# rpl-cmu/bevrender

Hardware: AMD Instinct MI355X
Metric: samples/sec fwd+bwd, 6-cam 256x704 BEV-lift+corr (higher is better)
Workload: dtype bf16; 1 GPU; cfg3: 6-cam 256x704 features (64x64x176), 200x200 BEV, C=64 h=2 D=5, L=2 encoder layers (TSA+SCA), T=2 (1 no-grad history frame(s) + 1 fwd+bwd), correlation head with contrastive + lifted-structure losses, AdamW; batch 8 per GPU; backbone/render CNN excluded; global_batch=8, per_gpu_batch=8, parallelism=dp1

## Files before the change

### bevrender_amd/_lib.py

```python
from __future__ import annotations

import ctypes as C
import os
import subprocess
import threading

import torch

_HERE = os.path.dirname(os.path.abspath(__file__))
LIB_PATH = os.environ.get("BEVRENDER_LIB") or os.path.join(_HERE, "lib", "libbevrender_hip.so")
CSRC = os.path.join(_HERE, "csrc")

PREC_F32, PREC_BF16, PREC_F16, PREC_BF16X3 = 0, 1, 2, 3
ABI_VERSION = 6

SYMBOLS = [
    "bevr_abi_version", "bevr_strerror", "bevr_attn_table_dims", "bevr_attn_key_ws_bytes", "bevr_attn_key_prep",
    "bevr_attn_fwd", "bevr_attn_bwd_q",
    "bevr_attn_bwd_k", "bevr_attn_fwd_dropout", "bevr_attn_bwd_q_dropout", "bevr_attn_bwd_k_dropout", "bevr_attn_cell_fwd", "bevr_attn_cell_bwd_q", "bevr_attn_cell_bwd_k", "bevr_attn_tap_ws_bytes", "bevr_attn_tap_prep", "bevr_attn_tap_fwd", "bevr_attn_tap_bwd_q", "bevr_attn_tap_bwd_k", "bevr_attn_tap_fwd_dropout", "bevr_attn_tap_bwd_q_dropout", "bevr_attn_tap_bwd_k_dropout", "bevr_attn_gather_fwd", "bevr_attn_gather_fwd_rows", "bevr_attn_gather_fwd_x3", "bevr_attn_slab_ws_bytes", "bevr_attn_slab_prep", "bevr_attn_slab_bwd_q", "bevr_attn_slab_rows_ws_bytes", "bevr_attn_slab_rows_prep", "bevr_attn_slab_bwd_q_rows", "bevr_sample_fwd", "bevr_sample_bwd", "bevr_sample_fwd_bf16", "bevr_sample_bwd_bf16", "bevr_project_bev_grid", "bevr_project_bev_grid_masked", "bevr_corr_fwd",
    "bevr_corr_bwd", "bevr_recall_rank", "bevr_dwconv_fwd", "bevr_dwconv_bwd_w", "bevr_dwconv_res_gelu", "bevr_affine_warp_fwd", "bevr_affine_warp_bwd",
    "bevr_offset_head_fwd", "bevr_offset_head_bwd", "bevr_key_positions_fwd", "bevr_key_positions_bwd", "bevr_kv_project", "bevr_layernorm_fwd", "bevr_layernorm_bwd", "bevr_merge_views_fwd", "bevr_merge_views_bwd", "bevr_merge_tap_fwd", "bevr_merge_tap_bwd", "bevr_attn_bwd_prep", "bevr_pack_kv", "bevr_unpack_dkv",
]


class AttnDesc(C.Structure):
    _fields_ = [(n, C.c_int32) for n in (
        "n_prob", "q_div", "heads", "groups", "S", "Sp", "N", "Np", "Ht", "Wt", "Hp", "Wp",
        "y_off", "x_off", "precision", "reserved")]


class BevrError(RuntimeError):
    pass


_lib = None
_lock = threading.Lock()


def build(verbose: bool = False) -> str:
    cmd = ["make", "-C", CSRC, "-j", "4"]
    res = subprocess.run(cmd, capture_output=True, text=True)
    if verbose or res.returncode != 0:
        print(res.stdout)
        print(res.stderr)
    if res.returncode != 0:
        raise BevrError("building libbevrender_hip.so failed (see output above)")
    return LIB_PATH


def lib() -> C.CDLL:
    global _lib
    if _lib is not None:
        return _lib
    with _lock:
        if _lib is not None:
            return _lib
        if not os.path.exists(LIB_PATH):
            raise BevrError(
                f"{LIB_PATH} not found: the HIP extension is required (no CPU fallback). "
                "Run `python -c 'import __graft_entry__ as g; g.build()'` or `make -C bevrender_amd/csrc`.")
        L = C.CDLL(LIB_PATH)
        vp, fp, ip = C.c_void_p, C.c_void_p, C.c_int
        dp = C.POINTER(AttnDesc)
        L.bevr_abi_version.restype = C.c_int
        L.bevr_strerror.restype = C.c_char_p
        L.bevr_strerror.argtypes = [C.c_int]
        L.bevr_attn_table_dims.argtypes = [dp]
        L.bevr_attn_key_ws_bytes.argtypes = [dp]
        L.bevr_attn_key_prep.argtypes = [dp, fp, fp, vp, vp]
        L.bevr_attn_fwd.argtypes = [dp, vp, vp, vp, vp, fp, fp, fp, vp]
        L.bevr_attn_bwd_q.argtypes = [dp] + [vp] * 4 + [vp, fp] + [vp, fp, fp, fp, fp, fp, vp]
        L.bevr_attn_bwd_k.argtypes = [dp] + [vp] * 4 + [fp] * 3 + [vp, vp, fp, fp, fp] + [fp] * 4 + [vp]
        u32 = C.c_uint32
        L.bevr_attn_fwd_dropout.argtypes = [dp, vp, vp, vp, vp, fp, fp, fp, u32, u32, vp]
        L.bevr_attn_bwd_q_dropout.argtypes = [dp] + [vp] * 4 + [vp, fp] + [vp, fp, fp, fp, fp, fp, u32, u32, vp]
        L.bevr_attn_bwd_k_dropout.argtypes = [dp] + [vp] * 4 + [fp] * 3 + [vp, vp, fp, fp, fp] + [fp] * 4 + [u32, u32, vp]
        L.bevr_attn_cell_fwd.argtypes = [dp, vp, vp, vp, vp, fp, fp, fp, fp, fp, vp]
        L.bevr_attn_cell_bwd_q.argtypes = [dp] + [vp] * 4 + [vp, fp] + [vp, fp, fp, fp, fp, fp, vp]
        L.bevr_attn_cell_bwd_k.argtypes = [dp] + [vp] * 4 + [vp, fp] + [vp, vp, fp, fp, fp] + [fp] * 4 + [vp]
        L.bevr_attn_tap_ws_bytes.argtypes = [dp]
        L.bevr_attn_tap_prep.argtypes = [dp, fp, fp, fp, fp, vp, vp]
        L.bevr_attn_tap_fwd.argtypes = [dp, vp, vp, fp, fp, fp, vp, vp]
        L.bevr_attn_tap_bwd_q.argtypes = [dp, vp, vp, vp, fp, fp, fp, vp]
        L.bevr_attn_tap_bwd_k.argtypes = [dp, vp, vp, vp, fp, fp, fp, fp, fp, vp]
        L.bevr_attn_tap_fwd_dropout.argtypes = [dp, vp, vp, fp, fp, fp, fp, vp, u32, u32, u32, vp]
        L.bevr_attn_tap_bwd_q_dropout.argtypes = [dp, vp, vp, vp, fp, fp, fp, u32, u32, u32, vp]
        L.bevr_attn_tap_bwd_k_dropout.argtypes = [dp, vp, vp, vp, fp, fp, fp, fp, fp, u32, u32, u32, vp]
        L.bevr_attn_gather_fwd.argtypes = [dp, vp, vp, vp, vp, vp, fp, fp, fp, vp, vp]
        L.bevr_attn_gather_fwd_rows.argtypes = [dp, vp, vp, vp, vp, vp, fp, fp, fp, vp, ip, ip, vp]
        L.bevr_attn_gather_fwd_x3.argtypes = [dp, vp, vp, vp, vp, vp, fp, fp, fp, vp, ip, ip, vp]
        L.bevr_attn_slab_ws_bytes.argtypes = [dp]
        L.bevr_attn_slab_prep.argtypes = [dp, fp, fp, vp, vp, vp]
        L.bevr_attn_slab_bwd_q.argtypes = [dp, vp, vp, vp, vp, fp, vp, fp, fp, fp, fp, fp, vp]
        L.bevr_attn_slab_rows_ws_bytes.argtypes = [dp]
        L.bevr_attn_slab_rows_prep.argtypes = [dp, fp, fp, vp, vp, vp]
        L.bevr_attn_slab_bwd_q_rows.argtypes = [dp, vp, vp, vp, vp, fp, vp, fp, fp, fp, fp, fp, ip, ip, vp]
        L.bevr_sample_fwd.argtypes = [fp, fp, fp] + [ip] * 5 + [vp]
        L.bevr_sample_bwd.argtypes = [fp] * 5 + [ip] * 5 + [vp]
        L.bevr_sample_fwd_bf16.argtypes = [vp, fp, fp] + [ip] * 5 + [vp]
        L.bevr_sample_bwd_bf16.argtypes = [vp] + [fp] * 4 + [ip] * 5 + [vp]
        L.bevr_project_bev_grid.argtypes = [fp] * 4 + [ip] * 4 + [vp]
        L.bevr_project_bev_grid_masked.argtypes = [fp] * 4 + [ip] * 4 + [vp] + [ip] * 3 + [vp]
        L.bevr_corr_fwd.argtypes = [fp] * 5 + [ip] * 4 + [vp]
        L.bevr_corr_bwd.argtypes = [fp] * 8 + [ip] * 4 + [vp]
        L.bevr_recall_rank.argtypes = [fp, vp, ip, vp]
        L.bevr_dwconv_fwd.argtypes = [fp, fp, fp, fp] + [ip] * 7 + [vp]
        L.bevr_dwconv_bwd_w.argtypes = [fp, fp, fp, fp] + [ip] * 6 + [vp]
        L.bevr_dwconv_res_gelu.argtypes = [fp] * 5 + [ip] * 6 + [vp]
        L.bevr_affine_warp_fwd.argtypes = [fp, fp, fp] + [ip] * 4 + [vp]
        L.bevr_affine_warp_bwd.argtypes = [fp, fp, fp] + [ip] * 4 + [vp]
        L.bevr_offset_head_fwd.argtypes = [fp] * 7 + [C.c_longlong] + [ip] * 4 + [C.c_float, vp]
        L.bevr_offset_head_bwd.argtypes = [fp] * 13 + [C.c_longlong] + [ip] * 4 + [C.c_float, vp]
        L.bevr_layernorm_fwd.argtypes = [fp] * 6 + [C.c_longlong, ip, C.c_float, vp]
        L.bevr_layernorm_bwd.argtypes = [fp] * 8 + [C.c_longlong, ip, vp]
        L.bevr_kv_project.argtypes = [vp, ip, fp, C.c_longlong, vp, fp] + [ip] * 9 + [vp] * 6 + [ip, vp]
        L.bevr_key_positions_fwd.argtypes = [fp, fp, vp, fp] + [ip] * 8 + [C.c_float, C.c_float, vp]
        L.bevr_key_positions_bwd.argtypes = [fp, fp, vp, fp, fp] + [ip] * 8 + [C.c_float, C.c_float, vp]
        L.bevr_pack_kv.argtypes = [fp, fp, C.c_longlong, C.c_longlong] + [ip] * 6 + [vp] * 5
        L.bevr_merge_views_fwd.argtypes = [fp] * 5 + [ip] * 6 + [vp]
        L.bevr_merge_views_bwd.argtypes = [fp] * 9 + [ip] * 6 + [vp]
        L.bevr_merge_tap_fwd.argtypes = [fp] * 7 + [ip] * 6 + [vp]
        L.bevr_merge_tap_bwd.argtypes = [fp] * 13 + [ip] * 6 + [vp]
        L.bevr_attn_bwd_prep.argtypes = [fp] * 5 + [vp, vp, fp, fp] + [ip] * 3 + [vp]
        L.bevr_unpack_dkv.argtypes = [fp] * 4 + [C.c_longlong, C.c_longlong] + [ip] * 5 + [vp]
        for name in SYMBOLS:
            fn = getattr(L, name)
            if name in ("bevr_attn_key_ws_bytes", "bevr_attn_tap_ws_bytes", "bevr_attn_slab_ws_bytes",
                        "bevr_attn_slab_rows_ws_bytes"):
                fn.restype = C.c_size_t
            elif name not in ("bevr_strerror",):
                fn.restype = C.c_int
        if L.bevr_abi_version() != ABI_VERSION:
            raise BevrError(f"libbevrender_hip.so ABI version {L.bevr_abi_version()} != {ABI_VERSION}: rebuild "
                            "(make -C bevrender_amd/csrc)")
        _lib = L
    return _lib


def check(code: int, what: str) -> None:
    if code != 0:
        msg = lib().bevr_strerror(code).decode()
        raise BevrError(f"{what} failed: {msg} (code {code})")
```

### bevrender_amd/csrc/attn_bwd_k.hip

```cpp
#include "attn_kstage.h"

#include "bevr_prof.h"

BEVR_PROF_DEFINE(bwd_k, 16)

namespace {

constexpr int KEYS_WG = 384;

struct KBox { int amin, amax; float bmin, bmax; };

__device__ __forceinline__ KBox wg_key_box(int a_lo, int a_hi, float b_lo, float b_hi, KBox* red, int n_wave, int wave,
                                           int lane) {
  KBox w;
  w.amin = lanes_min<64>(a_lo);
  w.amax = lanes_max<64>(a_hi);
  w.bmin = lanes_min<64>(b_lo);
  w.bmax = lanes_max<64>(b_hi);
  if (lane == 0) red[wave] = w;
  __syncthreads();
  KBox r = red[0];
  for (int k = 1; k < n_wave; ++k) {
    const KBox o = red[k];
    r.amin = min(r.amin, o.amin);
    r.amax = max(r.amax, o.amax);
    r.bmin = fminf(r.bmin, o.bmin);
    r.bmax = fmaxf(r.bmax, o.bmax);
  }
  return r;
}

struct Slab {
  int rows;
  int pitch;
  int ncw;
  bool fits;
};
__device__ __forceinline__ Slab make_slab(const KBox& kb, const bevr_attn_desc& d, int wcap, float rx_ceil) {
  Slab sl;
  if (kb.amax < kb.amin) {
    sl.rows = 1; sl.pitch = 1; sl.ncw = 1; sl.fits = true;
    return sl;
  }
  sl.rows = kb.amax - kb.amin + d.Sp + 1;
  sl.pitch = sl.rows + ((7 - sl.rows) & 31);
  sl.ncw = wcap / sl.pitch - 1;
  const int need = (int)floorf(kb.bmax - kb.bmin) + 4 + (int)rx_ceil + 1;
  sl.fits = sl.ncw >= need;
  return sl;
}

__device__ __forceinline__ void key_split(float a, float b, const bevr_attn_desc& d, int& A, float& fy, float& bc) {
  const KeyClamp c = key_clamp(a, b, d);
  bc = c.b;
  A = (int)c.af;
  fy = c.a - c.af;
}

constexpr int TW = 768;
constexpr int KWW = 1;

template <int PREC>
__global__ __launch_bounds__(TW, 3) void attn_bwd_k_win_kernel(
    bevr_attn_desc d, const char* __restrict__ Q, const char* __restrict__ Qt, const char* __restrict__ K,
    const char* __restrict__ V, const float* __restrict__ key_a, const float* __restrict__ key_b,
    const char* __restrict__ table_pair, const char* __restrict__ dO, const char* __restrict__ dOt,
    const float* __restrict__ LSE, const float* __restrict__ delta, const float* __restrict__ grad_scale,
    float* __restrict__ dK, float* __restrict__ dV, float* __restrict__ dkey_a, float* __restrict__ dkey_b BEVR_DROP_PARAMS) {
  constexpr int NT = is16(PREC) ? 2 : 1;
  const float kp16 = PREC == BEVR_PREC_F16 ? grad_scale[2] : 0.f, c2_16 = PREC == BEVR_PREC_F16 ? grad_scale[3] : 1.f;
  const float ds_inv = PREC == BEVR_PREC_F16 ? grad_scale[4] : 1.f, p_inv = PREC == BEVR_PREC_F16 ? grad_scale[5] : 1.f;
  typedef LdsK<PREC, NT> L;
  constexpr int EB = L::EB;
  static_assert(2 * L::BUF + L::WCAP * 4 + 256 <= 160 * 1024, "LDS budget");
  __shared__ __attribute__((aligned(16))) char smem[2 * L::BUF];
  __shared__ __attribute__((aligned(16))) float win[L::WCAP];
  __shared__ __attribute__((aligned(16))) KBox red[TW / 64];

  const int n_kb = (d.Np + KEYS_WG - 1) / KEYS_WG;
  const int n_ph = d.n_prob * d.heads;
  const int xcd = blockIdx.x & 7, slot = blockIdx.x >> 3;
  const int ph = (slot / n_kb) * 8 + xcd;
  if (ph >= n_ph) return;
  const int kblk = slot % n_kb;
  const int prob = ph / d.heads, hd = ph % d.heads;
  const int grp = hd / (d.heads / d.groups);
  const int qb = prob / d.q_div;

  const int tid = threadIdx.x, wave = tid >> 6, lane = tid & 63, lq = lane & 31, hi = lane >> 5;
  const int Mp = d.S * d.Sp;
  const int n_rb = d.Sp / 32;

  const char* Kh = K + ((size_t)ph * d.Np) * 32 * EB;
  const char* Vh = V + ((size_t)ph * d.Np) * 32 * EB;
  const float* ka = key_a + (size_t)(prob * d.groups + grp) * d.Np;
  const float* kb = key_b + (size_t)(prob * d.groups + grp) * d.Np;
  const char* tbl = table_pair + (size_t)hd * d.Wp * d.Hp * 8;
  const float rx = (float)(d.Wt - 1) / (2.0f * (float)(d.S - 1));

  bool wave_live[KWW], dead[KWW];
  int key[KWW], A[KWW];
  float fy[KWW], bcl[KWW];
  int a_lo = 0x7fffffff, a_hi = (int)0x80000000;
  float b_lo = 3.0e38f, b_hi = -3.0e38f;
#pragma unroll
  for (int w = 0; w < KWW; ++w) {
    const int k0 = kblk * KEYS_WG + (wave * KWW + w) * 32;
    wave_live[w] = k0 < d.Np;
    key[w] = wave_live[w] ? k0 + lq : lq;
    dead[w] = !wave_live[w] || key[w] >= d.N;
    key_split(ka[key[w]], kb[key[w]], d, A[w], fy[w], bcl[w]);
    if (!dead[w]) {
      a_lo = min(a_lo, A[w]); a_hi = max(a_hi, A[w]);
      b_lo = fminf(b_lo, bcl[w]); b_hi = fmaxf(b_hi, bcl[w]);
    }
  }
  const KBox box = wg_key_box(a_lo, a_hi, b_lo, b_hi, red, TW / 64, wave, lane);
  const Slab sl = make_slab(box, d, L::WCAP, ceilf(rx));
  if (!sl.fits) {
#pragma unroll
    for (int w = 0; w < KWW; ++w) {
      if (!wave_live[w]) continue;
      float* kr = dK + ((size_t)ph * d.Np + key[w]) * 32;
      float* vr = dV + ((size_t)ph * d.Np + key[w]) * 32;
      const f32x4 z = {0.f, 0.f, 0.f, 0.f};
#pragma unroll
      for (int g4 = 0; g4 < 4; ++g4) {
        *reinterpret_cast<f32x4*>(kr + 8 * g4 + 4 * hi) = z;
        *reinterpret_cast<f32x4*>(vr + 8 * g4 + 4 * hi) = z;
      }
    }
    return;
  }
  if (box.amax < box.amin) {
#pragma unroll
    for (int w = 0; w < KWW; ++w) {
      if (!wave_live[w]) continue;
      float* kr = dK + ((size_t)ph * d.Np + key[w]) * 32;
      float* vr = dV + ((size_t)ph * d.Np + key[w]) * 32;
      const f32x4 z = {0.f, 0.f, 0.f, 0.f};
#pragma unroll
      for (int g4 = 0; g4 < 4; ++g4) {
        *reinterpret_cast<f32x4*>(kr + 8 * g4 + 4 * hi) = z;
        *reinterpret_cast<f32x4*>(vr + 8 * g4 + 4 * hi) = z;
      }
    }
    return;
  }
  int arel4[KWW];
  Frag<PREC> kf[KWW], vf[KWW];
  f32x16 dk[KWW], dv[KWW];
  float da[KWW], db[KWW], fx[KWW];
  int base0[KWW], base1[KWW];
#pragma unroll
  for (int w = 0; w < KWW; ++w) {
    if (dead[w]) { A[w] = box.amin; bcl[w] = box.bmin; fy[w] = 0.f; }
    arel4[w] = (A[w] - box.amin) * 4;
    kf[w].load(Kh + (size_t)key[w] * 32 * EB, hi);
    vf[w].load(Vh + (size_t)key[w] * 32 * EB, hi);
#pragma unroll
    for (int r = 0; r < 16; ++r) { dk[w][r] = 0.f; dv[w][r] = 0.f; }
    da[w] = 0.f; db[w] = 0.f; fx[w] = 0.f; base0[w] = 0; base1[w] = 0;
  }

  QStage<PREC, TW, NT> qs;
  qs.init(tid, Q + ((size_t)(qb * d.heads + hd) * Mp) * 32 * EB, dO + ((size_t)ph * Mp) * 32 * EB,
          Qt + ((size_t)(qb * d.heads + hd) * 32) * Mp * EB, dOt + ((size_t)ph * 32) * Mp * EB,
          LSE + (size_t)ph * Mp, delta + (size_t)ph * Mp, Mp, kp16);
  const int n_tile = d.S * n_rb;
  const int n_it = (n_tile + NT - 1) / NT;
  auto first_tile = [&](int it) { return NT == 1 ? it : max(0, min(NT * it, n_tile - NT)); };
  qs.load(tid, (size_t)first_tile(0) * 32);
  qs.store(tid, smem);

  const int xbase = (int)floorf(box.bmin) - 8;
  const float inv_ncw = 1.0f / (float)sl.ncw;
  auto slot_of = [&](int X) {
    const int xs = X - xbase;
    int q = (int)((float)xs * inv_ncw);
    int r = xs - q * sl.ncw;
    r = r < 0 ? r + sl.ncw : r;
    r = r >= sl.ncw ? r - sl.ncw : r;
    return r;
  };
  int whi = -(1 << 30);
  constexpr int PF = 4;
  const int kill_off = sl.ncw * sl.pitch * 4;
  for (int r = tid; r < sl.pitch; r += TW) win[sl.ncw * sl.pitch + r] = BEVR_NEG_BIG;
  const int n_chunk = (sl.rows + 63) / 64;
  const size_t trow0 = (size_t)(box.amin + d.y_off);
  __syncthreads();

  PROF_ACC(8);
  for (int it = 0; it < n_it; ++it) {
    PROF_T_LGKM(t0, 0.f);
    const int buf = it & 1;
    const char* base = smem + buf * L::BUF;
    const int t_first = first_tile(it);
    if (it + 1 < n_it) qs.load(tid, (size_t)first_tile(it + 1) * 32);
    int pf_first = 0, pf_units = 0;
    float pf_v[PF];
#pragma unroll
    for (int sub = 0; sub < NT; ++sub) {
    const int t = t_first + sub;
    if (t < NT * it) continue;
    const int j = t / n_rb, rb = t - j * n_rb;
    if (rb == 0) {
      const float jr = (float)j * rx;
      const int xhi = (int)floorf(jr + box.bmax) + 1;
      if (whi < xhi) {
        const int xlo = (int)floorf(jr + box.bmin);
        const int xfirst = max(whi + 1, xlo);
        const int n_new = xhi - xfirst + 1;
        for (int u = wave; u < n_new * n_chunk; u += TW / 64) {
          const int c = u / n_chunk, ch = u - c * n_chunk;
          const int X = xfirst + c;
          const int row = ch * 64 + lane;
          if (row < sl.rows) {
            const float v = *reinterpret_cast<const float*>(tbl + ((size_t)(X + d.x_off) * d.Hp + trow0 + row) * 8);
            win[slot_of(X) * sl.pitch + row] = v;
          }
        }
        whi = xhi;
        __syncthreads();
      }
#pragma unroll
      for (int w = 0; w < KWW; ++w) {
        const float tx = jr + bcl[w];
        const float xf = floorf(tx);
        fx[w] = dead[w] ? 0.f : tx - xf;
        const int X = (int)xf;
        base0[w] = dead[w] ? kill_off : slot_of(X) * sl.pitch * 4 + arel4[w];
        base1[w] = dead[w] ? kill_off : slot_of(X + 1) * sl.pitch * 4 + arel4[w];
      }
    }
    if (sub == NT - 1 && rb == n_rb - 1 && j + 1 < d.S) {
      const float jr = (float)(j + 1) * rx;
      const int xhi = (int)floorf(jr + box.bmax) + 1;
      const int xfirst = max(whi + 1, (int)floorf(jr + box.bmin));
      const int units = (xhi - xfirst + 1) * n_chunk;
      if (units <= PF * (TW / 64)) {
        pf_first = xfirst;
        pf_units = units;
        whi = xhi;
#pragma unroll
        for (int k = 0; k < PF; ++k) {
          const int u = wave + k * (TW / 64);
          const int c = u / n_chunk, ch = u - c * n_chunk;
          const int row = ch * 64 + lane;
          pf_v[k] = 0.f;
          if (u < units && row < sl.rows)
            pf_v[k] = *reinterpret_cast<const float*>(tbl + ((size_t)(xfirst + c + d.x_off) * d.Hp + trow0 + row) * 8);
        }
      }
    }
    PROF_T_LGKM(t1, 0.f);
    PROF_ADD(0, t1 - t0);

#pragma unroll
    for (int w = 0; w < KWW; ++w) {
      if (!wave_live[w]) continue;
      const f32x4* rc = reinterpret_cast<const f32x4*>(base + 2 * L::TILE_Q + 2 * L::TILE_T) + sub * 8;
      f32x16 s, dp;
      {
        Frag<PREC> qf;
        qf.load(base + (sub * 32 + lq) * L::STRIDE, hi);
#pragma unroll
        for (int g4 = 0; g4 < 4; ++g4) {
          const f32x4 l4 = rc[2 * g4 + hi];
#pragma unroll
          for (int k = 0; k < 4; ++k) s[4 * g4 + k] = l4[k];
        }
        s = mma_frag(qf, kf[w], s);
      }
      {
        Frag<PREC> dof;
        dof.load(base + L::TILE_Q + (sub * 32 + lq) * L::STRIDE, hi);
#pragma unroll
        for (int g4 = 0; g4 < 4; ++g4) {
          const f32x4 d4 = rc[NT * 8 + 2 * g4 + hi];
#pragma unroll
          for (int k = 0; k < 4; ++k) dp[4 * g4 + k] = d4[k];
        }
        dp = mma_frag(dof, vf[w], dp);
      }
#if BEVR_DROP
      unsigned kmask = 0u;
      const float ksc = 65536.0f / (65536.0f - (float)drop_thr);
#pragma unroll
      for (int r = 0; r < 16; ++r) {
        const uint32_t hrow = bevr_drop_row(drop_seed, (uint32_t)ph, (uint32_t)(j * d.Sp + rb * 32 + crow(r, hi)));
        const bool keep = bevr_drop_keep(hrow, (uint32_t)key[w], drop_thr);
        const float nd = rc[NT * 8 + 2 * (r >> 2) + hi][r & 3];
        dp[r] = keep ? fmaf(ksc, dp[r] - nd, nd) : nd;
        kmask |= (keep ? 1u : 0u) << r;
      }
#endif
      PROF_T_LGKM(t2, s[0] + dp[15]);
      PROF_ADD(1, t2 - t1);

      const int ioff = (rb * 32 + 4 * hi) * 4;
      const char* p0 = reinterpret_cast<const char*>(win) + base0[w] + ioff;
      const char* p1 = reinterpret_cast<const char*>(win) + base1[w] + ioff;
      const f32x2 fy2 = {fy[w], fy[w]}, fx2 = {fx[w], fx[w]};
      f32x2 sa2 = {0.f, 0.f}, sb2 = {0.f, 0.f};
      const int n_live = d.S - rb * 32;
#pragma unroll
      for (int g4 = 0; g4 < 4; ++g4) {
        if (8 * g4 >= n_live) {
#pragma unroll
          for (int k = 0; k < 4; ++k) { s[4 * g4 + k] = 0.f; dp[4 * g4 + k] = 0.f; }
          continue;
        }
#pragma unroll
        for (int h = 0; h < 2; ++h) {
          const int r = 4 * g4 + 2 * h, o = (8 * g4 + 2 * h) * 4;
          const float* a0 = reinterpret_cast<const float*>(p0 + o);
          const float* a1 = reinterpret_cast<const float*>(p1 + o);
          const f32x2 ta = {a0[0], a0[1]}, tb = {a0[1], a0[2]};
          const f32x2 qa = {a1[0], a1[1]}, qb = {a1[1], a1[2]};
          const f32x2 d0 = tb - ta, d1 = qb - qa;
          const f32x2 u0 = ta + fy2 * d0;
          const f32x2 u1 = qa + fy2 * d1;
          const f32x2 du = u1 - u0;
          const f32x2 s2 = {s[r], s[r + 1]}, dp2 = {dp[r], dp[r + 1]};
          const f32x2 sv = (s2 + u0) + fx2 * du;
          const f32x2 pp = {fast_exp2(sv[0]), fast_exp2(sv[1])};
          f32x2 ds = pp * dp2;
          if constexpr (PREC == BEVR_PREC_F16) ds *= f32x2{c2_16, c2_16};
          s[r] = pp[0]; s[r + 1] = pp[1];
          dp[r] = ds[0]; dp[r + 1] = ds[1];
          sa2 += ds * (d0 + fx2 * (d1 - d0));
          sb2 += ds * du;
        }
      }
      const float sa = sa2[0] + sa2[1], sb = sb2[0] + sb2[1];
      da[w] += sa;
      db[w] += sb;
#if BEVR_DROP
#pragma unroll
      for (int r = 0; r < 16; ++r) s[r] = ((kmask >> r) & 1u) ? s[r] * ksc : 0.f;
#endif
      PROF_T_LGKM(t3, sa + sb + s[15]);
      PROF_ADD(2, t3 - t2);
      {
        Frag<PREC> dotf;
        load_perm(dotf, base + 2 * L::TILE_Q + L::TILE_T + lq * L::TSTRIDE + sub * 32 * EB, hi);
        dv[w] = mma_acc_b(dotf, s, dv[w]);
      }
      {
        Frag<PREC> qtf;
        load_perm(qtf, base + 2 * L::TILE_Q + lq * L::TSTRIDE + sub * 32 * EB, hi);
        dk[w] = mma_acc_b(qtf, dp, dk[w]);
      }
      PROF_T_LGKM(t4, dk[w][0] + dv[w][0]);
      PROF_ADD(3, t4 - t3);
    }

    }

    PROF_T_LGKM(t5, 0.f);
    if (pf_units > 0) {
#pragma unroll
      for (int k = 0; k < PF; ++k) {
        const int u = wave + k * (TW / 64);
        const int c = u / n_chunk, ch = u - c * n_chunk;
        const int row = ch * 64 + lane;
        if (u < pf_units && row < sl.rows) win[slot_of(pf_first + c) * sl.pitch + row] = pf_v[k];
      }
    }
    if (it + 1 < n_it) qs.store(tid, smem + (buf ^ 1) * L::BUF);
    PROF_T_LGKM(t6, 0.f);
    __syncthreads();
    PROF_T_LGKM(t7, 0.f);
    PROF_ADD(4, t6 - t5);
    PROF_ADD(5, t7 - t6);
    PROF_ADD(6, t7 - t0);
    PROF_ADD(7, 1);
  }
  PROF_FLUSH(bwd_k, wave ? 8 : 0, lane == 0 && (wave == 0 || wave == 11));

#pragma unroll
  for (int w = 0; w < KWW; ++w) {
    if (!wave_live[w]) continue;
    float* kr = dK + ((size_t)ph * d.Np + key[w]) * 32;
    float* vr = dV + ((size_t)ph * d.Np + key[w]) * 32;
#pragma unroll
    for (int g4 = 0; g4 < 4; ++g4) {
      f32x4 a, b;
#pragma unroll
      for (int k = 0; k < 4; ++k) { a[k] = BEVR_LN2 * ds_inv * dk[w][4 * g4 + k]; b[k] = p_inv * dv[w][4 * g4 + k]; }
      *reinterpret_cast<f32x4*>(kr + 8 * g4 + 4 * hi) = a;
      *reinterpret_cast<f32x4*>(vr + 8 * g4 + 4 * hi) = b;
    }
    const float sa = BEVR_LN2 * ds_inv * (da[w] + __shfl_xor(da[w], 32));
    const float sb = BEVR_LN2 * ds_inv * (db[w] + __shfl_xor(db[w], 32));
    if (hi == 0) {
      atomicAdd(dkey_a + (size_t)(prob * d.groups + grp) * d.Np + key[w], sa);
      atomicAdd(dkey_b + (size_t)(prob * d.groups + grp) * d.Np + key[w], sb);
    }
  }
}

constexpr int TG = 256;
constexpr int KW = 3;
constexpr int GSPLIT = 4;

template <int PREC>
__global__ __launch_bounds__(TG) void attn_bwd_k_gather_kernel(
    bevr_attn_desc d, const char* __restrict__ Q, const char* __restrict__ Qt, const char* __restrict__ K,
    const char* __restrict__ V, const float* __restrict__ key_a, const float* __restrict__ key_b,
    const char* __restrict__ table_pair, const char* __restrict__ dO, const char* __restrict__ dOt,
    const float* __restrict__ LSE, const float* __restrict__ delta, const float* __restrict__ grad_scale,
    float* __restrict__ dK, float* __restrict__ dV, float* __restrict__ dkey_a, float* __restrict__ dkey_b BEVR_DROP_PARAMS) {
  typedef LdsK<PREC> L;
  const float kp16 = PREC == BEVR_PREC_F16 ? grad_scale[2] : 0.f, c2_16 = PREC == BEVR_PREC_F16 ? grad_scale[3] : 1.f;
  const float ds_inv = PREC == BEVR_PREC_F16 ? grad_scale[4] : 1.f, p_inv = PREC == BEVR_PREC_F16 ? grad_scale[5] : 1.f;
  constexpr int EB = L::EB;
  __shared__ __attribute__((aligned(16))) char smem[2 * L::BUF];
  __shared__ __attribute__((aligned(16))) KBox red[4];

  const int n_kb = (d.Np + KEYS_WG - 1) / KEYS_WG;
  const int n_ph = d.n_prob * d.heads;
  const int xcd = blockIdx.x & 7, slot = blockIdx.x >> 3;
  const int ph = (slot / (n_kb * GSPLIT)) * 8 + xcd;
  if (ph >= n_ph) return;
  const int kblk = (slot % (n_kb * GSPLIT)) / GSPLIT;
  const int split = slot % GSPLIT;
  const int prob = ph / d.heads, hd = ph % d.heads;
  const int grp = hd / (d.heads / d.groups);
  const int qb = prob / d.q_div;

  const int tid = threadIdx.x, wave = tid >> 6, lane = tid & 63, lq = lane & 31, hi = lane >> 5;
  const int Mp = d.S * d.Sp;
  const int n_rb = d.Sp / 32;

  const char* Kh = K + ((size_t)ph * d.Np) * 32 * EB;
  const char* Vh = V + ((size_t)ph * d.Np) * 32 * EB;
  const float* ka = key_a + (size_t)(prob * d.groups + grp) * d.Np;
  const float* kb = key_b + (size_t)(prob * d.groups + grp) * d.Np;
  const char* tbl = table_pair + (size_t)hd * d.Wp * d.Hp * 8;
  const int Hp8 = d.Hp * 8;
  const float rx = (float)(d.Wt - 1) / (2.0f * (float)(d.S - 1));

  KeyC kc[KW];
  bool wave_live[KW];
  int key_idx[KW];
#pragma unroll
  for (int w = 0; w < KW; ++w) {
    const int k0 = kblk * KEYS_WG + (wave * KW + w) * 32;
    wave_live[w] = k0 < d.Np;
    const int key = wave_live[w] ? k0 + lq : lq;
    key_idx[w] = key;
    kc[w] = make_keyc(ka[key], kb[key], d);
  }
  KBox box;
  {
    int a_lo = 0x7fffffff, a_hi = (int)0x80000000;
    float b_lo = 3.0e38f, b_hi = -3.0e38f;
#pragma unroll
    for (int w = 0; w < KW; ++w) {
      if (wave_live[w] && key_idx[w] < d.N) {
        int A;
        float fy, bc;
        key_split(ka[key_idx[w]], kb[key_idx[w]], d, A, fy, bc);
        a_lo = min(a_lo, A); a_hi = max(a_hi, A);
        b_lo = fminf(b_lo, bc); b_hi = fmaxf(b_hi, bc);
      }
    }
    box = wg_key_box(a_lo, a_hi, b_lo, b_hi, red, TG / 64, wave, lane);
  }
  if (make_slab(box, d, L::WCAP, ceilf(rx)).fits) return;

  Frag<PREC> kf[KW], vf[KW];
#pragma unroll
  for (int w = 0; w < KW; ++w) {
    kf[w].load(Kh + (size_t)key_idx[w] * 32 * EB, hi);
    vf[w].load(Vh + (size_t)key_idx[w] * 32 * EB, hi);
  }
  f32x16 dk[KW], dv[KW];
  float da[KW], db[KW];
#pragma unroll
  for (int w = 0; w < KW; ++w) {
#pragma unroll
    for (int r = 0; r < 16; ++r) { dk[w][r] = 0.f; dv[w][r] = 0.f; }
    da[w] = 0.f;
    db[w] = 0.f;
  }

  QStage<PREC, TG> qs;
  qs.init(tid, Q + ((size_t)(qb * d.heads + hd) * Mp) * 32 * EB, dO + ((size_t)ph * Mp) * 32 * EB,
          Qt + ((size_t)(qb * d.heads + hd) * 32) * Mp * EB, dOt + ((size_t)ph * 32) * Mp * EB,
          LSE + (size_t)ph * Mp, delta + (size_t)ph * Mp, Mp, kp16);
  const int n_all = d.S * n_rb;
  const int chunk = (n_all + GSPLIT - 1) / GSPLIT;
  const int it_first = split * chunk, n_it = min(n_all, it_first + chunk);
  if (it_first >= n_it) return;
  qs.load(tid, (size_t)(it_first / n_rb) * d.Sp + (it_first % n_rb) * 32);
  qs.store(tid, smem);
  __syncthreads();

  for (int it = it_first; it < n_it; ++it) {
    const int buf = (it - it_first) & 1;
    const char* base = smem + buf * L::BUF;
    const int j = it / n_rb, i0 = (it % n_rb) * 32;
    if (it + 1 < n_it) {
      const int jn = (it + 1) / n_rb, rbn = (it + 1) % n_rb;
      qs.load(tid, (size_t)jn * d.Sp + rbn * 32);
    }
    const float jr = (float)j * rx;

    Frag<PREC> qf, dof, qtf, dotf;
    qf.load(base + lq * L::STRIDE, hi);
    dof.load(base + L::TILE + lq * L::STRIDE, hi);
    load_perm(qtf, base + 2 * L::TILE + lq * L::STRIDE, hi);
    load_perm(dotf, base + 3 * L::TILE + lq * L::STRIDE, hi);
    const f32x4* rc = reinterpret_cast<const f32x4*>(base + 4 * L::TILE);

#pragma unroll
    for (int w = 0; w < KW; ++w) {
      if (!wave_live[w]) continue;
      f32x16 s, dp;
#pragma unroll
      for (int g4 = 0; g4 < 4; ++g4) {
        f32x4 l4 = rc[2 * g4 + hi], d4 = rc[8 + 2 * g4 + hi];
#pragma unroll
        for (int k = 0; k < 4; ++k) { s[4 * g4 + k] = l4[k]; dp[4 * g4 + k] = d4[k]; }
      }
      s = mma_frag(qf, kf[w], s);
      dp = mma_frag(dof, vf[w], dp);
#if BEVR_DROP
      unsigned kmask = 0u;
      const float ksc = 65536.0f / (65536.0f - (float)drop_thr);
#pragma unroll
      for (int r = 0; r < 16; ++r) {
        const uint32_t hrow = bevr_drop_row(drop_seed, (uint32_t)ph, (uint32_t)(j * d.Sp + i0 + crow(r, hi)));
        const bool keep = bevr_drop_keep(hrow, (uint32_t)key_idx[w], drop_thr);
        const float nd = rc[8 + 2 * (r >> 2) + hi][r & 3];
        dp[r] = keep ? fmaf(ksc, dp[r] - nd, nd) : nd;
        kmask |= (keep ? 1u : 0u) << r;
      }
#endif

      const KeyC c = kc[w];
      float tx = jr + c.b;
      float xf = floorf(tx);
      float fx = tx - xf;
      const char* tp = tbl + (unsigned)((int)xf * Hp8 + c.aoff + (i0 + 4 * hi) * 8);
      const bool dead = key_idx[w] >= d.N;
      float sa = 0.f, sb = 0.f;
#pragma unroll
      for (int r = 0; r < 16; ++r) {
        f32x2 t0 = *reinterpret_cast<const f32x2*>(tp + crow(r, 0) * 8);
        f32x2 t1 = *reinterpret_cast<const f32x2*>(tp + Hp8 + crow(r, 0) * 8);
        float u0 = t0[0] * c.wy0 + t0[1] * c.fy;
        float u1 = t1[0] * c.wy0 + t1[1] * c.fy;
        float sv = s[r] + u0 + fx * (u1 - u0);
        float p = dead ? 0.f : fast_exp2(sv);
        float ds = BEVR_LN2 * c2_16 * p * dp[r];
        s[r] = p;
        dp[r] = ds;
        float ga = (t0[1] - t0[0]) + fx * ((t1[1] - t1[0]) - (t0[1] - t0[0]));
        sa += ds * ga;
        sb += ds * (u1 - u0);
      }
      da[w] += sa;
      db[w] += sb;
#if BEVR_DROP
#pragma unroll
      for (int r = 0; r < 16; ++r) s[r] = ((kmask >> r) & 1u) ? s[r] * ksc : 0.f;
#endif
      dv[w] = mma_acc_b(dotf, s, dv[w]);
      dk[w] = mma_acc_b(qtf, dp, dk[w]);
    }

    if (it + 1 < n_it) qs.store(tid, smem + (buf ^ 1) * L::BUF);
    __syncthreads();
  }

#pragma unroll
  for (int w = 0; w < KW; ++w) {
    if (!wave_live[w]) continue;
    const int key = key_idx[w];
    float* kr = dK + ((size_t)ph * d.Np + key) * 32;
    float* vr = dV + ((size_t)ph * d.Np + key) * 32;
#pragma unroll
    for (int g4 = 0; g4 < 4; ++g4) {
#pragma unroll
      for (int k = 0; k < 4; ++k) {
        atomicAdd(kr + 8 * g4 + 4 * hi + k, ds_inv * dk[w][4 * g4 + k]);
        atomicAdd(vr + 8 * g4 + 4 * hi + k, p_inv * dv[w][4 * g4 + k]);
      }
    }
    float sa = ds_inv * (da[w] + __shfl_xor(da[w], 32));
    float sb = ds_inv * (db[w] + __shfl_xor(db[w], 32));
    if (hi == 0) {
      atomicAdd(dkey_a + (size_t)(prob * d.groups + grp) * d.Np + key, sa);
      atomicAdd(dkey_b + (size_t)(prob * d.groups + grp) * d.Np + key, sb);
    }
  }
}

template <int PREC>
int launch(const bevr_attn_desc& d, const void* Q, const void* Qt, const void* K, const void* V, const float* key_a,
           const float* key_b, const float* table_pair, const void* dO, const void* dOt, const float* LSE,
           const float* delta, const float* gs, float* dK, float* dV, float* dka, float* dkb, hipStream_t st BEVR_DROP_PARAMS) {
  const int n_kb = (d.Np + KEYS_WG - 1) / KEYS_WG;
  const int n_ph = d.n_prob * d.heads;
  const int grid = ((n_ph + 7) / 8) * 8 * n_kb;
  hipLaunchKernelGGL((attn_bwd_k_win_kernel<PREC>), dim3(grid), dim3(TW), 0, st, d, (const char*)Q, (const char*)Qt,
                     (const char*)K, (const char*)V, key_a, key_b, (const char*)table_pair, (const char*)dO,
                     (const char*)dOt, LSE, delta, gs, dK, dV, dka, dkb BEVR_DROP_ARGS);
  int rc = (int)hipGetLastError();
  if (rc) return rc;
  hipLaunchKernelGGL((attn_bwd_k_gather_kernel<PREC>), dim3(grid * GSPLIT), dim3(TG), 0, st, d, (const char*)Q,
                     (const char*)Qt, (const char*)K, (const char*)V, key_a, key_b, (const char*)table_pair,
                     (const char*)dO, (const char*)dOt, LSE, delta, gs, dK, dV, dka, dkb BEVR_DROP_ARGS);
  return (int)hipGetLastError();
}

}

#if BEVR_DROP
extern "C" int bevr_attn_bwd_k_dropout(const bevr_attn_desc* d, const void* Q, const void* Qt, const void* K, const void* V,
                                       const float* key_a, const float* key_b, const float* table_pair, const void* dO,
                                       const void* dOt, const float* LSE, const float* delta, const float* grad_scale,
                                       float* dK, float* dV, float* dkey_a, float* dkey_b, unsigned drop_thr,
                                       unsigned drop_seed, void* stream) {
  if (drop_thr >= 65536u) return BEVR_E_SHAPE;
#else
extern "C" int bevr_attn_bwd_k(const bevr_attn_desc* d, const void* Q, const void* Qt, const void* K, const void* V,
                               const float* key_a, const float* key_b, const float* table_pair, const void* dO,
                               const void* dOt, const float* LSE, const float* delta, const float* grad_scale,
                               float* dK, float* dV, float* dkey_a, float* dkey_b, void* stream) {
#endif
  int rc = bevr_check_desc(d);
  if (rc) return rc;
  if (!Q || !Qt || !K || !V || !key_a || !key_b || !table_pair || !dO || !dOt || !LSE || !delta || !dK || !dV ||
      !dkey_a || !dkey_b || (d->precision == BEVR_PREC_F16 && !grad_scale))
    return BEVR_E_NULL;
  if (!bevr_aligned16(Q) || !bevr_aligned16(Qt) || !bevr_aligned16(K) || !bevr_aligned16(V) || !bevr_aligned16(dO) ||
      !bevr_aligned16(dOt) || !bevr_aligned16(dK) || !bevr_aligned16(dV) || !bevr_aligned16(table_pair))
    return BEVR_E_ALIGN;
  hipStream_t st = (hipStream_t)stream;
  if (d->precision == BEVR_PREC_BF16)
    return launch<BEVR_PREC_BF16>(*d, Q, Qt, K, V, key_a, key_b, table_pair, dO, dOt, LSE, delta, grad_scale, dK, dV,
                                  dkey_a, dkey_b, st BEVR_DROP_ARGS);
  if (d->precision == BEVR_PREC_F16)
    return launch<BEVR_PREC_F16>(*d, Q, Qt, K, V, key_a, key_b, table_pair, dO, dOt, LSE, delta, grad_scale, dK, dV,
                                 dkey_a, dkey_b, st BEVR_DROP_ARGS);
  if (d->precision == BEVR_PREC_BF16X3)
    return launch<BEVR_PREC_BF16X3>(*d, Q, Qt, K, V, key_a, key_b, table_pair, dO, dOt, LSE, delta, grad_scale, dK, dV,
                               dkey_a, dkey_b, st BEVR_DROP_ARGS);
  return launch<BEVR_PREC_F32>(*d, Q, Qt, K, V, key_a, key_b, table_pair, dO, dOt, LSE, delta, grad_scale, dK, dV,
                               dkey_a, dkey_b, st BEVR_DROP_ARGS);
}
```

### bevrender_amd/csrc/attn_tap_bwd_k.hip

```cpp
#include <type_traits>
#include "attn_tap.h"

namespace {

constexpr int NKW = 7;
constexpr int NCW = 8;
constexpr int NRX = 8;
constexpr int SPB = 2;
template <int NP> struct LdsKn {
  static constexpr int OFF_G = 0;
  static constexpr int OFF_H = 1024;
  static constexpr int OFF_LO = 2048;
  static constexpr int SLAB = 2048 * NP;
  static constexpr int BUF = SPB * SLAB;
};
typedef LdsKn<1> LdsK;
template <int PREC> using LdsKp = LdsKn<tap_np<PREC>>;
constexpr int tap_bwd_k_waves(int prec) { return tap_split(prec) ? 2 : 4; }
__host__ __device__ __forceinline__ int win_dwords(int Sp) { return (Sp + NRX + 8) / 2; }

__device__ __forceinline__ bool tile_fits(const StepBox& sb, float jrx, int a0w, float bminw) {
  const int da = sb.amin - a0w;
  const int dx = (int)floorf(jrx + sb.bmin) - (int)floorf(jrx + bminw);
  return sb.amax >= sb.amin && da >= 0 && da <= NRX && box_fits(sb, jrx) && dx >= 0 && dx <= NCW - CELL_C;
}

template <int PREC, bool SLOW>
__global__ __launch_bounds__(64 * (NKW + 1), tap_bwd_k_waves(PREC)) void attn_tap_bwd_k_kernel(
    bevr_attn_desc d, const char* __restrict__ G, const char* __restrict__ H, const char* __restrict__ tap_ws,
    const float* __restrict__ table_t, float* __restrict__ dkey_a, float* __restrict__ dkey_b,
    float* __restrict__ dkey_y, float* __restrict__ dkey_x, int n_wg_ph TAP_DROP_PARAMS) {
  typedef LdsKp<PREC> L;
  constexpr bool X3 = tap_split(PREC);
  constexpr int NP = tap_np<PREC>;
  extern __shared__ __attribute__((aligned(16))) char smem[];

  const int n_ph = d.n_prob * d.heads;
  const int xcd = blockIdx.x & 7, slot = blockIdx.x >> 3;
  const int ph = (slot / n_wg_ph) * 8 + xcd;
  if (ph >= n_ph) return;
  const int wg = slot % n_wg_ph;
  const int prob = ph / d.heads, hd = ph % d.heads;
  const int tid = threadIdx.x;
  const int wave = __builtin_amdgcn_readfirstlane(tid >> 6), lane = tid & 63;
  const int li = lane & 15, g = lane >> 4;
  const int Mp = d.S * d.Sp;
  const int nslab = d.Sp / 32, nstep = (nslab + SPB - 1) / SPB;
  const int n_tiles = d.Np / 32;
  const float rx = (float)(d.Wt - 1) / (2.0f * (float)(d.S - 1));
  const int HpT = d.Hp + 1;
  const float* tbl = table_t + (size_t)hd * d.Wp * HpT;
  const StepBox* box = reinterpret_cast<const StepBox*>(tap_ws + tap_ws_box_offset(d)) + (size_t)prob * (d.Np / 32);
  const int NRWD = win_dwords(d.Sp);
  const int win_bytes = 4 * NCW * NRWD * 4;
  char* win_base = smem + 2 * L::BUF;
  TapRec* stash = reinterpret_cast<TapRec*>(win_base + 3 * win_bytes) + wave * 32;

  int a0w = 0x7fffffff;
  float bminw = 3.0e38f;
  for (int t = 0; t < NKW; ++t) {
    const int tile = wg * NKW + t;
    if (tile < n_tiles) {
      const StepBox b = box[tile];
      if (b.amax >= b.amin) {
        a0w = min(a0w, b.amin);
        bminw = fminf(bminw, b.bmin);
      }
    }
  }
  if (a0w == 0x7fffffff) { a0w = 0; bminw = 0.f; }
  if constexpr (SLOW) {
    bool unfit = false;
    for (int t = 0; t < NKW; ++t) {
      const int tile = wg * NKW + t;
      if (tile >= n_tiles) break;
      const StepBox b = box[tile];
      if (b.amax < b.amin) continue;
      for (int j = lane; j < d.S; j += 64) unfit = unfit || !tile_fits(b, (float)j * rx, a0w, bminw);
    }
    if (!__any(unfit)) return;
  }

  if (wave == NKW) {
    __builtin_amdgcn_s_setprio(3);
    const int n_quad = (NRWD + 1) / 2, n_item = NCW * n_quad;
    auto item_load = [&](int jn, int it, float (&t)[5]) {
      if (it >= n_item || jn >= d.S) return;
      const int c = it / n_quad, m = it - c * n_quad;
      const int x0w = (int)floorf((float)jn * rx + bminw);
      const int xc = max(0, min(x0w + c + d.x_off, d.Wp - 1));
      const int y = max(0, min(a0w + d.y_off + 4 * m, HpT - 5));
      const float* src = tbl + (size_t)xc * HpT + y;
#pragma unroll
      for (int k = 0; k < 5; ++k) t[k] = src[k];
    };
    auto item_store = [&](int jn, int it, const float (&t)[5]) {
      if (it >= n_item || jn >= d.S) return;
      const int c = it / n_quad, m = it - c * n_quad;
      const uint32_t h01 = TapHalf<PREC>::pack2(t[0], t[1]), h23 = TapHalf<PREC>::pack2(t[2], t[3]);
      const uint32_t h12 = TapHalf<PREC>::pack2(t[1], t[2]), h34 = TapHalf<PREC>::pack2(t[3], t[4]);
      const uint32_t l01 = TapHalf<PREC>::pack2(t[0] - TapHalf<PREC>::lo(h01), t[1] - TapHalf<PREC>::hi(h01));
      const uint32_t l23 = TapHalf<PREC>::pack2(t[2] - TapHalf<PREC>::lo(h23), t[3] - TapHalf<PREC>::hi(h23));
      const uint32_t l12 = TapHalf<PREC>::pack2(t[1] - TapHalf<PREC>::lo(h12), t[2] - TapHalf<PREC>::hi(h12));
      const uint32_t l34 = TapHalf<PREC>::pack2(t[3] - TapHalf<PREC>::lo(h34), t[4] - TapHalf<PREC>::hi(h34));
      uint32_t* w = reinterpret_cast<uint32_t*>(win_base + (jn % 3) * win_bytes) + c * NRWD + 2 * m;
      const bool second = 2 * m + 1 < NRWD;
      w[0] = h01;
      w[NCW * NRWD] = h12;
      w[2 * NCW * NRWD] = l01;
      w[3 * NCW * NRWD] = l12;
      if (second) {
        w[1] = h23;
        w[NCW * NRWD + 1] = h34;
        w[2 * NCW * NRWD + 1] = l23;
        w[3 * NCW * NRWD + 1] = l34;
      }
    };
    const int per_step = (n_item + nstep - 1) / nstep;
    auto slice_item = [&](int s2, int r) {
      const int k = r * 64 + lane;
      return k < per_step ? s2 * per_step + k : n_item;
    };
    float f0[5] = {0.f, 0.f, 0.f, 0.f, 0.f}, f1[5] = {0.f, 0.f, 0.f, 0.f, 0.f};
    if constexpr (!SLOW) {
      for (int it = lane; it < n_item; it += 64) {
        float t[5] = {0.f, 0.f, 0.f, 0.f, 0.f};
        item_load(0, it, t);
        item_store(0, it, t);
      }
      item_load(1, slice_item(0, 0), f0);
      item_load(1, slice_item(0, 1), f1);
    }
    const char* Gp = G + ((size_t)ph * Mp) * 32 + lane * 16;
    const char* Hq = H + ((size_t)ph * Mp) * 32 + lane * 16;
    auto slab_index = [&](int j2, int st2, int u) { return min(j2 * nslab + min(SPB * st2 + u, nslab - 1), d.S * nslab - 1); };
    int e = 0;
    u32x4 gv[NP][SPB], hv[NP][SPB];
    const size_t g_lo = (size_t)n_ph * Mp * 32;
    auto rows_load = [&](int j2, int st2) {
#pragma unroll
      for (int pl = 0; pl < NP; ++pl)
#pragma unroll
        for (int u = 0; u < SPB; ++u) {
          gv[pl][u] = gload16(Gp + pl * g_lo + (size_t)slab_index(j2, st2, u) * 1024);
          hv[pl][u] = gload16(Hq + pl * g_lo + (size_t)slab_index(j2, st2, u) * 1024);
        }
    };
    rows_load(0, 0);
    for (int j = 0; j < d.S; ++j) {
      for (int st = 0; st < nstep; ++st, ++e) {
        char* bb = smem + (e & 1) * L::BUF;
#pragma unroll
        for (int pl = 0; pl < NP; ++pl)
#pragma unroll
          for (int u = 0; u < SPB; ++u) {
            *reinterpret_cast<u32x4*>(bb + u * L::SLAB + pl * L::OFF_LO + L::OFF_G + lane * 16) = gv[pl][u];
            *reinterpret_cast<u32x4*>(bb + u * L::SLAB + pl * L::OFF_LO + L::OFF_H + lane * 16) = hv[pl][u];
          }
        if constexpr (!SLOW) {
          item_store(j + 1, slice_item(st, 0), f0);
          item_store(j + 1, slice_item(st, 1), f1);
          for (int k = 128 + lane; k < per_step; k += 64) {
            float t[5] = {0.f, 0.f, 0.f, 0.f, 0.f};
            item_load(j + 1, st * per_step + k, t);
            item_store(j + 1, st * per_step + k, t);
          }
        }
        const int jn = st + 1 < nstep ? j : min(j + 1, d.S - 1), stn = st + 1 < nstep ? st + 1 : 0;
        rows_load(jn, stn);
        if constexpr (!SLOW) {
          const int jf = st + 1 < nstep ? j + 1 : j + 2;
          item_load(jf, slice_item(stn, 0), f0);
          item_load(jf, slice_item(stn, 1), f1);
        }
        __syncthreads();
      }
    }
    __syncthreads();
    return;
  }

  const int tile = wg * NKW + wave;
  const bool have_tile = tile < n_tiles;
  const TapRec* recs = reinterpret_cast<const TapRec*>(tap_ws) + (size_t)prob * d.Np;
  const int tl = have_tile ? tile : 0;
  const StepBox sb = box[tl];
  const int da = sb.amin - a0w;

  TapOp<NP> bk[2];
  f32x4 zt[2], zv[2], zc[2];
  float acc_a[2] = {0.f, 0.f}, acc_b[2] = {0.f, 0.f};
#pragma unroll
  for (int kb = 0; kb < 2; ++kb) {
    const TapRec r0 = recs[(size_t)tl * 32 + 16 * kb + li];
    if (g == 0) stash[16 * kb + li] = r0;
    TapOp<NP> t[2];
    tap_weights<PREC>(r0.ys, r0.xs, t);
#pragma unroll
    for (int pl = 0; pl < NP; ++pl) bk[kb].p[pl] = g == 0 ? t[0].p[pl] : t[1].p[pl];
    zt[kb] = f32x4{0.f, 0.f, 0.f, 0.f};
    zv[kb] = f32x4{0.f, 0.f, 0.f, 0.f};
    zc[kb] = f32x4{0.f, 0.f, 0.f, 0.f};
  }
  const int a_row = L::OFF_G + li * 32 + (g & 1) * 16;
  const int t_off = (4 * g + (li >> 2)) * 32 + (lane & 3) * 8;
  const int cell_c = li >> 2, cell_r = li & 3;
#if BEVR_DROP
  uint32_t khk[2];
#pragma unroll
  for (int kb = 0; kb < 2; ++kb)
    khk[kb] = ((key0 + (uint32_t)(tl * 32 + 16 * kb + li)) * 0xC2B2AE3Du) ^ drop_seed ^ ((uint32_t)ph * 0x9E3779B1u);
  uint32_t hcol = 0u;
#endif

  int e = 0;
  float jrx = 0.f;
  const char* win_b = nullptr;
  int wq0 = 0, wq1 = 0, wth = 0, wtl = 0;
  const int win_lo = 2 * NCW * NRWD * 4;
  auto slab = [&](auto fit_tag, const char* base, int i0) {
    constexpr bool FIT = decltype(fit_tag)::value;
    TapOp<NP> qa[2], ha[2];
#pragma unroll
    for (int rb = 0; rb < 2; ++rb) {
      qa[rb] = ha[rb] = TapOp<NP>{};
      if (g < 2) {
        qa[rb] = tap_ld<NP>(base + a_row + rb * 512, L::OFF_LO);
        ha[rb] = tap_ld<NP>(base + L::OFF_H - L::OFF_G + a_row + rb * 512, L::OFF_LO);
      } else if (FIT) {
#pragma unroll
        for (int pl = 0; pl < NP; ++pl) {
          const uint32_t* w0 = reinterpret_cast<const uint32_t*>(win_b + pl * win_lo + wq0 + 2 * i0) + 8 * rb;
          const uint32_t* w1 = reinterpret_cast<const uint32_t*>(win_b + pl * win_lo + wq1 + 2 * i0) + 8 * rb;
          qa[rb].p[pl] = __builtin_bit_cast(bf16x8, u32x4{w0[0], w0[1], w1[0], w1[1]});
        }
      }
    }
    const TapOp<NP> gt = tap_ld_tr<NP>(base + L::OFF_G + t_off, 512, L::OFF_LO);
    const TapOp<NP> ht = tap_ld_tr<NP>(base + L::OFF_H + t_off, 512, L::OFF_LO);
    bf16x8 thi = gt.p[0], tlo = gt.p[0];
    if constexpr (FIT) {
      const uint32_t* w0 = reinterpret_cast<const uint32_t*>(win_b + wth + 2 * i0);
      const uint32_t* w1 = reinterpret_cast<const uint32_t*>(win_b + wtl + 2 * i0);
      thi = __builtin_bit_cast(bf16x8, u32x4{w0[0], w0[1], w0[8], w0[9]});
      tlo = __builtin_bit_cast(bf16x8, u32x4{w1[0], w1[1], w1[8], w1[9]});
    }
#if BEVR_DROP
    const uint32_t hq0 = hcol + (uint32_t)i0 * 0x85EBCA77u;
    auto hq = [&](int r) { return hq0 + (uint32_t)(16 * (r >> 2) + (r & 3)) * 0x85EBCA77u; };
    float ndel[8];
#pragma unroll
    for (int r = 0; r < 8; ++r) {
      const uint32_t c2 = *reinterpret_cast<const uint32_t*>(base + L::OFF_H + (16 * (r >> 2) + 4 * g + (r & 3)) * 32 + TAP_CHI * 2);
      ndel[r] = TapHalf<PREC>::lo(c2) + TapHalf<PREC>::hi(c2);
    }
#endif
#pragma unroll
    for (int kb = 0; kb < 2; ++kb) {
      const f32x4 z4 = {0.f, 0.f, 0.f, 0.f};
      const f32x4 s0 = tap_mm<PREC, true>(qa[0], bk[kb], z4);
      const f32x4 s1 = tap_mm<PREC, true>(qa[1], bk[kb], z4);
      const f32x4 q0 = tap_mm<PREC>(ha[0], bk[kb], z4);
      const f32x4 q1 = tap_mm<PREC>(ha[1], bk[kb], z4);
      float p[8], ds[8];
      if constexpr (!FIT) {
        const TapRec rk = stash[16 * kb + li];
        const float a = rk.a, tx = jrx + rk.b;
        const float af = floorf(a), xf = floorf(tx);
        const float fy = a - af, fx = tx - xf;
        const bool dead = rk.ys < -50.0f;
        const int xc = max(0, min((int)xf + d.x_off, d.Wp - 2));
        const int yb = (int)af + d.y_off + i0 + 4 * g;
        float pa = 0.f, pb = 0.f;
#pragma unroll
        for (int r = 0; r < 8; ++r) {
          const int y = max(0, min(yb + (r & 3) + 16 * (r >> 2), HpT - 2));
          const float* c0p = tbl + (size_t)xc * HpT + y;
          const float t00 = c0p[0], t01 = c0p[1], t10 = c0p[HpT], t11 = c0p[HpT + 1];
          const float u0 = t00 + fy * (t01 - t00), u1 = t10 + fy * (t11 - t10);
          const float sv = (r < 4 ? s0[r & 3] : s1[r & 3]) + (dead ? 0.f : u0 + fx * (u1 - u0));
          p[r] = fast_exp2(sv);
#if BEVR_DROP
          {
            const bool keep = tap_drop_keep(hq(r), khk[kb], drop_thr);
            ds[r] = p[r] * (keep ? (r < 4 ? q0[r & 3] : q1[r & 3]) : ndel[r]);
            p[r] = keep ? p[r] : 0.f;
          }
#else
          ds[r] = p[r] * (r < 4 ? q0[r & 3] : q1[r & 3]);
#endif
          pa += ds[r] * ((1.0f - fx) * (t01 - t00) + fx * (t11 - t10));
          pb += ds[r] * (u1 - u0);
        }
        acc_a[kb] += dead ? 0.f : pa;
        acc_b[kb] += dead ? 0.f : pb;
      } else {
#pragma unroll
        for (int r = 0; r < 4; ++r) {
#if BEVR_DROP
          p[r] = fast_exp2(s0[r]);
          p[4 + r] = fast_exp2(s1[r]);
          const bool keep0 = tap_drop_keep(hq(r), khk[kb], drop_thr), keep1 = tap_drop_keep(hq(4 + r), khk[kb], drop_thr);
          ds[r] = p[r] * (keep0 ? q0[r] : ndel[r]);
          ds[4 + r] = p[4 + r] * (keep1 ? q1[r] : ndel[4 + r]);
          p[r] = keep0 ? p[r] : 0.f;
          p[4 + r] = keep1 ? p[4 + r] : 0.f;
#else
          p[r] = fast_exp2(s0[r]);
          ds[r] = p[r] * q0[r];
          p[4 + r] = fast_exp2(s1[r]);
          ds[4 + r] = p[4 + r] * q1[r];
#endif
        }
      }
      u32x4 dsw[NP], pw[NP];
#pragma unroll
      for (int k = 0; k < 4; ++k) {
        tap_pack2<PREC>(ds[2 * k], ds[2 * k + 1], k, dsw);
        tap_pack2<PREC>(p[2 * k], p[2 * k + 1], k, pw);
      }
      const TapOp<NP> ds8 = tap_op(dsw), p8 = tap_op(pw);
      zt[kb] = tap_mm<PREC>(gt, ds8, zt[kb]);
      zv[kb] = tap_mm<PREC>(ht, p8, zv[kb]);
      if constexpr (FIT) {
        zc[kb] = mfma16<PREC>(tlo, ds8.p[0], zc[kb]);
        if constexpr (X3) zc[kb] = mfma16<PREC>(thi, ds8.p[1], zc[kb]);
        zc[kb] = mfma16<PREC>(thi, ds8.p[0], zc[kb]);
      }
    }
  };

  for (int j = 0; j < d.S; ++j) {
    jrx = (float)j * rx;
#if BEVR_DROP
    hcol = (uint32_t)(j * d.Sp + 4 * g) * 0x85EBCA77u;
#endif
    const int x0 = (int)floorf(jrx + sb.bmin), a0 = sb.amin;
    const int dx = x0 - (int)floorf(jrx + bminw);
    const bool fit = tile_fits(sb, jrx, a0w, bminw);
    const bool mine = have_tile && sb.amax >= sb.amin && fit != SLOW;
    auto chunk_coords = [&](int kb, float& tcol, float& trow) {
      const TapRec rk = stash[16 * kb + li];
      const float tx = jrx + rk.b;
      const float xf = floorf(tx);
      tcol = rk.ys < -50.0f ? -8.0f : (xf - (float)x0) + (tx - xf);
      trow = rk.a - (float)a0;
    };
#pragma unroll
    for (int kb = 0; kb < 2; ++kb) {
      if (g >= 2) {
        bk[kb] = TapOp<NP>{};
        if (!SLOW && mine) {
          float tcol, trow;
          chunk_coords(kb, tcol, trow);
          bk[kb] = tap_cell_half<PREC>(tcol, trow, g - 2);
        }
      }
      zc[kb] = f32x4{0.f, 0.f, 0.f, 0.f};
    }
    win_b = win_base + (j % 3) * win_bytes;
    {
      const int iq = li + da, pq = iq & 1;
      wq0 = ((pq * NCW + dx + 2 * max(g - 2, 0)) * NRWD + ((iq - pq) >> 1)) * 4;
      wq1 = wq0 + NRWD * 4;
      const int it = 4 * g + cell_r + da, pt = it & 1;
      wth = ((pt * NCW + dx + cell_c) * NRWD + ((it - pt) >> 1)) * 4;
      wtl = wth + win_lo;
    }
    for (int st = 0; st < nstep; ++st, ++e) {
      __syncthreads();
      if (!mine) continue;
#pragma unroll
      for (int u = 0; u < SPB; ++u)
        if (SPB * st + u < nslab) slab(std::integral_constant<bool, !SLOW>{}, smem + (e & 1) * L::BUF + u * L::SLAB, 32 * (SPB * st + u));
    }
    if (!SLOW && mine) {
#pragma unroll
      for (int kb = 0; kb < 2; ++kb) {
        float tc, tr;
        chunk_coords(kb, tc, tr);
        const float c0 = floorf(tc), r0 = floorf(tr);
        const float wxg = hat((float)g - tc);
        const float z0 = zc[kb][0], z1 = zc[kb][1], z2 = zc[kb][2], z3 = zc[kb][3];
        const float zl = r0 < 0.5f ? z0 : (r0 < 1.5f ? z1 : z2);
        const float zh = r0 < 0.5f ? z1 : (r0 < 1.5f ? z2 : z3);
        const float zrow = hat(0.f - tr) * z0 + hat(1.f - tr) * z1 + hat(2.f - tr) * z2 + hat(3.f - tr) * z3;
        const float sg = ((float)g == c0 + 1.0f ? 1.0f : 0.f) - ((float)g == c0 ? 1.0f : 0.f);
        acc_a[kb] += wxg * (zh - zl);
        acc_b[kb] += sg * zrow;
      }
    }
  }
  __syncthreads();

  if (!have_tile) return;
#pragma unroll
  for (int kb = 0; kb < 2; ++kb) {
    const TapRec rk = stash[16 * kb + li];
    const float ys = rk.ys, xs = rk.xs;
    const float y0 = floorf(ys), x0f = floorf(xs);
    float gy = 0.f, gx = 0.f;
#pragma unroll
    for (int e2 = 0; e2 < 4; ++e2) {
      const int t = 4 * g + e2;
      const float r = (float)(t / 3), c = (float)(t % 3);
      const float dwy = (r == y0 + 1.0f ? 1.0f : 0.f) - (r == y0 ? 1.0f : 0.f);
      const float dwx = (c == x0f + 1.0f ? 1.0f : 0.f) - (c == x0f ? 1.0f : 0.f);
      const float z = g < 3 ? zt[kb][e2] + BEVR_LOG2E * zv[kb][e2] : 0.f;
      gy += z * dwy * hat(c - xs);
      gx += z * hat(r - ys) * dwx;
    }
    float va = acc_a[kb], vb = acc_b[kb];
    gy += __shfl_xor(gy, 16); gx += __shfl_xor(gx, 16); va += __shfl_xor(va, 16); vb += __shfl_xor(vb, 16);
    gy += __shfl_xor(gy, 32); gx += __shfl_xor(gx, 32); va += __shfl_xor(va, 32); vb += __shfl_xor(vb, 32);
    const int n = tile * 32 + 16 * kb + li;
    if (g == 0 && n < d.N) {
      const size_t idx = (size_t)prob * d.Np + n;
      atomicAdd(dkey_a + idx, va);
      atomicAdd(dkey_b + idx, vb);
      atomicAdd(dkey_y + idx, gy);
      atomicAdd(dkey_x + idx, gx);
    }
  }
}

template <int PREC>
int launch(const bevr_attn_desc& d, const void* G, const void* H, const void* tap_ws, const float* table_t, float* dkey_a,
           float* dkey_b, float* dkey_y, float* dkey_x, hipStream_t st TAP_DROP_PARAMS) {
  typedef LdsKp<PREC> L;
  const int n_ph = d.n_prob * d.heads;
  const int n_tiles = d.Np / 32;
  const int n_wg_ph = (n_tiles + NKW - 1) / NKW;
  const size_t lds = 2 * L::BUF + (size_t)3 * 4 * NCW * win_dwords(d.Sp) * 4 + NKW * 32 * sizeof(TapRec);
  if (lds > 160 * 1024) return BEVR_E_SHAPE;
  const long long grid = (long long)((n_ph + 7) / 8) * 8 * n_wg_ph;
  if (grid > 0x7fffffffLL) return BEVR_E_SHAPE;
  hipLaunchKernelGGL((attn_tap_bwd_k_kernel<PREC, false>), dim3((unsigned)grid), dim3(64 * (NKW + 1)), lds, st, d, (const char*)G,
                     (const char*)H, (const char*)tap_ws, table_t, dkey_a, dkey_b, dkey_y, dkey_x, n_wg_ph TAP_DROP_ARGS);
  const int rc = (int)hipGetLastError();
  if (rc) return rc;
  hipLaunchKernelGGL((attn_tap_bwd_k_kernel<PREC, true>), dim3((unsigned)grid), dim3(64 * (NKW + 1)), lds, st, d, (const char*)G,
                     (const char*)H, (const char*)tap_ws, table_t, dkey_a, dkey_b, dkey_y, dkey_x, n_wg_ph TAP_DROP_ARGS);
  return (int)hipGetLastError();
}

}

#if BEVR_TAP_X3
int bevr_tap_bwd_k_x3(const bevr_attn_desc& d, const void* G, const void* H, const void* tap_ws, const float* table_t,
                      float* dkey_a, float* dkey_b, float* dkey_y, float* dkey_x, hipStream_t st) {
  return launch<BEVR_PREC_BF16X3>(d, G, H, tap_ws, table_t, dkey_a, dkey_b, dkey_y, dkey_x, st);
}
#else
#if BEVR_DROP
extern "C" int bevr_attn_tap_bwd_k_dropout(const bevr_attn_desc* d, const void* G, const void* H, const void* tap_ws,
                                           const float* table_t, float* dkey_a, float* dkey_b, float* dkey_y,
                                           float* dkey_x, unsigned key0, unsigned drop_thr, unsigned drop_seed,
                                           void* stream) {
  if (drop_thr >= 65536u) return BEVR_E_SHAPE;
#else
extern "C" int bevr_attn_tap_bwd_k(const bevr_attn_desc* d, const void* G, const void* H, const void* tap_ws,
                                   const float* table_t, float* dkey_a, float* dkey_b, float* dkey_y, float* dkey_x,
                                   void* stream) {
#endif
  int rc = bevr_check_desc(d);
  if (rc) return rc;
  if (!G || !H || !tap_ws || !table_t || !dkey_a || !dkey_b || !dkey_y || !dkey_x) return BEVR_E_NULL;
  if (d->groups != 1) return BEVR_E_SHAPE;
  if (!bevr_aligned16(G) || !bevr_aligned16(H) || !bevr_aligned16(tap_ws)) return BEVR_E_ALIGN;
  hipStream_t st = (hipStream_t)stream;
  if (d->precision == BEVR_PREC_BF16) return launch<BEVR_PREC_BF16>(*d, G, H, tap_ws, table_t, dkey_a, dkey_b, dkey_y, dkey_x, st TAP_DROP_ARGS);
  if (d->precision == BEVR_PREC_F16) return launch<BEVR_PREC_F16>(*d, G, H, tap_ws, table_t, dkey_a, dkey_b, dkey_y, dkey_x, st TAP_DROP_ARGS);
#if !BEVR_DROP
  if (d->precision == BEVR_PREC_BF16X3) return bevr_tap_bwd_k_x3(*d, G, H, tap_ws, table_t, dkey_a, dkey_b, dkey_y, dkey_x, st);
#endif
  return BEVR_E_PRECISION;
}
#endif
```

### bevrender_amd/ops.py

```python
from __future__ import annotations

import ctypes as C
import math
import os
from dataclasses import dataclass, replace as dc_replace
from types import SimpleNamespace
from typing import Optional, Tuple

import torch
import torch.nn.functional as F

from . import _lib

LOG2E = 1.4426950408889634
HEAD_DIM = 32


def perm32(r: int) -> int:
    return (r & ~12) | ((r & 4) << 1) | ((r & 8) >> 1)


_PERM_CACHE = {}


def perm_index(n: int, device) -> torch.Tensor:
    key = (n, str(device))
    if key not in _PERM_CACHE:
        base = torch.arange(n, device=device)
        r = base % 32
        pr = (r & ~12) | ((r & 4) << 1) | ((r & 8) >> 1)
        _PERM_CACHE[key] = (base - r + pr)
    return _PERM_CACHE[key]


@dataclass(frozen=True)
class AttnGeom:
    n_prob: int
    q_div: int
    heads: int
    groups: int
    S: int
    N: int
    Wt: int
    precision: int

    @property
    def Sp(self): return 32 * ((self.S + 31) // 32)
    @property
    def Mp(self): return self.S * self.Sp
    @property
    def Np(self): return 64 * ((self.N + 63) // 64)
    @property
    def Ht(self): return 2 * self.S - 1
    @property
    def y_off(self): return self.Sp + 2
    @property
    def Hp(self): return self.Ht + 2 * self.Sp + 4
    @property
    def x_off(self): return self.Wt // 2 + 4
    @property
    def Wp(self): return self.Wt + 2 * (self.Wt // 2) + 9
    @property
    def rx(self): return (self.Wt - 1) / (2.0 * (self.S - 1))

    def desc(self) -> _lib.AttnDesc:
        return _lib.AttnDesc(self.n_prob, self.q_div, self.heads, self.groups, self.S, self.Sp, self.N, self.Np,
                             self.Ht, self.Wt, self.Hp, self.Wp, self.y_off, self.x_off, self.precision, 0)


def pack_query(query: torch.Tensor, heads: int) -> torch.Tensor:
    B, Cc, S, _ = query.shape
    c = Cc // heads
    if c > HEAD_DIM:
        raise ValueError(f"head_dim {c} > {HEAD_DIM} is not supported by the gfx950 kernels")
    Sp = 32 * ((S + 31) // 32)
    q = query.reshape(B, heads, c, S, S) * (c ** -0.5 * LOG2E)
    q = q.permute(0, 1, 4, 3, 2)
    q = F.pad(q, (0, HEAD_DIM - c, 0, Sp - S))
    return q.reshape(B, heads, S * Sp, HEAD_DIM)


def pack_keys(x: torch.Tensor, heads: int) -> torch.Tensor:
    Bp, N, Cc = x.shape
    c = Cc // heads
    Np = 64 * ((N + 63) // 64)
    k = x.reshape(Bp, N, heads, c).permute(0, 2, 1, 3)
    return F.pad(k, (0, HEAD_DIM - c, 0, Np - N))


def unpack_out(O: torch.Tensor, S: int, c: int) -> torch.Tensor:
    Bp, h, Mp, _ = O.shape
    Sp = Mp // S
    o = O.reshape(Bp, h, S, Sp, HEAD_DIM)[:, :, :, :S, :c]
    return o.permute(0, 3, 2, 1, 4).reshape(Bp, S * S, h * c)


def unpack_out_views(O: torch.Tensor, S: int, c: int, views: int) -> torch.Tensor:
    BV, h, Mp, _ = O.shape
    Sp = Mp // S
    o = O.reshape(BV // views, views, h, S, Sp, HEAD_DIM)[:, :, :, :, :S, :c]
    return o.permute(0, 4, 3, 1, 2, 5).reshape(BV // views, S * S, views * h * c)


class _LinearRows(torch.autograd.Function):

    @staticmethod
    def forward(ctx, x, weight, bias):
        ctx.save_for_backward(x, weight)
        ctx.has_bias = bias is not None
        return F.linear(x, weight, bias)

    @staticmethod
    def backward(ctx, dy):
        x, weight = ctx.saved_tensors
        K, N = x.shape[-1], dy.shape[-1]
        d2, x2 = dy.reshape(-1, N), x.reshape(-1, K)
        R = d2.shape[0]
        dx = dw = db = None
        if ctx.needs_input_grad[0]:
            dx = (d2 @ weight).reshape(x.shape)
        if ctx.needs_input_grad[1]:
            nfull = R // LINEAR_ROWS_CHUNK
            n0 = nfull * LINEAR_ROWS_CHUNK
            dw = torch.bmm(d2[:n0].reshape(nfull, LINEAR_ROWS_CHUNK, N).transpose(1, 2),
                           x2[:n0].reshape(nfull, LINEAR_ROWS_CHUNK, K)).sum(0)
            if n0 < R:
                dw = dw + d2[n0:].t() @ x2[n0:]
        if ctx.has_bias and ctx.needs_input_grad[2]:
            db = d2.sum(0)
        return dx, dw, db


LINEAR_ROWS_CHUNK = 4096
LINEAR_ROWS_MIN = 65536


def linear_rows(x: torch.Tensor, weight: torch.Tensor, bias: Optional[torch.Tensor] = None) -> torch.Tensor:
    if not x.is_cuda or x.dtype != torch.float32 or x.numel() // x.shape[-1] < LINEAR_ROWS_MIN or not x.is_contiguous():
        return F.linear(x, weight, bias)
    return _LinearRows.apply(x, weight, bias)


class _MergeViews(torch.autograd.Function):

    @staticmethod
    def forward(ctx, O_r, L_r, O_c, L_c, S, c, views):
        _require_gpu(O_r, L_r, O_c, L_c)
        BV, h, Mp, hd = O_r.shape
        assert hd == HEAD_DIM and Mp % S == 0 and BV % views == 0
        two = O_c is not None
        O_r = O_r.float().contiguous()
        if two:
            O_c, L_r, L_c = O_c.float().contiguous(), L_r.float().contiguous(), L_c.float().contiguous()
            assert O_c.shape == O_r.shape and L_r.shape == L_c.shape == O_r.shape[:3]
        out = torch.empty(BV // views, S * S, views * h * c, device=O_r.device, dtype=torch.float32)
        nbytes = float((O_r.numel() * (2 if two else 1)) * S / (Mp // S) * c / HEAD_DIM * 4 + out.numel() * 4)
        _launch("bevr_merge_views_fwd", _ptr(O_r), _ptr(L_r) if two else None, _ptr(O_c) if two else None,
                _ptr(L_c) if two else None, _ptr(out), BV, views, h, S, Mp // S, c, _stream(), flops=0.0, nbytes=nbytes)
        ctx.save_for_backward(*((O_r, L_r, O_c, L_c) if two else ()))
        ctx.dims = (BV, views, h, S, Mp // S, c, two)
        return out

    @staticmethod
    def backward(ctx, dout):
        BV, views, h, S, Sp, c, two = ctx.dims
        dout = dout.float().contiguous()
        dO_r = torch.empty(BV, h, S * Sp, HEAD_DIM, device=dout.device, dtype=torch.float32)
        if two:
            O_r, L_r, O_c, L_c = ctx.saved_tensors
            dO_c, dL_r, dL_c = torch.empty_like(dO_r), torch.empty_like(L_r), torch.empty_like(L_c)
        else:
            O_r = L_r = O_c = L_c = dO_c = dL_r = dL_c = None
        nbytes = float(dout.numel() * 4 * (5 if two else 2))
        _launch("bevr_merge_views_bwd", _ptr(dout), _ptr(O_r) if two else None, _ptr(L_r) if two else None,
                _ptr(O_c) if two else None, _ptr(L_c) if two else None, _ptr(dO_r), _ptr(dL_r) if two else None,
                _ptr(dO_c) if two else None, _ptr(dL_c) if two else None, BV, views, h, S, Sp, c, _stream(), flops=0.0,
                nbytes=nbytes)
        return dO_r, dL_r, dO_c, dL_c, None, None, None


class _MergeTap(torch.autograd.Function):

    @staticmethod
    def forward(ctx, O_r, L_r, Rn, L_c, Vp, bv, S, c, views):
        _require_gpu(O_r, L_r, Rn, L_c, Vp, bv)
        BV, h, Mp, hd = O_r.shape
        assert hd == HEAD_DIM and Mp % S == 0 and BV % views == 0 and Rn.shape == (BV, h, Mp, TAP_N)
        assert Vp.shape == (BV, h, TAP_N, HEAD_DIM) and bv.shape == (h, HEAD_DIM)
        O_r, L_r, Rn, L_c, Vp, bv = (t.float().contiguous() for t in (O_r, L_r, Rn, L_c, Vp, bv))
        out = torch.empty(BV // views, S * S, views * h * c, device=O_r.device, dtype=torch.float32)
        live = S / (Mp // S)
        nbytes = float(O_r.numel() * live * (c / HEAD_DIM + TAP_N / HEAD_DIM) * 4 + out.numel() * 4)
        _launch("bevr_merge_tap_fwd", _ptr(O_r), _ptr(L_r), _ptr(Rn), _ptr(L_c), _ptr(Vp), _ptr(bv), _ptr(out), BV, views, h, S,
                Mp // S, c, _stream(), flops=0.0, nbytes=nbytes, timer="bevr_merge_views_fwd")
        ctx.save_for_backward(O_r, L_r, Rn, L_c, Vp, bv)
        ctx.dims = (BV, views, h, S, Mp // S, c)
        return out

    @staticmethod
    def backward(ctx, dout):
        BV, views, h, S, Sp, c = ctx.dims
        O_r, L_r, Rn, L_c, Vp, bv = ctx.saved_tensors
        dout = dout.float().contiguous()
        dO_r, dL_r, dRn, dL_c = torch.empty_like(O_r), torch.empty_like(L_r), torch.empty_like(Rn), torch.empty_like(L_c)
        dVp, dbv = torch.zeros_like(Vp), torch.zeros_like(bv)
        nbytes = float(dout.numel() * 4 * (3 + 2 * TAP_N / HEAD_DIM))
        _launch("bevr_merge_tap_bwd", _ptr(dout), _ptr(O_r), _ptr(L_r), _ptr(Rn), _ptr(L_c), _ptr(Vp), _ptr(bv), _ptr(dO_r),
                _ptr(dL_r), _ptr(dRn), _ptr(dL_c), _ptr(dVp), _ptr(dbv), BV, views, h, S, Sp, c, _stream(), flops=0.0,
                nbytes=nbytes, timer="bevr_merge_views_bwd")
        return dO_r, dL_r, dRn, dL_c, dVp, dbv, None, None, None


def merge_tap(O_r, L_r, Rn, L_c, Vp, bv, S: int, c: int, views: int) -> torch.Tensor:
    return _MergeTap.apply(O_r, L_r, Rn, L_c, Vp, bv, S, c, views)


def merge_views(O_r: torch.Tensor, S: int, c: int, views: int, L_r=None, O_c=None, L_c=None) -> torch.Tensor:
    if c % 4 != 0:
        if O_c is not None:
            L_t = torch.logaddexp2(L_r, L_c)
            O_r = torch.exp2(L_r - L_t)[..., None] * O_r + torch.exp2(L_c - L_t)[..., None] * O_c
        return unpack_out_views(O_r, S, c, views)
    return _MergeViews.apply(O_r, L_r, O_c, L_c, S, c, views)


def key_coords(pos: torch.Tensor, S: int, Wt: int, Np: int) -> Tuple[torch.Tensor, torch.Tensor]:
    a = (1.0 - pos[..., 0]) * ((S - 1) / 2.0)
    b = (1.0 - pos[..., 1]) * ((Wt - 1) / 4.0)
    N = pos.shape[1]
    return F.pad(a, (0, Np - N)).contiguous(), F.pad(b, (0, Np - N)).contiguous()


def pack_table(rpe_table: torch.Tensor, g: AttnGeom) -> torch.Tensor:
    t = rpe_table * LOG2E
    t = F.pad(t, (g.x_off, g.Wp - g.Wt - g.x_off, g.y_off, g.Hp + 1 - g.Ht - g.y_off))
    return t.transpose(1, 2).contiguous()


def kd_key_order(pos_ref, S: int, Wt: int, leaf: int = 32):
    import numpy as np
    leaf = int(os.environ.get("BEVR_KD_LEAF", leaf))
    pr = np.asarray(pos_ref, dtype=np.float64)
    a = (1.0 - pr[:, 0]) * ((S - 1) / 2.0)
    b = (1.0 - pr[:, 1]) * ((Wt - 1) / 4.0)
    out = []

    def rec(ids):
        n = len(ids)
        if n <= leaf:
            out.append(ids)
            return
        ka, kb = a[ids], b[ids]
        key = ka if (ka.max() - ka.min()) >= (kb.max() - kb.min()) else kb
        order = np.argsort(key, kind="stable")
        n_leaf = -(-n // leaf)
        left = (n_leaf // 2) * leaf
        rec(ids[order[:left]])
        rec(ids[order[left:]])

    rec(np.arange(len(pr)))
    return np.concatenate(out)


def split_key_order(ref_yx, S: int, Wt: int, min_cell_keys: int = 1024):
    import numpy as np
    yx = np.asarray(ref_yx, dtype=np.float64)
    V, N, _ = yx.shape
    pinned = (yx == -1.0).all(-1)
    n_b = (int(pinned.sum(1).min()) // 64) * 64
    if n_b < min_cell_keys or os.environ.get("BEVR_CELL", "1") == "0":
        n_b = 0
    orders = []
    for v in range(V):
        ip = np.nonzero(pinned[v])[0]
        seg_b = ip[len(ip) - n_b:] if n_b else ip[:0]
        keep = np.ones(N, dtype=bool)
        keep[seg_b] = False
        seg_a = np.nonzero(keep)[0]
        seg_a = seg_a[kd_key_order(yx[v][seg_a], S, Wt)]
        orders.append(torch.from_numpy(np.concatenate((seg_a, seg_b))))
    return torch.stack(orders, 0), N - n_b


def _require_gpu(*tensors):
    for t in tensors:
        if t is not None and not t.is_cuda:
            raise _lib.BevrError("bevrender_amd ops need ROCm device tensors; there is no CPU fallback")


def _ptr(t: Optional[torch.Tensor]):
    return None if t is None else C.c_void_p(t.data_ptr())


def _stream():
    return C.c_void_p(torch.cuda.current_stream().cuda_stream)


class _KernelTimer:

    def __init__(self):
        self.on = False
        self.records = []
        self.by_tag = {}

    def start(self):
        self.on, self.records = True, []

    def stop(self):
        self.on = False
        torch.cuda.synchronize()
        out = {}
        self.by_tag = {}
        for name, flops, nbytes, e0, e1, tag in self.records:
            ms = e0.elapsed_time(e1)
            for key, dst in ((name, out), (f"{name}[{tag}]", self.by_tag)):
                r = dst.setdefault(key, {"ms": 0.0, "n": 0, "flops": 0.0, "bytes": 0.0, "max_ms": 0.0})
                r["ms"] += ms
                r["max_ms"] = max(r["max_ms"], ms)
                r["n"] += 1
                r["flops"] += flops
                r["bytes"] += nbytes
        self.records = []
        return out

    def run(self, name, flops, fn, *args, nbytes=0.0, tag=""):
        if not self.on:
            return fn(*args)
        e0, e1 = torch.cuda.Event(enable_timing=True), torch.cuda.Event(enable_timing=True)
        e0.record()
        rc = fn(*args)
        e1.record()
        self.records.append((name, flops, nbytes, e0, e1, tag))
        return rc


KERNEL_TIMER = _KernelTimer()


def _edtype(precision: int):
    return {_lib.PREC_BF16: torch.bfloat16, _lib.PREC_F16: torch.float16}.get(precision, torch.float32)


def _perm_t(x: torch.Tensor) -> torch.Tensor:
    L = x.shape[-2]
    return x.index_select(-2, perm_index(L, x.device)).transpose(-1, -2).contiguous()


def _split_rows(x: torch.Tensor) -> torch.Tensor:
    sh = x.shape[:-1]
    hi = x.to(torch.bfloat16)
    lo = (x - hi.float()).to(torch.bfloat16)
    out = torch.stack((hi.reshape(*sh, 2, 16), lo.reshape(*sh, 2, 16)), dim=-2)
    return out.reshape(*sh, 64).contiguous().view(torch.float32)


def _unsplit_rows(xs: torch.Tensor) -> torch.Tensor:
    sh = xs.shape[:-1]
    b = xs.contiguous().view(torch.bfloat16).reshape(*sh, 2, 2, 16).float()
    return (b[..., 0, :] + b[..., 1, :]).reshape(*sh, 32)


def _split_perm_t(x: torch.Tensor) -> torch.Tensor:
    y = _perm_t(x)
    sh, L = y.shape[:-1], y.shape[-1]
    hi = y.to(torch.bfloat16)
    lo = (y - hi.float()).to(torch.bfloat16)
    out = torch.stack((hi.reshape(*sh, L // 32, 2, 2, 8), lo.reshape(*sh, L // 32, 2, 2, 8)), dim=-4)
    return out.transpose(-3, -2).reshape(*sh, 2 * L).contiguous().view(torch.float32)


def _attn_flops(geom, n_matmul, n_keys=None):
    n = geom.N if n_keys is None else n_keys
    return 2.0 * HEAD_DIM * geom.n_prob * geom.heads * (geom.S * geom.S) * n * n_matmul


def _call_tag(geom) -> str:
    return ("tsa" if geom.Wt == 2 * geom.S - 1 else "sca") + f",N={geom.N}"


def cell_order(a: torch.Tensor, b: torch.Tensor, n_tail: int = 0) -> torch.Tensor:
    A = torch.floor(a).to(torch.int64)
    Bc = torch.floor(b).to(torch.int64)
    A = A - A.amin(1, keepdim=True)
    Bc = Bc - Bc.amin(1, keepdim=True)
    nB = Bc.amax(1, keepdim=True) + 1
    snake = torch.where(A % 2 == 0, Bc, nB - 1 - Bc)
    cid = (A * nB + snake).to(torch.int32)
    order = cid.argsort(1)
    if n_tail <= 0:
        return order
    P, N = cid.shape
    s = cid.gather(1, order)
    idx = torch.arange(N, device=cid.device, dtype=torch.int32).expand(P, N)
    pop = torch.searchsorted(s, s, right=True, out_int32=True) - torch.searchsorted(s, s, right=False, out_int32=True)
    if N <= 65536:
        tail = (pop.clamp(max=32767) * 65536 + idx).topk(n_tail, dim=1, largest=False, sorted=False).indices
    else:
        tail = pop.argsort(dim=1, stable=True)[:, :n_tail]
    flag = torch.ones(P, N, dtype=torch.uint8, device=cid.device).scatter_(1, tail, 0)
    return order.gather(1, flag.argsort(dim=1, stable=True))


def _u32(x):
    return x & 0xFFFFFFFF


def dropout_keep_mask(seed: int, thr16: int, n_ph: int, S: int, N: int, device="cpu", rows=None) -> torch.Tensor:
    Sp = 32 * ((S + 31) // 32)
    i = torch.arange(S, dtype=torch.int64, device=device)
    mq = (i[None, :] * Sp + i[:, None]).reshape(-1)
    if rows is not None:
        mq = mq[torch.as_tensor(rows, dtype=torch.int64, device=device)]
    ph = torch.arange(n_ph, dtype=torch.int64, device=device)
    n = torch.arange(N, dtype=torch.int64, device=device)
    row = _u32(seed ^ _u32(ph * 0x9E3779B1)[:, None] ^ _u32(mq * 0x85EBCA77)[None, :])
    x = _u32(row[:, :, None] ^ _u32(n * 0xC2B2AE3D)[None, None, :])
    x = x ^ (x >> 16)
    x = _u32(x * 0x7FEB352D)
    x = x ^ (x >> 15)
    x = _u32(x * 0x846CA68B)
    x = x ^ (x >> 16)
    return (x >> 16) >= thr16


def _launch(entry, *args, flops=None, nbytes=0.0, tag="", timer=None, label=None):
    fn = getattr(_lib.lib(), entry)
    rc = fn(*args) if flops is None else KERNEL_TIMER.run(timer or entry, flops, fn, *args, nbytes=nbytes, tag=tag)
    _lib.check(rc, label or entry)


class K:
    FWD, FWD_DROP = "bevr_attn_fwd", "bevr_attn_fwd_dropout"
    GATHER, GATHER_ROWS = "bevr_attn_gather_fwd", "bevr_attn_gather_fwd_rows"
    GATHER_X3 = "bevr_attn_gather_fwd_x3"
    BWD_Q, BWD_Q_DROP, SLAB_BWD_Q = "bevr_attn_bwd_q", "bevr_attn_bwd_q_dropout", "bevr_attn_slab_bwd_q"
    SLAB_BWD_Q_ROWS = "bevr_attn_slab_bwd_q_rows"
    BWD_K, BWD_K_DROP = "bevr_attn_bwd_k", "bevr_attn_bwd_k_dropout"
    CELL_FWD, CELL_BWD_Q, CELL_BWD_K = "bevr_attn_cell_fwd", "bevr_attn_cell_bwd_q", "bevr_attn_cell_bwd_k"
    TAP_FWD, TAP_FWD_DROP = "bevr_attn_tap_fwd", "bevr_attn_tap_fwd_dropout"
    TAP_BWD_Q, TAP_BWD_Q_DROP = "bevr_attn_tap_bwd_q", "bevr_attn_tap_bwd_q_dropout"
    TAP_BWD_K, TAP_BWD_K_DROP = "bevr_attn_tap_bwd_k", "bevr_attn_tap_bwd_k_dropout"


@dataclass(frozen=True)
class KeySegment:
    kind: str
    n0: int
    n1: int
    fwd: str
    bwd_q: str
    bwd_k: str


@dataclass(frozen=True)
class AttnRoute:
    segments: Tuple[KeySegment, ...]
    split: int
    gather: Optional[str]
    kn2: bool
    merge: str

    @property
    def tap(self) -> bool:
        return self.segments[-1].kind == "tap"

    @property
    def n_core(self) -> int:
        return self.segments[-1].n0 if self.tap else self.segments[-1].n1


def attention_route(precision: int, groups: int, S: int, Wt: int, N: int, cell_split: Optional[int] = None,
                    tap_source=False, dropout: bool = False, source: str = "kv", C: int = HEAD_DIM, heads: int = 1,
                    keys_in_tap_grid=None) -> AttnRoute:
    if dropout:
        if source == "tap_pix":
            raise ValueError("tap_pix has no attention dropout: pass every key's projected rows and no tap segment")
        if not (tap_source and cell_split is not None and source == "kv_source"
                and tap_supported(precision, groups, dropout=True) and 16 * ((S + 15) // 16) <= 448):
            cell_split, tap_source = None, None
    if source == "kv_source" and not kv_source_supported(C, heads, groups, precision):
        raise ValueError("kv_source needs a 16-bit operand mode, C % 16 == 0 and (C / groups) % 4 == 0")
    split = N if cell_split is None else int(cell_split)
    if not 0 <= split <= N:
        raise ValueError("cell_split must lie in [0, N]")
    if dropout and tap_source and tap_source != "pinned" and split < N:
        if not (split > 0 and keys_in_tap_grid(split)):
            tap_source, split = None, N
    tap = bool(tap_source) and split < N
    if tap and (source == "kv" or not tap_supported(precision, groups, dropout=dropout) or 16 * ((S + 15) // 16) > 448):
        raise ValueError("tap_source needs kv_source or tap_pix, groups == 1, a precision tap_supported accepts and S <= 448")
    if source == "tap_pix" and not tap:
        raise ValueError("tap_pix needs a tap segment: 0 <= cell_split < N")
    Sp = 32 * ((S + 31) // 32)
    f32_layout = precision in (_lib.PREC_F32, _lib.PREC_BF16X3)
    n_region = split
    if not tap and split < N and (Sp > 480 or (f32_layout and Sp > 224) or (N - split) > 8 * 100 * 1024):
        n_region = N
    segs, gather = [], None
    if n_region > 0:
        if dropout:
            segs.append(KeySegment("region", 0, n_region, K.FWD_DROP, K.BWD_Q_DROP, K.BWD_K_DROP))
        else:
            if gather_supported(precision, S):
                gather = "whole" if len(gather_bands(S)) == 1 else "bands"
            if precision == _lib.PREC_BF16X3 and gather:
                fwd = K.GATHER_X3
            else:
                fwd = {None: K.FWD, "whole": K.GATHER, "bands": K.GATHER_ROWS}[gather]
            if slab_rows_supported(precision, S, Wt):
                bwd_q = K.SLAB_BWD_Q_ROWS
            else:
                bwd_q = K.SLAB_BWD_Q if slab_supported(precision, S, Wt) else K.BWD_Q
            segs.append(KeySegment("region", 0, n_region, fwd, bwd_q, K.BWD_K))
    if tap and dropout:
        segs.append(KeySegment("tap", split, N, K.TAP_FWD_DROP, K.TAP_BWD_Q_DROP, K.TAP_BWD_K_DROP))
    elif tap:
        segs.append(KeySegment("tap", split, N, K.TAP_FWD, K.TAP_BWD_Q, K.TAP_BWD_K))
    elif n_region < N:
        segs.append(KeySegment("cell", n_region, N, K.CELL_FWD, K.CELL_BWD_Q, K.CELL_BWD_K))
    kn2 = source == "kv_source" and gather is not None and os.environ.get("BEVR_KNORM", "1") != "0"
    fused_merge = (tap and split > 0 and not dropout and (C // heads) % 4 == 0
                   and os.environ.get("BEVR_MERGE_TAP", "1") != "0")
    return AttnRoute(tuple(segs), split, gather, kn2, "merge_tap" if fused_merge else "merge_views")


def gather_supported(precision, S) -> bool:
    if S > GATHER_MAX_S or os.environ.get("BEVR_GATHER", "1") == "0":
        return False
    if precision == _lib.PREC_BF16X3:
        return os.environ.get("BEVR_GATHER_X3", GATHER_X3_DEFAULT) != "0"
    return precision in (_lib.PREC_BF16, _lib.PREC_F16)


GATHER_MAX_S, GATHER_BAND_ROWS = 448, 224
GATHER_X3_DEFAULT = "0"


def gather_split_table(pair: torch.Tensor) -> torch.Tensor:
    hi = pair.to(torch.bfloat16)
    return torch.stack((hi, (pair.float() - hi.float()).to(torch.bfloat16))).contiguous()


def gather_bands(S):
    n = -(-S // GATHER_BAND_ROWS)
    step = 16 * (-(-S // (16 * n)))
    return [(r, min(step, S - r)) for r in range(0, S, step)]


def slab_supported(precision, S, Wt=None) -> bool:
    mode = os.environ.get("BEVR_SLAB", "1")
    if mode == "0" or precision not in (_lib.PREC_BF16, _lib.PREC_F16) or S > 211:
        return False
    return mode == "2" or Wt is None or Wt - 1 >= 4 * (S - 1)


SLAB_ROWS_MAX_S, SLAB_BAND_BLOCKS = 448, 7


def slab_rows_supported(precision, S, Wt=None) -> bool:
    mode = os.environ.get("BEVR_SLAB_ROWS", "0")
    if mode not in ("1", "2") or precision not in (_lib.PREC_BF16, _lib.PREC_F16) or S > SLAB_ROWS_MAX_S:
        return False
    if mode == "2":
        return True
    slab = os.environ.get("BEVR_SLAB", "1")
    return S > 211 and slab != "0" and (slab == "2" or Wt is None or Wt - 1 >= 4 * (S - 1))


def slab_bands(S, max_blocks=None):
    max_blocks = SLAB_BAND_BLOCKS if max_blocks is None else max_blocks
    nb = -(-S // 31)
    n = -(-nb // max_blocks)
    step = 31 * (-(-nb // n))
    return [(r, min(step, S - r)) for r in range(0, S, step)]


def backward_scales(bound: torch.Tensor, pmax_log2: torch.Tensor, f16: bool, drop_thr: int = 0) -> torch.Tensor:
    dev = bound.device
    if drop_thr:
        pmax_log2 = pmax_log2 + math.log2(65536.0 / (65536.0 - drop_thr))
    zero, one = torch.zeros((), device=dev), torch.ones((), device=dev)
    if f16:
        kp = torch.floor(14.0 - pmax_log2)
        e16 = torch.floor(14.0 - torch.log2(bound) - pmax_log2).clamp(-100.0, 100.0)
        return torch.stack((torch.exp2(e16 + 16.0), torch.exp2(-e16 - 16.0), kp, torch.exp2(e16 - kp),
                            torch.exp2(-e16), torch.exp2(-kp), zero, zero)).float().contiguous()
    e = torch.floor(30.0 - torch.log2(bound) - pmax_log2).clamp(-100.0, 100.0)
    return torch.stack((torch.exp2(e), torch.exp2(-e), zero, one, one, one, zero, zero)).float().contiguous()


def _fwd_tile(name, o):
    _launch(name, C.byref(o.desc), _ptr(o.Qe), _ptr(o.Ke), _ptr(o.Vt), _ptr(o.key_ws), _ptr(o.pair), _ptr(o.O), _ptr(o.LSE),
            *o.drop, _stream(), flops=_attn_flops(o.g, 2), tag=_call_tag(o.g))


def _fwd_cell(name, o):
    chain = (_ptr(o.O), _ptr(o.LSE)) if o.chained else (None, None)
    _launch(name, C.byref(o.desc), _ptr(o.Qe), _ptr(o.Ke), _ptr(o.Vt), _ptr(o.key_ws), _ptr(o.pair), *chain, _ptr(o.O),
            _ptr(o.LSE), _stream(), flops=_attn_flops(o.g, 2), tag=_call_tag(o.g))


def _fwd_gather(name, o):
    g, Ttc = o.g, o.Ttc
    x3 = name == K.GATHER_X3
    pair_pk = gather_split_table(o.pair) if x3 else o.pair.to(o.Qe.dtype)
    tmax = torch.maximum(Ttc.amax(-1).amax(-1), -Ttc.amin(-1).amin(-1))
    qn = torch.linalg.vector_norm(o.Qp if x3 else o.Qe, dim=-1, dtype=torch.float32)
    if o.kn2 is not None:
        kmx = o.kn2.sqrt()
    elif x3:
        kmx = torch.linalg.vector_norm(o.krows.reshape(g.n_prob, g.N, g.heads, -1), dim=-1, dtype=torch.float32).amax(1)
    else:
        kmx = torch.linalg.vector_norm(o.Ke[:, :, :g.N], dim=-1, dtype=torch.float32).amax(-1)
    ub = 1.01 * (qn.repeat_interleave(g.q_div, 0) * kmx[..., None] + tmax[None, :, None]) + 0.01
    mref = (ub - tap_headroom(g.precision)).contiguous()
    bands = gather_bands(g.S) if name in (K.GATHER_ROWS, K.GATHER_X3) else [()]
    gflags = torch.zeros(len(bands), g.n_prob * g.heads * g.S, device=o.O.device, dtype=torch.int32)
    for bi, rows in enumerate(bands):
        flops = _attn_flops(g, 2) * rows[1] / g.S if rows else _attn_flops(g, 2)
        _launch(name, C.byref(o.desc), _ptr(o.Qe), _ptr(o.Ke), _ptr(o.Ve), _ptr(o.key_ws), _ptr(pair_pk), _ptr(mref),
                _ptr(o.O), _ptr(o.LSE), _ptr(gflags[bi]), *rows, _stream(), flops=flops, tag=_call_tag(g), timer=K.GATHER)


def _bwd_q_tile(name, o):
    _launch(name, C.byref(o.desc), _ptr(o.Qe), _ptr(o.Ke), _ptr(o.Kt), _ptr(o.Ve), _ptr(o.key_ws), _ptr(o.pair), _ptr(o.dOe),
            _ptr(o.LSE), _ptr(o.delta), _ptr(o.gscale), _ptr(o.dQ), _ptr(o.dT), *o.drop, _stream(),
            flops=_attn_flops(o.g, 3), tag=_call_tag(o.g))


def _slab_operands(o, ws_bytes, prep):
    g, Ke, Ve = o.g, o.Ke, o.Ve
    order = o.kb[:, :g.N].argsort(1)
    hpg = g.heads // g.groups
    idx = order.view(g.n_prob, g.groups, 1, g.N).expand(-1, -1, hpg, -1).reshape(g.n_prob, g.heads, g.N, 1)
    idx = idx.expand(-1, -1, -1, HEAD_DIM)
    Ks, Vs = Ke[:, :, :g.N].gather(2, idx), Ve[:, :, :g.N].gather(2, idx)
    sws = torch.empty(getattr(_lib.lib(), ws_bytes)(C.byref(o.desc)), device=Ke.device, dtype=torch.uint8)
    _launch(prep, C.byref(o.desc), _ptr(o.ka), _ptr(o.kb), _ptr(order.to(torch.int32).contiguous()), _ptr(sws), _stream())
    return Ks, Vs, sws


def _bwd_q_slab(name, o):
    g = o.g
    Ks, Vs, sws = _slab_operands(o, "bevr_attn_slab_ws_bytes", "bevr_attn_slab_prep")
    _launch(name, C.byref(o.desc), _ptr(o.Qe), _ptr(Ks), _ptr(Vs), _ptr(sws), _ptr(o.pair), _ptr(o.dOe), _ptr(o.LSE),
            _ptr(o.delta), _ptr(o.gscale), _ptr(o.dQ), _ptr(o.dT), _stream(), flops=_attn_flops(g, 3), tag=_call_tag(g))


def _bwd_q_slab_rows(name, o):
    g = o.g
    Ks, Vs, sws = _slab_operands(o, "bevr_attn_slab_rows_ws_bytes", "bevr_attn_slab_rows_prep")
    for row0, n_rows in slab_bands(g.S):
        _launch(name, C.byref(o.desc), _ptr(o.Qe), _ptr(Ks), _ptr(Vs), _ptr(sws), _ptr(o.pair), _ptr(o.dOe), _ptr(o.LSE),
                _ptr(o.delta), _ptr(o.gscale), _ptr(o.dQ), _ptr(o.dT), row0, n_rows, _stream(),
                flops=_attn_flops(g, 3) * n_rows / g.S, tag=_call_tag(g), timer=K.SLAB_BWD_Q)


def _bwd_k(name, o, *keys):
    _launch(name, C.byref(o.desc), _ptr(o.Qe), _ptr(o.Qt), _ptr(o.Ke), _ptr(o.Ve), *keys, _ptr(o.pair), _ptr(o.dOe),
            _ptr(o.dOt), _ptr(o.LSE), _ptr(o.delta), _ptr(o.gscale), _ptr(o.dK), _ptr(o.dV), _ptr(o.da), _ptr(o.db), *o.drop,
            _stream(), flops=_attn_flops(o.g, 4), tag=_call_tag(o.g))


def _bwd_k_tile(name, o):
    _bwd_k(name, o, _ptr(o.ka), _ptr(o.kb))


def _bwd_k_cell(name, o):
    _bwd_k(name, o, _ptr(o.key_ws))


def _tap_fwd(name, o):
    _launch(name, C.byref(o.desc), _ptr(o.G16), _ptr(o.ws), _ptr(o.pair), _ptr(o.mref), _ptr(o.R), *o.lsum, _ptr(o.flags),
            *o.drop, _stream(), flops=_attn_flops(o.g, 2), tag=_call_tag(o.g))


def _tap_bwd_q(name, o):
    _launch(name, C.byref(o.desc), _ptr(o.Gq), _ptr(o.H16), _ptr(o.ws), _ptr(o.pair), _ptr(o.dG), _ptr(o.dT), *o.drop,
            _stream(), flops=_attn_flops(o.g, 3), tag=_call_tag(o.g))


def _tap_bwd_k(name, o):
    _launch(name, C.byref(o.desc), _ptr(o.Gq), _ptr(o.H16), _ptr(o.ws), _ptr(o.Ttc), *[_ptr(t) for t in o.dk], *o.drop,
            _stream(), flops=_attn_flops(o.g, 4), tag=_call_tag(o.g))


_RUN = {K.FWD: _fwd_tile, K.FWD_DROP: _fwd_tile, K.GATHER: _fwd_gather, K.GATHER_ROWS: _fwd_gather,
        K.GATHER_X3: _fwd_gather, K.CELL_FWD: _fwd_cell,
        K.BWD_Q: _bwd_q_tile, K.BWD_Q_DROP: _bwd_q_tile, K.CELL_BWD_Q: _bwd_q_tile, K.SLAB_BWD_Q: _bwd_q_slab,
        K.SLAB_BWD_Q_ROWS: _bwd_q_slab_rows,
        K.BWD_K: _bwd_k_tile, K.BWD_K_DROP: _bwd_k_tile, K.CELL_BWD_K: _bwd_k_cell,
        K.TAP_FWD: _tap_fwd, K.TAP_FWD_DROP: _tap_fwd, K.TAP_BWD_Q: _tap_bwd_q, K.TAP_BWD_Q_DROP: _tap_bwd_q,
        K.TAP_BWD_K: _tap_bwd_k, K.TAP_BWD_K_DROP: _tap_bwd_k}


def _run(name, o):
    _RUN[name](name, o)


def _kv_source_adjoint(dkv, feat, spos, Wkv, G, need_dfeat, need_dW, need_dbias):
    nb, Hi, Wi, Cc = feat.shape
    fg = feat.reshape(nb, Hi, Wi, G, Cc // G).permute(0, 3, 1, 2, 4).reshape(nb * G, Hi, Wi, Cc // G).contiguous()
    xs = _Sample.sample(fg, spos).reshape(nb, G, -1, Cc // G).permute(0, 2, 1, 3).reshape(nb, -1, Cc)
    d2 = dkv.reshape(-1, dkv.shape[-1])
    dW = torch.bmm(dkv.transpose(1, 2), xs).sum(0) if need_dW else None
    dbias = d2.sum(0) if need_dbias else None
    dxs = (d2 @ Wkv.float()).reshape(nb, -1, G, Cc // G).permute(0, 2, 1, 3).reshape(nb * G, -1, Cc // G).contiguous()
    del xs
    dfg, dspos = _Sample.scatter(fg, spos, dxs, need_dfeat)
    dfeat = None if dfg is None else dfg.reshape(nb, G, Hi, Wi, Cc // G).permute(0, 2, 3, 1, 4).reshape(feat.shape)
    return dfeat, dspos, dW, dbias


class _AttnCore(torch.autograd.Function):

    @staticmethod
    def forward(ctx, Qp, kv, key_a, key_b, Tt, geom: AttnGeom, route: AttnRoute, feat=None, spos=None, Wkv=None, bkv=None,
                drop=None):
        _require_gpu(Qp, kv, key_a, key_b, Tt, feat, spos, Wkv, bkv)
        L = _lib.lib()
        ed = _edtype(geom.precision)
        ctx.drop = drop if drop and drop[0] > 0 else None
        x3 = geom.precision == _lib.PREC_BF16X3
        Qe = _split_rows(Qp.float()) if x3 else Qp.to(ed).contiguous()
        fused = kv is None
        if fused:
            feat, spos = feat.contiguous(), spos.float().contiguous()
            N, C2 = spos.shape[1], 2 * feat.shape[-1]
            W_e = Wkv.detach().to(ed).contiguous()
            vn2 = torch.zeros(1, device=Qp.device, dtype=torch.float32)
            b_f = None if bkv is None else bkv.detach().float().contiguous()
        else:
            kv = kv.float().contiguous()
            N, C2 = kv.shape[1], kv.shape[-1]
        c = C2 // 2 // geom.heads
        dev = Qp.device
        segs = [sg for sg in route.segments if sg.kind != "tap"]
        Ttc = Tt.contiguous()
        pair = torch.stack((Ttc[..., :-1], Ttc[..., 1:]), dim=-1).contiguous()
        O = torch.zeros(geom.n_prob, geom.heads, geom.Mp, HEAD_DIM, device=dev, dtype=torch.float32)
        LSE = torch.full((2, geom.n_prob, geom.heads, geom.Mp), float("-inf"), device=dev, dtype=torch.float32)
        need_bwd = any(ctx.needs_input_grad)
        o = SimpleNamespace(Qe=Qe, Qp=Qp, pair=pair, Ttc=Ttc, O=O, LSE=LSE, drop=ctx.drop or ())
        saved = []
        for i, sg in enumerate(segs):
            g = dc_replace(geom, N=sg.n1 - sg.n0)
            Ke = torch.empty(g.n_prob, g.heads, g.Np, HEAD_DIM, device=dev, dtype=ed)
            Ve = torch.empty_like(Ke)
            Vt = torch.empty(g.n_prob, g.heads, HEAD_DIM, g.Np, device=dev, dtype=ed)
            Kt = torch.empty_like(Vt) if need_bwd else None
            kn2 = None
            if fused:
                nb, Hi, Wi, Cc = feat.shape
                if route.kn2 and sg.kind == "region":
                    kn2 = torch.zeros(g.n_prob, g.heads, device=dev, dtype=torch.float32)
                _launch("bevr_kv_project", _ptr(feat), int(feat.dtype == torch.bfloat16),
                        C.c_void_p(spos.data_ptr() + sg.n0 * 8), N, _ptr(W_e), _ptr(b_f), nb, Hi, Wi, Cc, g.N, g.Np, g.heads, c,
                        g.precision, _ptr(Ke), _ptr(Ve), _ptr(Kt), _ptr(Vt), _ptr(vn2) if need_bwd else None, _ptr(kn2),
                        g.groups, _stream(), flops=0.0,
                        nbytes=float(feat.numel() * feat.element_size() + 8 * nb * g.N + (4 if need_bwd else 3) * Ke.numel() * 2))
            else:
                kp = kv.data_ptr() + sg.n0 * C2 * 4
                _launch("bevr_pack_kv", C.c_void_p(kp), C.c_void_p(kp + 2 * C2), C2, N, g.n_prob, g.N, g.Np, g.heads, c,
                        g.precision, _ptr(Ke), _ptr(Ve), _ptr(Kt), _ptr(Vt), _stream())
            ka = F.pad(key_a[:, sg.n0:sg.n1], (0, g.Np - g.N)).contiguous()
            kb = F.pad(key_b[:, sg.n0:sg.n1], (0, g.Np - g.N)).contiguous()
            d = g.desc()
            key_ws = torch.empty(L.bevr_attn_key_ws_bytes(C.byref(d)), device=dev, dtype=torch.uint8)
            _launch("bevr_attn_key_prep", C.byref(d), _ptr(ka), _ptr(kb), _ptr(key_ws), _stream())
            krows = None if fused else kv[:, sg.n0:sg.n1, :C2 // 2]
            o.__dict__.update(g=g, desc=d, Ke=Ke, Ve=Ve, Vt=Vt, key_ws=key_ws, kn2=kn2, krows=krows, chained=i > 0)
            _run(sg.fwd, o)
            saved += [Ke, Ve, Kt, ka, kb, key_ws]
        ctx.geom = geom
        ctx.vmax = kv[..., C2 // 2:].reshape(kv.shape[0], N, geom.heads, c).norm(dim=-1).max() if x3 and need_bwd else None
        ctx.segs = segs
        ctx.kv_shape = (geom.n_prob, N, C2)
        ctx.fused = fused
        if fused:
            ctx.n_seg_saved = len(saved)
            saved += [feat, spos, Wkv, vn2] + ([bkv] if bkv is not None else [])
            ctx.has_bias = bkv is not None
        ctx.save_for_backward(Qe, pair, O, LSE, *saved)
        ctx.set_materialize_grads(False)
        return O, LSE[0].clone()

    @staticmethod
    def backward(ctx, dO, dLSE=None):
        geom: AttnGeom = ctx.geom
        Qe, pair, O, LSE, *saved = ctx.saved_tensors
        if ctx.fused:
            src = saved[ctx.n_seg_saved:]
            saved = saved[:ctx.n_seg_saved]
        ed = _edtype(geom.precision)
        if dO is None:
            dO = torch.zeros_like(O)
        dO = dO.contiguous()
        f16 = geom.precision == _lib.PREC_F16
        if f16:
            sdo = torch.exp2(torch.floor(10.0 - torch.log2(dO.abs().max().clamp_min(1e-30))))
        x3 = geom.precision == _lib.PREC_BF16X3
        dev = dO.device
        prep = geom.precision in (_lib.PREC_BF16, _lib.PREC_F16) and dO.dtype == torch.float32 and O.dtype == torch.float32
        if prep:
            dOe = torch.empty(O.shape, device=dev, dtype=ed)
            dOt_p = torch.empty(geom.n_prob, geom.heads, HEAD_DIM, geom.Mp, device=dev, dtype=ed)
            delta = torch.empty(geom.n_prob, geom.heads, geom.Mp, device=dev, dtype=torch.float32)
            pstats = torch.zeros(2, device=dev, dtype=torch.float32)
            dl_in = dLSE.float().contiguous() if dLSE is not None else None
            lse0 = LSE[0].contiguous() if dLSE is not None else None
            _launch("bevr_attn_bwd_prep", _ptr(dO), _ptr(O), _ptr(sdo) if f16 else None, _ptr(dl_in), _ptr(lse0), _ptr(dOe),
                    _ptr(dOt_p), _ptr(delta), _ptr(pstats), geom.n_prob * geom.heads, geom.Mp, geom.precision, _stream())
            dOr = None
        else:
            if f16:
                dO = dO * sdo
            dOe = _split_rows(dO.float()) if x3 else dO.to(ed).contiguous()
            dOr = dO.float() if x3 else dOe.float()
            delta = (dOr * O).sum(-1)
            if dLSE is not None:
                dl = torch.where(torch.isfinite(LSE[0]), dLSE.float(), torch.zeros_like(delta)) * LOG2E
                delta = delta - (dl * sdo if f16 else dl)
            delta = delta.contiguous()
        dQ = torch.zeros(geom.n_prob, geom.heads, geom.Mp, HEAD_DIM, device=dev, dtype=torch.float32)
        dT = torch.zeros(geom.heads, geom.Wp, geom.Hp + 1, device=dev, dtype=torch.float32)
        Qt = _split_perm_t(_unsplit_rows(Qe)) if x3 else _perm_t(Qe)
        dOt = dOt_p if prep else (_split_perm_t(dOr) if x3 else _perm_t(dOe))
        N, C2 = ctx.kv_shape[1], ctx.kv_shape[-1]
        dkv = torch.empty(ctx.kv_shape, device=dev, dtype=torch.float32)
        if ctx.fused:
            vmax = src[3][0].sqrt() * 1.01
        elif x3:
            vmax = ctx.vmax
        else:
            vmax = torch.stack([saved[6 * i + 1].float().norm(dim=-1).max() for i in range(len(ctx.segs))]).max()
        if prep:
            bound = (pstats[0].sqrt() * vmax + pstats[1]).clamp_min(1e-30)
        else:
            bound = (dOr.norm(dim=-1).max() * vmax + delta.abs().max()).clamp_min(1e-30)
        pmax_log2 = (LSE[1].max() + 0.05).clamp(-60.0, 0.0)
        gscale = backward_scales(bound, pmax_log2, f16, ctx.drop[0] if ctx.drop else 0)
        o = SimpleNamespace(Qe=Qe, Qt=Qt, pair=pair, dOe=dOe, dOt=dOt, LSE=LSE, delta=delta, gscale=gscale, dQ=dQ, dT=dT,
                            drop=ctx.drop or ())
        das, dbs = [], []
        for i, sg in enumerate(ctx.segs):
            g = dc_replace(geom, N=sg.n1 - sg.n0)
            o.Ke, o.Ve, o.Kt, o.ka, o.kb, o.key_ws = saved[6 * i:6 * i + 6]
            o.g, o.desc = g, g.desc()
            _run(sg.bwd_q, o)
            o.dK = torch.empty(g.n_prob, g.heads, g.Np, HEAD_DIM, device=dev, dtype=torch.float32)
            o.dV = torch.empty_like(o.dK)
            o.da, o.db = torch.zeros_like(o.ka), torch.zeros_like(o.kb)
            _run(sg.bwd_k, o)
            kp = dkv.data_ptr() + sg.n0 * C2 * 4
            _launch("bevr_unpack_dkv", _ptr(o.dK), _ptr(o.dV), C.c_void_p(kp), C.c_void_p(kp + 2 * C2), C2, N, g.n_prob,
                    g.N, g.Np, g.heads, C2 // 2 // g.heads, _stream())
            das.append(o.da[:, :g.N])
            dbs.append(o.db[:, :g.N])
        if geom.q_div > 1:
            dQ = dQ.reshape(geom.n_prob // geom.q_div, geom.q_div, geom.heads, geom.Mp, HEAD_DIM).sum(1)
        da = das[0] if len(das) == 1 else torch.cat(das, 1)
        db = dbs[0] if len(dbs) == 1 else torch.cat(dbs, 1)
        if f16:
            inv = 1.0 / sdo
            dQ, dkv, da, db, dT = dQ * inv, dkv * inv, da * inv, db * inv, dT * inv
        if not ctx.fused:
            return dQ, dkv, da, db, dT, None, None, None, None, None, None, None
        dfeat, dspos, dW, dbias = _kv_source_adjoint(dkv, src[0], src[1], src[2], geom.groups, ctx.needs_input_grad[7],
                                                     ctx.needs_input_grad[9], ctx.has_bias and ctx.needs_input_grad[10])
        return dQ, None, da, db, dT, None, None, dfeat, dspos, dW, dbias, None


def attention_core(query: torch.Tensor, kproj: Optional[torch.Tensor], vproj: Optional[torch.Tensor], pos: torch.Tensor,
                   rpe_table: torch.Tensor, *, heads: int, groups: int, views: int, precision: int,
                   kv: Optional[torch.Tensor] = None, cell_split: Optional[int] = None, kv_source=None,
                   tap_source=None, attn_drop=None, concat_views: bool = False, tap_pix=None) -> torch.Tensor:
    B, Cc, S, _ = query.shape
    drop = None
    if attn_drop is not None and attn_drop[0] > 0.0:
        thr = int(round(float(attn_drop[0]) * 65536.0))
        if not 0 < thr < 65536:
            raise ValueError("attention dropout probability must lie in (0, 1)")
        drop = (thr, int(attn_drop[1]) & 0xFFFFFFFF)
    if kv_source is not None:
        if kv is not None or kproj is not None or vproj is not None:
            raise ValueError("pass kv_source alone")
        source, (feat, Wkv, bkv) = "kv_source", kv_source
        Bp, N = feat.shape[0], pos.shape[1]
        if pos.shape[0] != Bp * groups or feat.shape[-1] != Cc or tuple(Wkv.shape) != (2 * Cc, Cc):
            raise ValueError("kv_source shapes: feat (B*views, Hi, Wi, C), pos (B*views*groups, N, 2), Wkv (2C, C)")
    else:
        if kv is None:
            kv = torch.cat((kproj, vproj), -1)
        elif kproj is not None or vproj is not None:
            raise ValueError("pass either kproj and vproj, or kv")
        Bp, N, C2 = kv.shape
        if C2 != 2 * Cc:
            raise ValueError(f"K | V rows must have 2 x {Cc} channels, got {C2}")
        source = "kv" if tap_pix is None else "tap_pix"
        if tap_pix is not None:
            if not tap_source or cell_split is None or N != int(cell_split) or pos.shape[0] != Bp:
                raise ValueError("tap_pix needs tap_source, cell_split and the projected rows of the keys [0, cell_split) alone")
            N = pos.shape[1]
            feat, Wkv, bkv = tap_pix
            if feat.shape[0] != Bp or feat.shape[-1] != Cc or tuple(Wkv.shape) != (2 * Cc, Cc):
                raise ValueError("tap_pix shapes: feat (B*views, Hi, Wi, C), Wkv (2C, C), bkv (2C,)")
    Wt = rpe_table.shape[-1]
    if rpe_table.shape[-2] != 2 * S - 1:
        raise ValueError("rpe_table height must be 2S-1")

    def keys_in_tap_grid(split):
        ky = (pos[:, split:, 0].float() + 1.0) * (0.5 * (feat.shape[1] - 1))
        kx = (pos[:, split:, 1].float() + 1.0) * (0.5 * (feat.shape[2] - 1))
        return bool(((ky < TAP_R - 1) & (kx < TAP_C - 1)).all())
    route = attention_route(precision, groups, S, Wt, N, cell_split, tap_source, drop is not None, source, Cc, heads,
                            keys_in_tap_grid)
    c = Cc // heads
    n = route.n_core
    geom = AttnGeom(n_prob=Bp, q_div=views, heads=heads, groups=groups, S=S, N=n, Wt=Wt, precision=precision)
    Qp = pack_query(query.float(), heads)
    a, b = key_coords(pos.float(), S, Wt, N)
    Tt = pack_table(rpe_table.float(), geom)
    O_r = LSE_r = None
    if n > 0:
        a_r, b_r = (a, b) if n == N else (a[:, :n], b[:, :n])
        if source == "kv_source":
            spos = pos.float() if n == N else pos[:, :n].float().contiguous()
            O_r, LSE_r = _AttnCore.apply(Qp, None, a_r, b_r, Tt, geom, route, feat, spos, Wkv, bkv, drop)
        else:
            O_r, LSE_r = _AttnCore.apply(Qp, kv.float(), a_r, b_r, Tt, geom, route, None, None, None, None, drop)
    if not route.tap:
        return _unpacked(O_r, S, c, views, concat_views)

    V = views
    Hi, Wi = feat.shape[1], feat.shape[2]
    fpix = feat[:, :TAP_R, :TAP_C, :].float()
    fpix = F.pad(fpix, (0, 0, 0, TAP_C - fpix.shape[2], 0, TAP_R - fpix.shape[1])).reshape(Bp, TAP_N, Cc)
    kvp = F.linear(fpix, Wkv.float())
    pad_c = HEAD_DIM - c
    Kp = F.pad(kvp[..., :Cc].reshape(B, V, TAP_N, heads, c), (0, pad_c)).permute(0, 3, 4, 1, 2).reshape(B, heads, HEAD_DIM, V * TAP_N)
    G = torch.matmul(Qp, Kp).reshape(B, heads, geom.Mp, V, TAP_N).permute(0, 3, 1, 2, 4).reshape(Bp, heads, geom.Mp, TAP_N)
    Gb = torch.matmul(Qp[..., :c], bkv[:Cc].float().reshape(heads, c, 1)).squeeze(-1)
    key_y = (pos[:, n:, 0].float() + 1.0) * (0.5 * (Hi - 1))
    key_x = (pos[:, n:, 1].float() + 1.0) * (0.5 * (Wi - 1))
    Rn, *mass, LSE_c = _TapAttn.apply(G, a[:, n:], b[:, n:], key_y, key_x, Tt, dc_replace(geom, N=N - n), route.segments[-1],
                                      drop and (drop[0], drop[1], n))
    LSE_c = (LSE_c.reshape(B, V, heads, geom.Mp) + Gb[:, None]).reshape(Bp, heads, geom.Mp)
    Vp = F.pad(kvp[..., Cc:].reshape(Bp, TAP_N, heads, c), (0, pad_c)).permute(0, 2, 1, 3)
    bv = F.pad(bkv[Cc:].float().reshape(1, heads, 1, c), (0, pad_c))
    if route.merge == "merge_tap":
        return merge_tap(O_r, LSE_r, Rn, LSE_c, Vp, bv.reshape(heads, HEAD_DIM), S, c, views if concat_views else 1)
    O_c = torch.matmul(Rn, Vp) + (mass[0][..., None] * bv if mass else bv)
    if O_r is None:
        return _unpacked(O_c, S, c, views, concat_views)
    return _unpacked(O_r, S, c, views, concat_views, LSE_r, O_c, LSE_c)


def _unpacked(O, S, c, views, concat_views, L_r=None, O_c=None, L_c=None):
    return merge_views(O, S, c, views if concat_views else 1, L_r, O_c, L_c)


TAP_R, TAP_C, TAP_N, TAP_SLOTS = 4, 3, 12, 16
TAP_HEADROOM = 64.0
TAP_HEADROOM_F16 = 8.0


TAP_X3_DEFAULT = "0"


def tap_headroom(precision: int) -> float:
    return TAP_HEADROOM_F16 if precision == _lib.PREC_F16 else TAP_HEADROOM
LN2 = 0.6931471805599453


def _neg_big(ed):
    return -1.0e30 if ed == torch.bfloat16 else -30000.0


def _set_offset(op: torch.Tensor, c: torch.Tensor, x3: bool = False) -> torch.Tensor:
    dst = [(op[0], 12), (op[1], 12), (op[0], 13), (op[1], 13)] if x3 else [(op, 12), (op, 13)]
    r, parts = c.float(), []
    for t, slot in dst:
        p = r.to(op.dtype)
        t[..., slot] = p
        parts.append(p.float())
        r = r - p.float()
    total = parts.pop()
    while parts:
        total = total + parts.pop()
    return total


def _tap_operand(rows: torch.Tensor, x3: bool, ed=torch.bfloat16, dead: float = 0.0, slot15=None):
    rows = rows.float()
    shape = tuple(rows.shape[:-1]) + (TAP_SLOTS,)
    if x3:
        op = torch.zeros((2,) + shape, device=rows.device, dtype=torch.bfloat16)
        hi = rows.to(torch.bfloat16)
        op[0][..., :TAP_N] = hi
        op[1][..., :TAP_N] = (rows - hi.float()).to(torch.bfloat16)
        main = op[0]
    else:
        main = op = torch.zeros(shape, device=rows.device, dtype=ed)
        op[..., :TAP_N] = rows
    main[..., 14] = dead
    if slot15 is not None:
        main[..., 15] = slot15
    return op, (op[0][..., :TAP_N].float() + op[1][..., :TAP_N].float() if x3 else op[..., :TAP_N].float())


def tap_split_rows(rows: torch.Tensor, c: Optional[torch.Tensor] = None, dead: float = 0.0):
    planes, _ = _tap_operand(rows, True, dead=dead)
    return planes, None if c is None else _set_offset(planes, c, True)


class _TapAttn(torch.autograd.Function):

    @staticmethod
    def forward(ctx, G, key_a, key_b, key_y, key_x, Tt, geom: AttnGeom, seg: KeySegment, drop=None):
        _require_gpu(G, key_a, key_b, key_y, key_x, Tt)
        L = _lib.lib()
        ed = _edtype(geom.precision)
        dev = G.device
        P, h, Mp = geom.n_prob, geom.heads, geom.Mp
        d = geom.desc()
        pad = geom.Np - geom.N
        ka, kb, ky, kx = (F.pad(t.float(), (0, pad)).contiguous() for t in (key_a, key_b, key_y, key_x))
        ws = torch.empty(L.bevr_attn_tap_ws_bytes(C.byref(d)), device=dev, dtype=torch.uint8)
        _launch("bevr_attn_tap_prep", C.byref(d), _ptr(ka), _ptr(kb), _ptr(ky), _ptr(kx), _ptr(ws), _stream())
        Ttc = Tt.contiguous()
        pair = torch.stack((Ttc[..., :-1], Ttc[..., 1:]), dim=-1).contiguous()
        x3 = geom.precision == _lib.PREC_BF16X3
        tmax = Ttc.amax(-1).amax(-1).clamp_min(0.0)
        G16, Gv = _tap_operand(G, x3, ed, _neg_big(torch.bfloat16 if x3 else ed))
        ub = 1.01 * ((G.float() if x3 else Gv).amax(-1).clamp_min(0.0) + tmax[None, :, None]) + 0.01
        mref = (-_set_offset(G16, tap_headroom(geom.precision) - ub, x3)).contiguous()
        R = torch.zeros(P, h, Mp, TAP_SLOTS, device=dev, dtype=torch.float32)
        flags = torch.zeros(P * h, geom.S, device=dev, dtype=torch.int32)
        ctx.drop = drop if drop and drop[0] > 0 else None
        valid = (torch.arange(Mp, device=dev) % geom.Sp) < geom.S
        lsum = torch.zeros(P, h, Mp, device=dev, dtype=torch.float32) if ctx.drop else None
        thr, seed, key0 = ctx.drop or (0, 0, 0)
        _run(seg.fwd, SimpleNamespace(g=geom, desc=d, G16=G16, ws=ws, pair=pair, mref=mref, R=R, flags=flags,
                                      lsum=(_ptr(lsum),) if ctx.drop else (), drop=(key0, thr, seed) if ctx.drop else ()))
        l = torch.where(valid, lsum if ctx.drop else R[..., 15], torch.ones_like(mref))
        LSE = torch.where(valid, mref + torch.log2(l), torch.zeros_like(mref))
        if ctx.drop:
            sc = torch.where(valid, (65536.0 / (65536.0 - thr)) / l, torch.zeros_like(l))
            outs = (R[..., :TAP_N] * sc[..., None], R[..., 15] * sc, LSE)
        else:
            outs = (torch.where(valid[:, None], R[..., :TAP_N] / l[..., None], torch.zeros_like(R[..., :TAP_N])), LSE)
        ctx.geom, ctx.seg = geom, seg
        ctx.save_for_backward(G16, outs[0], LSE, ws, pair, Ttc, *outs[1:-1])
        ctx.set_materialize_grads(False)
        return outs

    @staticmethod
    def backward(ctx, dRn, *rest):
        geom: AttnGeom = ctx.geom
        drop = ctx.drop
        dmass, dLSE = rest if drop else (None, rest[0])
        G16, Rn, LSE, ws, pair, Ttc, *mass = ctx.saved_tensors
        Dk = 65536.0 / (65536.0 - drop[0]) if drop else 1.0
        ed = G16.dtype
        dev = G16.device
        P, h, Mp = geom.n_prob, geom.heads, geom.Mp
        valid = (torch.arange(Mp, device=dev) % geom.Sp) < geom.S
        x3 = geom.precision == _lib.PREC_BF16X3
        sdo = None
        if ed == torch.float16:
            big = torch.zeros((), device=dev)
            for t in (dRn, dLSE, dmass):
                if t is not None:
                    big = torch.maximum(big, t.abs().max())
            sdo = torch.exp2(torch.floor(8.0 - torch.log2(big.clamp_min(1e-30))) - math.ceil(math.log2(Dk)))
            dRn, dLSE, dmass = (None if t is None else t * sdo for t in (dRn, dLSE, dmass))
        H16, Hv = _tap_operand(torch.zeros_like(Rn) if dRn is None else dRn * (LN2 * Dk), x3, ed,
                               slot15=None if dmass is None else dmass * (LN2 * Dk))
        delta = (Rn * Hv).sum(-1)
        if drop:
            delta = (delta + mass[0] * H16[..., 15].float()) / Dk
        if dLSE is not None:
            delta = delta - dLSE
        _set_offset(H16, -delta, x3)
        Gq = G16.clone()
        _set_offset(Gq, torch.where(valid, -LSE, torch.full_like(LSE, _neg_big(ed))), x3)
        dG = torch.zeros(P, h, Mp, TAP_SLOTS, device=dev, dtype=torch.float32)
        dT = torch.zeros_like(Ttc)
        dk = [torch.zeros(P, geom.Np, device=dev, dtype=torch.float32) for _ in range(4)]
        o = SimpleNamespace(g=geom, desc=geom.desc(), Gq=Gq, H16=H16, ws=ws, pair=pair, Ttc=Ttc, dG=dG, dT=dT, dk=dk,
                            drop=(drop[2], drop[0], drop[1]) if drop else ())
        _run(ctx.seg.bwd_q, o)
        _run(ctx.seg.bwd_k, o)
        da, db, dy, dx = (t[:, :geom.N] for t in dk)
        dGo = dG[..., :TAP_N] * valid[:, None]
        if sdo is not None:
            inv = 1.0 / sdo
            dGo, da, db, dy, dx, dT = dGo * inv, da * inv, db * inv, dy * inv, dx * inv, dT * inv
        return dGo, da, db, dy, dx, dT, None, None, None


def tap_supported(precision: int, groups: int, dropout: bool = False) -> bool:
    if groups != 1 or os.environ.get("BEVR_TAP", "1") == "0":
        return False
    if precision == _lib.PREC_BF16X3:
        return not dropout and os.environ.get("BEVR_TAP_X3", TAP_X3_DEFAULT) != "0"
    return precision in (_lib.PREC_BF16, _lib.PREC_F16)


def kv_source_supported(C: int, heads: int, groups: int, precision: int) -> bool:
    return (groups >= 1 and C % groups == 0 and (C // groups) % 4 == 0 and precision in (_lib.PREC_BF16, _lib.PREC_F16)
            and C % 16 == 0 and C <= 256 and C % heads == 0 and C // heads <= 32
            and os.environ.get("BEVR_FUSED_KV", "1") != "0")


class _Sample(torch.autograd.Function):

    @staticmethod
    def forward(ctx, feat, pos):
        _require_gpu(feat, pos)
        feat, pos = feat.contiguous(), pos.contiguous()
        out = _Sample.sample(feat, pos)
        ctx.save_for_backward(feat, pos)
        return out

    @staticmethod
    def backward(ctx, dout):
        feat, pos = ctx.saved_tensors
        return _Sample.scatter(feat, pos, dout, ctx.needs_input_grad[0])

    @staticmethod
    def sample(feat, pos):
        nb, Hi, Wi, Cc = feat.shape
        N = pos.shape[1]
        out = torch.empty(nb, N, Cc, device=feat.device, dtype=torch.float32)
        bf = feat.dtype == torch.bfloat16
        _launch("bevr_sample_fwd" + ("_bf16" if bf else ""), _ptr(feat), _ptr(pos), _ptr(out), nb, Hi, Wi, Cc, N, _stream(),
                flops=0.0, nbytes=4.0 * nb * (Hi * Wi * Cc * (0.5 if bf else 1.0) + N * Cc + 2 * N),
                timer="bevr_sample_fwd", label="bevr_sample_fwd")
        return out

    @staticmethod
    def scatter(feat, pos, dout, need_dfeat=True):
        nb, Hi, Wi, Cc = feat.shape
        N = pos.shape[1]
        dout = dout.contiguous()
        bf = feat.dtype == torch.bfloat16
        dfeat = torch.zeros(feat.shape, device=feat.device, dtype=torch.float32)
        dpos = torch.empty_like(pos)
        _launch("bevr_sample_bwd" + ("_bf16" if bf else ""), _ptr(feat), _ptr(pos), _ptr(dout), _ptr(dfeat), _ptr(dpos), nb, Hi,
                Wi, Cc, N, _stream(), flops=0.0, nbytes=4.0 * nb * (N * Cc + (1.5 if bf else 2.0) * Hi * Wi * Cc + 4 * N),
                timer="bevr_sample_bwd", label="bevr_sample_bwd")
        return (dfeat.to(feat.dtype) if bf and need_dfeat else dfeat if not bf else None), dpos


def sample_features(feat_nchw: torch.Tensor, pos: torch.Tensor, groups: int) -> torch.Tensor:
    B, Cc, Hi, Wi = feat_nchw.shape
    g = groups
    N = pos.shape[1]
    f = feat_nchw if feat_nchw.dtype == torch.bfloat16 else feat_nchw.float()
    f = f.reshape(B, g, Cc // g, Hi, Wi).permute(0, 1, 3, 4, 2).reshape(B * g, Hi, Wi, Cc // g)
    xs = _Sample.apply(f.contiguous(), pos.float())
    return xs.reshape(B, g, N, Cc // g).permute(0, 2, 1, 3).reshape(B, N, Cc)


def project_bev_grid(points_3d: torch.Tensor, cam_inv: torch.Tensor, Kmat: torch.Tensor, img_w: int,
                     img_h: int, gray_ref: Optional[torch.Tensor] = None) -> torch.Tensor:
    _require_gpu(points_3d, cam_inv, Kmat, gray_ref)
    pts = points_3d.float().contiguous()
    ci, km = cam_inv.float().contiguous(), Kmat.float().contiguous()
    ncam, P = ci.shape[0], pts.shape[1]
    out = torch.empty(ncam, 2, P, device=pts.device, dtype=torch.float32)
    if gray_ref is None:
        _launch("bevr_project_bev_grid", _ptr(pts), _ptr(ci), _ptr(km), _ptr(out), ncam, P, img_w, img_h, _stream())
        return out
    if gray_ref.dtype != torch.uint8 or gray_ref.dim() != 4 or gray_ref.shape[0] != ncam:
        raise ValueError("gray_ref must be a (ncam, C, H, W) uint8 tensor")
    ref = gray_ref.contiguous()
    _launch("bevr_project_bev_grid_masked", _ptr(pts), _ptr(ci), _ptr(km), _ptr(out), ncam, P, img_w, img_h, _ptr(ref),
            ref.shape[1], ref.shape[2], ref.shape[3], _stream())
    return out


class _Corr(torch.autograd.Function):

    @staticmethod
    def forward(ctx, cam, mp, normalize: bool):
        _require_gpu(cam, mp)
        ctx.summed = cam is mp and ctx.needs_input_grad[0] and ctx.needs_input_grad[1]
        alias = cam is mp
        cam = cam.float().contiguous()
        if cam.data_ptr() % 16:
            cam = cam.clone()
        mp = cam if alias else mp.float().contiguous()
        if mp.data_ptr() % 16:
            mp = mp.clone()
        n, E = cam.shape
        m = mp.shape[0]
        D = torch.empty(n, m, device=cam.device, dtype=torch.float32)
        inc = torch.empty(n, device=cam.device, dtype=torch.float32)
        inm = torch.empty(m, device=cam.device, dtype=torch.float32)
        same = cam.data_ptr() == mp.data_ptr() and n == m
        _launch("bevr_corr_fwd", _ptr(cam), _ptr(mp), _ptr(D), _ptr(inc), _ptr(inm), n, m, E, int(normalize), _stream(),
                flops=0.0, nbytes=4.0 * E * (n if same else n + m))
        ctx.normalize = normalize
        ctx.save_for_backward(cam, mp, D, inc, inm)
        return D

    @staticmethod
    def backward(ctx, dD):
        cam, mp, D, inc, inm = ctx.saved_tensors
        n, E = cam.shape
        m = mp.shape[0]
        same = cam.data_ptr() == mp.data_ptr() and n == m
        if same and not ctx.summed:
            mp, same = mp.clone(), False
        dcam = torch.empty_like(cam)
        dmap = dcam if same else torch.empty_like(mp)
        _launch("bevr_corr_bwd", _ptr(cam), _ptr(mp), _ptr(D), _ptr(dD.contiguous()), _ptr(inc), _ptr(inm), _ptr(dcam),
                _ptr(dmap), n, m, E, int(ctx.normalize), _stream(), flops=0.0,
                nbytes=4.0 * E * (2 * n if same else 2 * (n + m)))
        return (dcam, None, None) if ctx.summed else (dcam, dmap, None)


def pairwise_corr(cam: torch.Tensor, mp: torch.Tensor, normalize: bool = False) -> torch.Tensor:
    return _Corr.apply(cam, mp, normalize)


def recall_rank(D: torch.Tensor) -> torch.Tensor:
    _require_gpu(D)
    D = D.float().contiguous()
    n = D.shape[0]
    rank = torch.empty(n, device=D.device, dtype=torch.int32)
    _launch("bevr_recall_rank", _ptr(D), _ptr(rank), n, _stream())
    return rank


def offset_head_supported(cg: int, mx: int, dout: int) -> bool:
    return cg <= 64 and ((mx == dout and 1 <= mx <= 8) or (mx == 1 and dout == 2))


class _OffsetHead(torch.autograd.Function):
    @staticmethod
    def forward(ctx, x, w0, b0, gamma, beta, W3, groups, eps):
        _require_gpu(x, gamma, beta, W3)
        x = x.float().contiguous()
        B, H, W, Cc = x.shape
        g = groups
        cg = Cc // g
        K = gamma.numel()
        mx, dout = K // cg, W3.shape[0]
        prm = [None if t is None else t.detach().float().contiguous() for t in (w0, b0, gamma, beta, W3)]
        P = B * H * W
        out = torch.empty(g, B, H, W, dout, device=x.device, dtype=torch.float32)
        for gi in range(g):
            xp = C.c_void_p(x.data_ptr() + gi * cg * 4)
            _launch("bevr_offset_head_fwd", xp, _ptr(prm[0]), _ptr(prm[1]), _ptr(prm[2]), _ptr(prm[3]), _ptr(prm[4]),
                    _ptr(out[gi]), P, cg, Cc, mx, dout, float(eps), _stream())
        ctx.save_for_backward(x, *[t for t in prm if t is not None])
        ctx.meta = (g, cg, mx, dout, float(eps), w0 is not None, b0 is not None)
        return out.permute(1, 0, 2, 3, 4).reshape(B * g, H, W, dout)

    @staticmethod
    def backward(ctx, dout_):
        g, cg, mx, dout, eps, has_w0, has_b0 = ctx.meta
        saved = list(ctx.saved_tensors)
        x = saved.pop(0)
        w0 = saved.pop(0) if has_w0 else None
        b0 = saved.pop(0) if has_b0 else None
        gamma, beta, W3 = saved
        B, H, W, Cc = x.shape
        P = B * H * W
        do = dout_.float().reshape(B, g, H, W, dout).permute(1, 0, 2, 3, 4).contiguous()
        dx = torch.zeros_like(x) if ctx.needs_input_grad[0] else None
        dw0 = torch.zeros_like(w0) if has_w0 else None
        db0 = torch.zeros_like(b0) if has_b0 else None
        dga, dbe, dW3 = torch.zeros_like(gamma), torch.zeros_like(beta), torch.zeros_like(W3)
        for gi in range(g):
            xp = C.c_void_p(x.data_ptr() + gi * cg * 4)
            dxp = None if dx is None else C.c_void_p(dx.data_ptr() + gi * cg * 4)
            _launch("bevr_offset_head_bwd", xp, _ptr(w0), _ptr(b0), _ptr(gamma), _ptr(beta), _ptr(W3), _ptr(do[gi]), dxp,
                    _ptr(dw0), _ptr(db0), _ptr(dga), _ptr(dbe), _ptr(dW3), P, cg, Cc, mx, dout, eps, _stream())
        return dx, dw0, db0, dga, dbe, dW3, None, None


def offset_head(x: torch.Tensor, w0, b0, gamma: torch.Tensor, beta: torch.Tensor, W3: torch.Tensor, groups: int = 1,
                eps: float = 1e-5) -> torch.Tensor:
    return _OffsetHead.apply(x, w0, b0, gamma, beta, W3, groups, eps)


class _LayerNorm(torch.autograd.Function):

    @staticmethod
    def forward(ctx, x, gamma, beta, eps):
        _require_gpu(x, gamma, beta)
        x = x.float().contiguous()
        Cc = x.shape[-1]
        rows = x.numel() // Cc
        gamma, beta = gamma.float().contiguous(), beta.float().contiguous()
        y = torch.empty_like(x)
        mean = torch.empty(rows, device=x.device, dtype=torch.float32)
        rstd = torch.empty_like(mean)
        _launch("bevr_layernorm_fwd", _ptr(x), _ptr(gamma), _ptr(beta), _ptr(y), _ptr(mean), _ptr(rstd), rows, Cc,
                float(eps), _stream())
        ctx.save_for_backward(x, gamma, mean, rstd)
        return y

    @staticmethod
    def backward(ctx, dy):
        x, gamma, mean, rstd = ctx.saved_tensors
        Cc = x.shape[-1]
        dy = dy.float().contiguous()
        dx = torch.empty_like(x)
        dg = torch.zeros(Cc, device=x.device, dtype=torch.float32)
        db = torch.zeros_like(dg)
        _launch("bevr_layernorm_bwd", _ptr(x), _ptr(gamma), _ptr(dy), _ptr(mean), _ptr(rstd), _ptr(dx), _ptr(dg), _ptr(db),
                x.numel() // Cc, Cc, _stream())
        return dx, dg, db, None


def layer_norm_supported(C: int) -> bool:
    c4 = C // 4
    return C % 4 == 0 and 0 < c4 <= 64 and (c4 & (c4 - 1)) == 0


def layer_norm(x: torch.Tensor, gamma: torch.Tensor, beta: torch.Tensor, eps: float = 1e-5) -> torch.Tensor:
    return _LayerNorm.apply(x, gamma, beta, eps)


class _KeyPositions(torch.autograd.Function):

    @staticmethod
    def forward(ctx, off, ref, order, B, G, sca_SD, use_tanh, sy, sx):
        _require_gpu(off, ref, order)
        off, ref = off.float().contiguous(), ref.float().contiguous()
        V, P = off.shape[0], off.shape[1]
        N = ref.shape[1]
        S, D = sca_SD if sca_SD else (0, 0)
        order = None if order is None else order.to(torch.int32).contiguous()
        pos = torch.empty(B, V, G, N, 2, device=off.device, dtype=torch.float32)
        ctx.args = (V, P, G, N, 1 if sca_SD else 0, S, D, 1 if use_tanh else 0, float(sy), float(sx))
        _launch("bevr_key_positions_fwd", _ptr(off), _ptr(ref), _ptr(order), _ptr(pos), *ctx.args, _stream())
        ctx.save_for_backward(off, ref, order)
        return pos

    @staticmethod
    def backward(ctx, dpos):
        off, ref, order = ctx.saved_tensors
        doff = torch.empty_like(off)
        _launch("bevr_key_positions_bwd", _ptr(off), _ptr(ref), _ptr(order), _ptr(dpos.float().contiguous()), _ptr(doff),
                *ctx.args, _stream())
        return doff, None, None, None, None, None, None, None, None


def key_positions(off: torch.Tensor, ref: torch.Tensor, order: Optional[torch.Tensor], batch: int, groups: int,
                  sca_SD=None, use_tanh: bool = True, sy: float = 1.0, sx: float = 1.0) -> torch.Tensor:
    return _KeyPositions.apply(off, ref, order, batch, groups, sca_SD, use_tanh, sy, sx)


class _AffineWarp(torch.autograd.Function):
    @staticmethod
    def forward(ctx, img, theta):
        _require_gpu(img, theta)
        img, theta = img.float().contiguous(), theta.float().contiguous()
        B, Cc, H, W = img.shape
        out = torch.empty_like(img)
        _launch("bevr_affine_warp_fwd", _ptr(img), _ptr(theta), _ptr(out), B, Cc, H, W, _stream())
        ctx.save_for_backward(theta)
        return out

    @staticmethod
    def backward(ctx, dout):
        (theta,) = ctx.saved_tensors
        dout = dout.float().contiguous()
        B, Cc, H, W = dout.shape
        dimg = torch.zeros_like(dout)
        _launch("bevr_affine_warp_bwd", _ptr(dout), _ptr(theta), _ptr(dimg), B, Cc, H, W, _stream())
        return dimg, None


def affine_theta(angle_rad: torch.Tensor, translate_xy: torch.Tensor) -> torch.Tensor:
    c, s = torch.cos(angle_rad), torch.sin(angle_rad)
    tx, ty = translate_xy[:, 0], translate_xy[:, 1]
    return torch.stack((c, s, -c * tx - s * ty, -s, c, s * tx - c * ty), 1).float()


def affine_warp(img: torch.Tensor, angle_rad: torch.Tensor, translate_xy: torch.Tensor) -> torch.Tensor:
    return _AffineWarp.apply(img, affine_theta(angle_rad.to(img.device), translate_xy.to(img.device)))


class _DwConv(torch.autograd.Function):
    @staticmethod
    def forward(ctx, x, weight, bias, nhwc: bool):
        _require_gpu(x, weight)
        x = x.contiguous()
        w = weight.contiguous()
        if nhwc:
            B, H, W, Cc = x.shape
        else:
            B, Cc, H, W = x.shape
        k = w.shape[-1]
        y = torch.empty_like(x)
        _launch("bevr_dwconv_fwd", _ptr(x), _ptr(w), _ptr(bias.contiguous()) if bias is not None else None, _ptr(y), B, H,
                W, Cc, k, int(nhwc), 0, _stream())
        ctx.save_for_backward(x, w)
        ctx.meta = (B, H, W, Cc, k, nhwc, bias is not None)
        return y

    @staticmethod
    def backward(ctx, dy):
        x, w = ctx.saved_tensors
        B, H, W, Cc, k, nhwc, has_bias = ctx.meta
        dy = dy.contiguous()
        dx = dw = db = None
        if ctx.needs_input_grad[0]:
            dx = torch.empty_like(x)
            _launch("bevr_dwconv_fwd", _ptr(dy), _ptr(w), None, _ptr(dx), B, H, W, Cc, k, int(nhwc), 1, _stream(),
                    label="bevr_dwconv_fwd(flip)")
        if ctx.needs_input_grad[1] or (has_bias and ctx.needs_input_grad[2]):
            dw = torch.zeros_like(w)
            db = torch.zeros(Cc, device=x.device, dtype=x.dtype) if has_bias else None
            _launch("bevr_dwconv_bwd_w", _ptr(x), _ptr(dy), _ptr(dw), _ptr(db) if db is not None else None, B, H, W, Cc, k,
                    int(nhwc), _stream())
        return dx, dw, db, None


class _DwResGelu(torch.autograd.Function):

    @staticmethod
    def forward(ctx, x, weight, bias):
        _require_gpu(x, weight)
        x, w = x.contiguous(), weight.contiguous()
        b = bias.contiguous() if bias is not None else None
        B, H, W, Cc = x.shape
        y = torch.empty_like(x)
        _launch("bevr_dwconv_res_gelu", _ptr(x), _ptr(w), _ptr(b), None, _ptr(y), B, H, W, Cc, 3, 1, _stream(),
                label="bevr_dwconv_res_gelu(1)")
        ctx.save_for_backward(x, w, b)
        return y

    @staticmethod
    def backward(ctx, dout):
        x, w, b = ctx.saved_tensors
        B, H, W, Cc = x.shape
        dout = dout.contiguous()
        g = torch.empty_like(x)
        _launch("bevr_dwconv_res_gelu", _ptr(x), _ptr(w), _ptr(b), _ptr(dout), _ptr(g), B, H, W, Cc, 3, 2, _stream(),
                label="bevr_dwconv_res_gelu(2)")
        dx = dw = db = None
        if ctx.needs_input_grad[0]:
            dx = torch.empty_like(x)
            _launch("bevr_dwconv_res_gelu", _ptr(g), _ptr(w), None, None, _ptr(dx), B, H, W, Cc, 3, 3, _stream(),
                    label="bevr_dwconv_res_gelu(3)")
        if ctx.needs_input_grad[1] or (b is not None and ctx.needs_input_grad[2]):
            dw = torch.zeros_like(w)
            db = torch.zeros(Cc, device=x.device, dtype=x.dtype) if b is not None else None
            _launch("bevr_dwconv_bwd_w", _ptr(x), _ptr(g), _ptr(dw), _ptr(db), B, H, W, Cc, 3, 1, _stream())
        return dx, dw, db


def dwconv_res_gelu_supported(x: torch.Tensor, weight: torch.Tensor) -> bool:
    return (x.is_cuda and x.dtype == torch.float32 and x.dim() == 4 and x.shape[-1] % 4 == 0 and weight.shape[-1] == 3
            and weight.shape[-2] == 3 and weight.shape[1] == 1 and weight.shape[0] == x.shape[-1]
            and os.environ.get("BEVR_FUSED_MLP", "1") != "0")


def dwconv_res_gelu(x: torch.Tensor, weight: torch.Tensor, bias) -> torch.Tensor:
    return _DwResGelu.apply(x, weight, bias)


def depthwise_conv(x: torch.Tensor, weight: torch.Tensor, bias, nhwc: bool) -> torch.Tensor:
    return _DwConv.apply(x, weight, bias, nhwc)
```

### include/bevrender_hip.h

```cpp
#ifndef BEVRENDER_HIP_H
#define BEVRENDER_HIP_H

#include <stddef.h>
#include <stdint.h>

#ifdef __cplusplus
extern "C" {
#endif

#define BEVR_ABI_VERSION 6

enum {
  BEVR_OK = 0,
  BEVR_E_NULL = -1,
  BEVR_E_SHAPE = -2,
  BEVR_E_PRECISION = -3,
  BEVR_E_ALIGN = -4
};

enum { BEVR_PREC_F32 = 0, BEVR_PREC_BF16 = 1, BEVR_PREC_F16 = 2, BEVR_PREC_BF16X3 = 3 };

int bevr_abi_version(void);
const char* bevr_strerror(int code);

typedef struct bevr_attn_desc {
  int32_t n_prob;
  int32_t q_div;
  int32_t heads;
  int32_t groups;
  int32_t S;
  int32_t Sp;
  int32_t N;
  int32_t Np;
  int32_t Ht, Wt;
  int32_t Hp, Wp;
  int32_t y_off, x_off;
  int32_t precision;
  int32_t reserved;
} bevr_attn_desc;

int bevr_attn_table_dims(bevr_attn_desc* d);

size_t bevr_attn_key_ws_bytes(const bevr_attn_desc* d);
int bevr_attn_key_prep(const bevr_attn_desc* d, const float* key_a, const float* key_b, void* key_ws, void* stream);

int bevr_attn_fwd(const bevr_attn_desc* d, const void* Q, const void* K, const void* Vt,
                  const void* key_ws, const float* table_pair,
                  float* O, float* LSE, void* stream);

int bevr_attn_bwd_q(const bevr_attn_desc* d, const void* Q, const void* K, const void* Kt, const void* V,
                    const void* key_ws, const float* table_pair,
                    const void* dO, const float* LSE, const float* delta, const float* grad_scale,
                    float* dQ, float* dtable, void* stream);

int bevr_attn_bwd_k(const bevr_attn_desc* d, const void* Q, const void* Qt, const void* K, const void* V,
                    const float* key_a, const float* key_b, const float* table_pair,
                    const void* dO, const void* dOt, const float* LSE, const float* delta, const float* grad_scale,
                    float* dK, float* dV, float* dkey_a, float* dkey_b, void* stream);

int bevr_attn_fwd_dropout(const bevr_attn_desc* d, const void* Q, const void* K, const void* Vt,
                          const void* key_ws, const float* table_pair, float* O, float* LSE,
                          unsigned drop_thr, unsigned drop_seed, void* stream);
int bevr_attn_bwd_q_dropout(const bevr_attn_desc* d, const void* Q, const void* K, const void* Kt, const void* V,
                            const void* key_ws, const float* table_pair, const void* dO, const float* LSE,
                            const float* delta, const float* grad_scale, float* dQ, float* dtable,
                            unsigned drop_thr, unsigned drop_seed, void* stream);
int bevr_attn_bwd_k_dropout(const bevr_attn_desc* d, const void* Q, const void* Qt, const void* K, const void* V,
                            const float* key_a, const float* key_b, const float* table_pair, const void* dO,
                            const void* dOt, const float* LSE, const float* delta, const float* grad_scale,
                            float* dK, float* dV, float* dkey_a, float* dkey_b, unsigned drop_thr, unsigned drop_seed,
                            void* stream);

int bevr_attn_cell_fwd(const bevr_attn_desc* d, const void* Q, const void* K, const void* Vt,
                       const void* key_ws, const float* table_pair, const float* O_in, const float* LSE_in,
                       float* O, float* LSE, void* stream);
int bevr_attn_cell_bwd_q(const bevr_attn_desc* d, const void* Q, const void* K, const void* Kt, const void* V,
                         const void* key_ws, const float* table_pair, const void* dO, const float* LSE,
                         const float* delta, const float* grad_scale, float* dQ, float* dtable, void* stream);
int bevr_attn_cell_bwd_k(const bevr_attn_desc* d, const void* Q, const void* Qt, const void* K, const void* V,
                         const void* key_ws, const float* table_pair, const void* dO, const void* dOt,
                         const float* LSE, const float* delta, const float* grad_scale, float* dK, float* dV,
                         float* dkey_a, float* dkey_b, void* stream);

size_t bevr_attn_tap_ws_bytes(const bevr_attn_desc* d);
int bevr_attn_tap_prep(const bevr_attn_desc* d, const float* key_a, const float* key_b, const float* key_y,
                       const float* key_x, void* tap_ws, void* stream);
int bevr_attn_tap_fwd(const bevr_attn_desc* d, const void* G, const void* tap_ws, const float* table_pair, float* mref,
                      float* R, int32_t* flags, void* stream);
int bevr_attn_tap_bwd_q(const bevr_attn_desc* d, const void* G, const void* H, const void* tap_ws,
                        const float* table_pair, float* dG, float* dtable, void* stream);
int bevr_attn_tap_bwd_k(const bevr_attn_desc* d, const void* G, const void* H, const void* tap_ws,
                        const float* table, float* dkey_a, float* dkey_b, float* dkey_y, float* dkey_x, void* stream);

int bevr_attn_tap_fwd_dropout(const bevr_attn_desc* d, const void* G, const void* tap_ws, const float* table_pair,
                              float* mref, float* R, float* lsum, int32_t* flags, unsigned key0, unsigned drop_thr,
                              unsigned drop_seed, void* stream);
int bevr_attn_tap_bwd_q_dropout(const bevr_attn_desc* d, const void* G, const void* H, const void* tap_ws,
                                const float* table_pair, float* dG, float* dtable, unsigned key0, unsigned drop_thr,
                                unsigned drop_seed, void* stream);
int bevr_attn_tap_bwd_k_dropout(const bevr_attn_desc* d, const void* G, const void* H, const void* tap_ws,
                                const float* table, float* dkey_a, float* dkey_b, float* dkey_y, float* dkey_x,
                                unsigned key0, unsigned drop_thr, unsigned drop_seed, void* stream);

int bevr_attn_gather_fwd(const bevr_attn_desc* d, const void* Q, const void* K, const void* V,
                         const void* key_ws, const void* table_pk, const float* mref, float* O, float* LSE,
                         int* flags, void* stream);
int bevr_attn_gather_fwd_rows(const bevr_attn_desc* d, const void* Q, const void* K, const void* V,
                              const void* key_ws, const void* table_pk, const float* mref, float* O, float* LSE,
                              int* flags, int row0, int n_rows, void* stream);
int bevr_attn_gather_fwd_x3(const bevr_attn_desc* d, const void* Q, const void* K, const void* V,
                            const void* key_ws, const void* table_pk2, const float* mref, float* O, float* LSE,
                            int* flags, int row0, int n_rows, void* stream);

size_t bevr_attn_slab_ws_bytes(const bevr_attn_desc* d);
int bevr_attn_slab_prep(const bevr_attn_desc* d, const float* key_a, const float* key_b, const int32_t* order,
                        void* slab_ws, void* stream);
int bevr_attn_slab_bwd_q(const bevr_attn_desc* d, const void* Q, const void* Ks, const void* Vs, const void* slab_ws,
                         const float* table_pair, const void* dO, const float* LSE, const float* delta,
                         const float* grad_scale, float* dQ, float* dtable, void* stream);
size_t bevr_attn_slab_rows_ws_bytes(const bevr_attn_desc* d);
int bevr_attn_slab_rows_prep(const bevr_attn_desc* d, const float* key_a, const float* key_b, const int32_t* order,
                             void* slab_ws, void* stream);
int bevr_attn_slab_bwd_q_rows(const bevr_attn_desc* d, const void* Q, const void* Ks, const void* Vs, const void* slab_ws,
                              const float* table_pair, const void* dO, const float* LSE, const float* delta,
                              const float* grad_scale, float* dQ, float* dtable, int row0, int n_rows, void* stream);

int bevr_sample_fwd(const float* feat, const float* pos, float* out,
                    int nb, int Hi, int Wi, int C, int N, void* stream);
int bevr_sample_bwd(const float* feat, const float* pos, const float* dout, float* dfeat, float* dpos,
                    int nb, int Hi, int Wi, int C, int N, void* stream);
int bevr_sample_fwd_bf16(const void* feat, const float* pos, float* out,
                         int nb, int Hi, int Wi, int C, int N, void* stream);
int bevr_sample_bwd_bf16(const void* feat, const float* pos, const float* dout, float* dfeat, float* dpos,
                         int nb, int Hi, int Wi, int C, int N, void* stream);

int bevr_project_bev_grid(const float* points_3d, const float* cam_inv, const float* Kmat, float* out,
                          int ncam, int P, int img_w, int img_h, void* stream);
int bevr_project_bev_grid_masked(const float* points_3d, const float* cam_inv, const float* Kmat, float* out,
                                 int ncam, int P, int img_w, int img_h, const uint8_t* ref_img, int ref_c,
                                 int ref_h, int ref_w, void* stream);

int bevr_corr_fwd(const float* cam, const float* map, float* D, float* inv_norm_cam, float* inv_norm_map,
                  int n, int m, int E, int normalize, void* stream);
int bevr_corr_bwd(const float* cam, const float* map, const float* D, const float* dD,
                  const float* inv_norm_cam, const float* inv_norm_map, float* dcam, float* dmap,
                  int n, int m, int E, int normalize, void* stream);
int bevr_recall_rank(const float* D, int32_t* rank, int n, void* stream);

int bevr_dwconv_fwd(const float* x, const float* w, const float* bias, float* y,
                    int B, int H, int W, int C, int k, int nhwc, int flip, void* stream);
int bevr_dwconv_bwd_w(const float* x, const float* dy, float* dw, float* dbias,
                      int B, int H, int W, int C, int k, int nhwc, void* stream);
int bevr_dwconv_res_gelu(const float* x, const float* w, const float* bias, const float* aux, float* y, int B, int H, int W,
                         int C, int k, int mode, void* stream);

int bevr_pack_kv(const float* k, const float* v, long long ld, long long pstride, int n_prob, int N, int Np, int heads,
                 int c, int precision, void* Kr, void* Vr, void* Kt, void* Vt, void* stream);
int bevr_unpack_dkv(const float* dK, const float* dV, float* dk, float* dv, long long ld, long long pstride, int n_prob,
                    int N, int Np, int heads, int c, void* stream);

int bevr_layernorm_fwd(const float* x, const float* gamma, const float* beta, float* y, float* mean, float* rstd,
                       long long rows, int C, float eps, void* stream);
int bevr_layernorm_bwd(const float* x, const float* gamma, const float* dy, const float* mean, const float* rstd,
                       float* dx, float* dgamma, float* dbeta, long long rows, int C, void* stream);

int bevr_merge_views_fwd(const float* O_r, const float* L_r, const float* O_c, const float* L_c, float* out, int n_prob,
                         int views, int heads, int S, int Sp, int c, void* stream);
int bevr_merge_views_bwd(const float* dout, const float* O_r, const float* L_r, const float* O_c, const float* L_c,
                         float* dO_r, float* dL_r, float* dO_c, float* dL_c, int n_prob, int views, int heads, int S,
                         int Sp, int c, void* stream);
int bevr_merge_tap_fwd(const float* O_r, const float* L_r, const float* Rn, const float* L_c, const float* Vp, const float* bv,
                       float* out, int n_prob, int views, int heads, int S, int Sp, int c, void* stream);
int bevr_merge_tap_bwd(const float* dout, const float* O_r, const float* L_r, const float* Rn, const float* L_c, const float* Vp,
                       const float* bv, float* dO_r, float* dL_r, float* dRn, float* dL_c, float* dVp, float* dbv, int n_prob,
                       int views, int heads, int S, int Sp, int c, void* stream);

int bevr_attn_bwd_prep(const float* dO, const float* O, const float* scale, const float* dLSE, const float* LSE0, void* dOe,
                       void* dOt, float* delta, float* stats, int n_ph, int Mp, int precision, void* stream);

int bevr_kv_project(const void* feat, int feat_bf16, const float* pos, long long pos_pstride, const void* Wkv,
                    const float* bkv, int nb, int Hi, int Wi, int C, int N, int Np, int heads, int c, int precision,
                    void* Kr, void* Vr, void* Kt, void* Vt, float* vnorm2_max, float* knorm2_max, int groups,
                    void* stream);

int bevr_key_positions_fwd(const float* off, const float* ref, const int* order, float* pos, int V, int P, int G, int N,
                           int sca, int S, int D, int use_tanh, float sy, float sx, void* stream);
int bevr_key_positions_bwd(const float* off, const float* ref, const int* order, const float* dpos, float* doff, int V,
                           int P, int G, int N, int sca, int S, int D, int use_tanh, float sy, float sx, void* stream);

int bevr_offset_head_fwd(const float* x, const float* w0, const float* b0, const float* gamma, const float* beta,
                         const float* W3, float* out, long long P, int Cg, int xstride, int Mx, int Dout, float eps,
                         void* stream);
int bevr_offset_head_bwd(const float* x, const float* w0, const float* b0, const float* gamma, const float* beta,
                         const float* W3, const float* dout, float* dx, float* dw0, float* db0, float* dgamma,
                         float* dbeta, float* dW3, long long P, int Cg, int xstride, int Mx, int Dout, float eps,
                         void* stream);

int bevr_affine_warp_fwd(const float* img, const float* theta, float* out, int B, int C, int H, int W, void* stream);
int bevr_affine_warp_bwd(const float* dout, const float* theta, float* dimg, int B, int C, int H, int W, void* stream);

#ifdef __cplusplus
}
#endif
#endif
```

Before: 5.795 samples/s.

## Compact slow key blocks into a worklist for persistent gather bwd_k kernel

The windowed bwd_k kernel now appends the (problem-head, key-block) units it cannot handle with the slab path to a device-side list via an atomic counter. A persistent gather kernel, sized to resident occupancy, then processes only the listed units, splitting the query range by a cost model instead of launching a full grid where most workgroups exit early. The same scheme is applied to the tap bwd_k path, enabled by default through an environment switch. It adds a memset, a per-call workspace allocation and atomics, and output ordering now depends on the list.

```diff
diff --git a/bevrender_amd/_lib.py b/bevrender_amd/_lib.py
--- a/bevrender_amd/_lib.py
+++ b/bevrender_amd/_lib.py
@@ -19,6 +19,7 @@
     "bevr_attn_fwd", "bevr_attn_bwd_q",
     "bevr_attn_bwd_k", "bevr_attn_fwd_dropout", "bevr_attn_bwd_q_dropout", "bevr_attn_bwd_k_dropout", "bevr_attn_cell_fwd", "bevr_attn_cell_bwd_q", "bevr_attn_cell_bwd_k", "bevr_attn_tap_ws_bytes", "bevr_attn_tap_prep", "bevr_attn_tap_fwd", "bevr_attn_tap_bwd_q", "bevr_attn_tap_bwd_k", "bevr_attn_tap_fwd_dropout", "bevr_attn_tap_bwd_q_dropout", "bevr_attn_tap_bwd_k_dropout", "bevr_attn_gather_fwd", "bevr_attn_gather_fwd_rows", "bevr_attn_gather_fwd_x3", "bevr_attn_slab_ws_bytes", "bevr_attn_slab_prep", "bevr_attn_slab_bwd_q", "bevr_attn_slab_rows_ws_bytes", "bevr_attn_slab_rows_prep", "bevr_attn_slab_bwd_q_rows", "bevr_sample_fwd", "bevr_sample_bwd", "bevr_sample_fwd_bf16", "bevr_sample_bwd_bf16", "bevr_project_bev_grid", "bevr_project_bev_grid_masked", "bevr_corr_fwd",
     "bevr_corr_bwd", "bevr_recall_rank", "bevr_dwconv_fwd", "bevr_dwconv_bwd_w", "bevr_dwconv_res_gelu", "bevr_affine_warp_fwd", "bevr_affine_warp_bwd",
+    "bevr_attn_bwd_k_ws_bytes", "bevr_attn_bwd_k_ws", "bevr_attn_tap_bwd_k_ws_bytes", "bevr_attn_tap_bwd_k_ws",
     "bevr_offset_head_fwd", "bevr_offset_head_bwd", "bevr_key_positions_fwd", "bevr_key_positions_bwd", "bevr_kv_project", "bevr_layernorm_fwd", "bevr_layernorm_bwd", "bevr_merge_views_fwd", "bevr_merge_views_bwd", "bevr_merge_tap_fwd", "bevr_merge_tap_bwd", "bevr_attn_bwd_prep", "bevr_pack_kv", "bevr_unpack_dkv",
 ]
 
@@ -71,6 +72,10 @@
         L.bevr_attn_fwd.argtypes = [dp, vp, vp, vp, vp, fp, fp, fp, vp]
         L.bevr_attn_bwd_q.argtypes = [dp] + [vp] * 4 + [vp, fp] + [vp, fp, fp, fp, fp, fp, vp]
         L.bevr_attn_bwd_k.argtypes = [dp] + [vp] * 4 + [fp] * 3 + [vp, vp, fp, fp, fp] + [fp] * 4 + [vp]
+        L.bevr_attn_bwd_k_ws_bytes.argtypes = [dp]
+        L.bevr_attn_bwd_k_ws.argtypes = [dp] + [vp] * 4 + [fp] * 3 + [vp, vp, fp, fp, fp] + [fp] * 4 + [vp, ip, vp]
+        L.bevr_attn_tap_bwd_k_ws_bytes.argtypes = [dp]
+        L.bevr_attn_tap_bwd_k_ws.argtypes = [dp, vp, vp, vp, fp, fp, fp, fp, fp, vp, ip, vp]
         u32 = C.c_uint32
         L.bevr_attn_fwd_dropout.argtypes = [dp, vp, vp, vp, vp, fp, fp, fp, u32, u32, vp]
         L.bevr_attn_bwd_q_dropout.argtypes = [dp] + [vp] * 4 + [vp, fp] + [vp, fp, fp, fp, fp, fp, u32, u32, vp]
@@ -126,7 +131,7 @@
         for name in SYMBOLS:
             fn = getattr(L, name)
             if name in ("bevr_attn_key_ws_bytes", "bevr_attn_tap_ws_bytes", "bevr_attn_slab_ws_bytes",
-                        "bevr_attn_slab_rows_ws_bytes"):
+                        "bevr_attn_slab_rows_ws_bytes", "bevr_attn_bwd_k_ws_bytes", "bevr_attn_tap_bwd_k_ws_bytes"):
                 fn.restype = C.c_size_t
             elif name not in ("bevr_strerror",):
                 fn.restype = C.c_int
diff --git a/bevrender_amd/csrc/attn_bwd_k.hip b/bevrender_amd/csrc/attn_bwd_k.hip
--- a/bevrender_amd/csrc/attn_bwd_k.hip
+++ b/bevrender_amd/csrc/attn_bwd_k.hip
@@ -7,6 +7,7 @@
 namespace {
 
 constexpr int KEYS_WG = 384;
+constexpr int LIST_HEAD = 4;
 
 struct KBox { int amin, amax; float bmin, bmax; };
 
@@ -66,7 +67,8 @@
     const char* __restrict__ V, const float* __restrict__ key_a, const float* __restrict__ key_b,
     const char* __restrict__ table_pair, const char* __restrict__ dO, const char* __restrict__ dOt,
     const float* __restrict__ LSE, const float* __restrict__ delta, const float* __restrict__ grad_scale,
-    float* __restrict__ dK, float* __restrict__ dV, float* __restrict__ dkey_a, float* __restrict__ dkey_b BEVR_DROP_PARAMS) {
+    float* __restrict__ dK, float* __restrict__ dV, float* __restrict__ dkey_a, float* __restrict__ dkey_b,
+    int* __restrict__ slow_list BEVR_DROP_PARAMS) {
   constexpr int NT = is16(PREC) ? 2 : 1;
   const float kp16 = PREC == BEVR_PREC_F16 ? grad_scale[2] : 0.f, c2_16 = PREC == BEVR_PREC_F16 ? grad_scale[3] : 1.f;
   const float ds_inv = PREC == BEVR_PREC_F16 ? grad_scale[4] : 1.f, p_inv = PREC == BEVR_PREC_F16 ? grad_scale[5] : 1.f;
@@ -130,6 +132,7 @@
         *reinterpret_cast<f32x4*>(vr + 8 * g4 + 4 * hi) = z;
       }
     }
+    if (slow_list && tid == 0) slow_list[LIST_HEAD + atomicAdd(slow_list, 1)] = ph * n_kb + kblk;
     return;
   }
   if (box.amax < box.amin) {
@@ -405,28 +408,21 @@
 constexpr int TG = 256;
 constexpr int KW = 3;
 constexpr int GSPLIT = 4;
-
-template <int PREC>
-__global__ __launch_bounds__(TG) void attn_bwd_k_gather_kernel(
-    bevr_attn_desc d, const char* __restrict__ Q, const char* __restrict__ Qt, const char* __restrict__ K,
+constexpr int GATHER_MIN_TILES = 32;
+constexpr int GATHER_ITEM_TILES = 4;
+
+template <int PREC, bool FULL_GRID>
+__device__ __forceinline__ void gather_sweep(
+    const bevr_attn_desc& d, const char* __restrict__ Q, const char* __restrict__ Qt, const char* __restrict__ K,
     const char* __restrict__ V, const float* __restrict__ key_a, const float* __restrict__ key_b,
     const char* __restrict__ table_pair, const char* __restrict__ dO, const char* __restrict__ dOt,
     const float* __restrict__ LSE, const float* __restrict__ delta, const float* __restrict__ grad_scale,
-    float* __restrict__ dK, float* __restrict__ dV, float* __restrict__ dkey_a, float* __restrict__ dkey_b BEVR_DROP_PARAMS) {
+    float* __restrict__ dK, float* __restrict__ dV, float* __restrict__ dkey_a, float* __restrict__ dkey_b,
+    char* smem, KBox* red, int ph, int kblk, int it_first, int it_end BEVR_DROP_PARAMS) {
   typedef LdsK<PREC> L;
   const float kp16 = PREC == BEVR_PREC_F16 ? grad_scale[2] : 0.f, c2_16 = PREC == BEVR_PREC_F16 ? grad_scale[3] : 1.f;
   const float ds_inv = PREC == BEVR_PREC_F16 ? grad_scale[4] : 1.f, p_inv = PREC == BEVR_PREC_F16 ? grad_scale[5] : 1.f;
   constexpr int EB = L::EB;
-  __shared__ __attribute__((aligned(16))) char smem[2 * L::BUF];
-  __shared__ __attribute__((aligned(16))) KBox red[4];
-
-  const int n_kb = (d.Np + KEYS_WG - 1) / KEYS_WG;
-  const int n_ph = d.n_prob * d.heads;
-  const int xcd = blockIdx.x & 7, slot = blockIdx.x >> 3;
-  const int ph = (slot / (n_kb * GSPLIT)) * 8 + xcd;
-  if (ph >= n_ph) return;
-  const int kblk = (slot % (n_kb * GSPLIT)) / GSPLIT;
-  const int split = slot % GSPLIT;
   const int prob = ph / d.heads, hd = ph % d.heads;
   const int grp = hd / (d.heads / d.groups);
   const int qb = prob / d.q_div;
@@ -454,8 +450,7 @@
     key_idx[w] = key;
     kc[w] = make_keyc(ka[key], kb[key], d);
   }
-  KBox box;
-  {
+  if constexpr (FULL_GRID) {
     int a_lo = 0x7fffffff, a_hi = (int)0x80000000;
     float b_lo = 3.0e38f, b_hi = -3.0e38f;
 #pragma unroll
@@ -468,9 +463,9 @@
         b_lo = fminf(b_lo, bc); b_hi = fmaxf(b_hi, bc);
       }
     }
-    box = wg_key_box(a_lo, a_hi, b_lo, b_hi, red, TG / 64, wave, lane);
-  }
-  if (make_slab(box, d, L::WCAP, ceilf(rx)).fits) return;
+    const KBox box = wg_key_box(a_lo, a_hi, b_lo, b_hi, red, TG / 64, wave, lane);
+    if (make_slab(box, d, L::WCAP, ceilf(rx)).fits) return;
+  }
 
   Frag<PREC> kf[KW], vf[KW];
 #pragma unroll
@@ -492,9 +487,7 @@
   qs.init(tid, Q + ((size_t)(qb * d.heads + hd) * Mp) * 32 * EB, dO + ((size_t)ph * Mp) * 32 * EB,
           Qt + ((size_t)(qb * d.heads + hd) * 32) * Mp * EB, dOt + ((size_t)ph * 32) * Mp * EB,
           LSE + (size_t)ph * Mp, delta + (size_t)ph * Mp, Mp, kp16);
-  const int n_all = d.S * n_rb;
-  const int chunk = (n_all + GSPLIT - 1) / GSPLIT;
-  const int it_first = split * chunk, n_it = min(n_all, it_first + chunk);
+  const int n_it = it_end;
   if (it_first >= n_it) return;
   qs.load(tid, (size_t)(it_first / n_rb) * d.Sp + (it_first % n_rb) * 32);
   qs.store(tid, smem);
@@ -602,38 +595,107 @@
 }
 
 template <int PREC>
+__global__ __launch_bounds__(TG) void attn_bwd_k_gather_kernel(
+    bevr_attn_desc d, const char* __restrict__ Q, const char* __restrict__ Qt, const char* __restrict__ K,
+    const char* __restrict__ V, const float* __restrict__ key_a, const float* __restrict__ key_b,
+    const char* __restrict__ table_pair, const char* __restrict__ dO, const char* __restrict__ dOt,
+    const float* __restrict__ LSE, const float* __restrict__ delta, const float* __restrict__ grad_scale,
+    float* __restrict__ dK, float* __restrict__ dV, float* __restrict__ dkey_a, float* __restrict__ dkey_b BEVR_DROP_PARAMS) {
+  __shared__ __attribute__((aligned(16))) char smem[2 * LdsK<PREC>::BUF];
+  __shared__ __attribute__((aligned(16))) KBox red[TG / 64];
+  const int n_kb = (d.Np + KEYS_WG - 1) / KEYS_WG;
+  const int xcd = blockIdx.x & 7, slot = blockIdx.x >> 3;
+  const int ph = (slot / (n_kb * GSPLIT)) * 8 + xcd;
+  if (ph >= d.n_prob * d.heads) return;
+  const int kblk = (slot % (n_kb * GSPLIT)) / GSPLIT;
+  const int split = slot % GSPLIT;
+  const int n_all = d.S * (d.Sp / 32);
+  const int chunk = (n_all + GSPLIT - 1) / GSPLIT;
+  gather_sweep<PREC, true>(d, Q, Qt, K, V, key_a, key_b, table_pair, dO, dOt, LSE, delta, grad_scale, dK, dV, dkey_a,
+                           dkey_b, smem, red, ph, kblk, split * chunk, min(n_all, (split + 1) * chunk) BEVR_DROP_ARGS);
+}
+
+#if !BEVR_DROP
+template <int PREC>
+__global__ __launch_bounds__(TG) void attn_bwd_k_gather_list_kernel(
+    bevr_attn_desc d, const char* __restrict__ Q, const char* __restrict__ Qt, const char* __restrict__ K,
+    const char* __restrict__ V, const float* __restrict__ key_a, const float* __restrict__ key_b,
+    const char* __restrict__ table_pair, const char* __restrict__ dO, const char* __restrict__ dOt,
+    const float* __restrict__ LSE, const float* __restrict__ delta, const float* __restrict__ grad_scale,
+    float* __restrict__ dK, float* __restrict__ dV, float* __restrict__ dkey_a, float* __restrict__ dkey_b,
+    const int* __restrict__ slow_list) {
+  __shared__ __attribute__((aligned(16))) char smem[2 * LdsK<PREC>::BUF];
+  const int n_list = slow_list[0];
+  if (n_list <= 0) return;
+  const int n_kb = (d.Np + KEYS_WG - 1) / KEYS_WG;
+  const int n_all = d.S * (d.Sp / 32);
+  int chunk = n_all;
+  long long best = 0x7fffffffffffffffLL;
+  for (int r = 1; r <= max(1, n_all / GATHER_MIN_TILES); ++r) {
+    const int ch = (n_all + r - 1) / r, nr = (n_all + ch - 1) / ch;
+    const long long rounds = ((long long)n_list * nr + gridDim.x - 1) / gridDim.x;
+    const long long cost = rounds * (ch + GATHER_ITEM_TILES);
+    if (cost < best) { best = cost; chunk = ch; }
+  }
+  const int n_rng = (n_all + chunk - 1) / chunk;
+  for (int item = blockIdx.x; item < n_list * n_rng; item += gridDim.x) {
+    const int unit = slow_list[LIST_HEAD + item % n_list], rng = item / n_list;
+    gather_sweep<PREC, false>(d, Q, Qt, K, V, key_a, key_b, table_pair, dO, dOt, LSE, delta, grad_scale, dK, dV, dkey_a,
+                              dkey_b, smem, nullptr, unit / n_kb, unit % n_kb, rng * chunk, min(n_all, (rng + 1) * chunk));
+  }
+}
+
+template <typename Kern>
+int resident_workgroups(Kern kern, int threads) {
+  int dev = 0, cus = 0, per_cu = 0;
+  if (hipGetDevice(&dev) != hipSuccess ||
+      hipDeviceGetAttribute(&cus, hipDeviceAttributeMultiprocessorCount, dev) != hipSuccess ||
+      hipOccupancyMaxActiveBlocksPerMultiprocessor(&per_cu, kern, threads, 0) != hipSuccess)
+    return 0;
+  return cus * per_cu;
+}
+#endif
+
+template <int PREC>
 int launch(const bevr_attn_desc& d, const void* Q, const void* Qt, const void* K, const void* V, const float* key_a,
            const float* key_b, const float* table_pair, const void* dO, const void* dOt, const float* LSE,
-           const float* delta, const float* gs, float* dK, float* dV, float* dka, float* dkb, hipStream_t st BEVR_DROP_PARAMS) {
+           const float* delta, const float* gs, float* dK, float* dV, float* dka, float* dkb, int* slow_list, int max_wg,
+           hipStream_t st BEVR_DROP_PARAMS) {
   const int n_kb = (d.Np + KEYS_WG - 1) / KEYS_WG;
   const int n_ph = d.n_prob * d.heads;
   const int grid = ((n_ph + 7) / 8) * 8 * n_kb;
+  int rc;
+  if (slow_list) {
+    if ((long long)n_ph * n_kb * (d.S * (d.Sp / 32) / GATHER_MIN_TILES + 1) > 0x7fffffffLL) return BEVR_E_SHAPE;
+    rc = (int)hipMemsetAsync(slow_list, 0, LIST_HEAD * sizeof(int), st);
+    if (rc) return rc;
+  }
   hipLaunchKernelGGL((attn_bwd_k_win_kernel<PREC>), dim3(grid), dim3(TW), 0, st, d, (const char*)Q, (const char*)Qt,
                      (const char*)K, (const char*)V, key_a, key_b, (const char*)table_pair, (const char*)dO,
-                     (const char*)dOt, LSE, delta, gs, dK, dV, dka, dkb BEVR_DROP_ARGS);
-  int rc = (int)hipGetLastError();
+                     (const char*)dOt, LSE, delta, gs, dK, dV, dka, dkb, slow_list BEVR_DROP_ARGS);
+  rc = (int)hipGetLastError();
   if (rc) return rc;
+#if !BEVR_DROP
+  if (slow_list) {
+    static const int resident = resident_workgroups(attn_bwd_k_gather_list_kernel<PREC>, TG);
+    if (resident <= 0) return (int)hipErrorInvalidDevice;
+    const int n_wg = max_wg > 0 && max_wg < resident ? max_wg : resident;
+    hipLaunchKernelGGL((attn_bwd_k_gather_list_kernel<PREC>), dim3(n_wg), dim3(TG), 0, st, d, (const char*)Q,
+                       (const char*)Qt, (const char*)K, (const char*)V, key_a, key_b, (const char*)table_pair,
+                       (const char*)dO, (const char*)dOt, LSE, delta, gs, dK, dV, dka, dkb, (const int*)slow_list);
+    return (int)hipGetLastError();
+  }
+#endif
   hipLaunchKernelGGL((attn_bwd_k_gather_kernel<PREC>), dim3(grid * GSPLIT), dim3(TG), 0, st, d, (const char*)Q,
                      (const char*)Qt, (const char*)K, (const char*)V, key_a, key_b, (const char*)table_pair,
                      (const char*)dO, (const char*)dOt, LSE, delta, gs, dK, dV, dka, dkb BEVR_DROP_ARGS);
   return (int)hipGetLastError();
 }
 
-}
-
-#if BEVR_DROP
-extern "C" int bevr_attn_bwd_k_dropout(const bevr_attn_desc* d, const void* Q, const void* Qt, const void* K, const void* V,
-                                       const float* key_a, const float* key_b, const float* table_pair, const void* dO,
-                                       const void* dOt, const float* LSE, const float* delta, const float* grad_scale,
-                                       float* dK, float* dV, float* dkey_a, float* dkey_b, unsigned drop_thr,
-                                       unsigned drop_seed, void* stream) {
-  if (drop_thr >= 65536u) return BEVR_E_SHAPE;
-#else
-extern "C" int bevr_attn_bwd_k(const bevr_attn_desc* d, const void* Q, const void* Qt, const void* K, const void* V,
-                               const float* key_a, const float* key_b, const float* table_pair, const void* dO,
-                               const void* dOt, const float* LSE, const float* delta, const float* grad_scale,
-                               float* dK, float* dV, float* dkey_a, float* dkey_b, void* stream) {
-#endif
+int run(const bevr_attn_desc* d, const void* Q, const void* Qt, const void* K, const void* V, const float* key_a,
+        const float* key_b, const float* table_pair, const void* dO, const void* dOt, const float* LSE, const float* delta,
+        const float* grad_scale, float* dK, float* dV, float* dkey_a, float* dkey_b, int* slow_list, int max_wg,
+        void* stream BEVR_DROP_PARAMS) {
   int rc = bevr_check_desc(d);
   if (rc) return rc;
   if (!Q || !Qt || !K || !V || !key_a || !key_b || !table_pair || !dO || !dOt || !LSE || !delta || !dK || !dV ||
@@ -645,13 +707,53 @@
   hipStream_t st = (hipStream_t)stream;
   if (d->precision == BEVR_PREC_BF16)
     return launch<BEVR_PREC_BF16>(*d, Q, Qt, K, V, key_a, key_b, table_pair, dO, dOt, LSE, delta, grad_scale, dK, dV,
-                                  dkey_a, dkey_b, st BEVR_DROP_ARGS);
+                                  dkey_a, dkey_b, slow_list, max_wg, st BEVR_DROP_ARGS);
   if (d->precision == BEVR_PREC_F16)
     return launch<BEVR_PREC_F16>(*d, Q, Qt, K, V, key_a, key_b, table_pair, dO, dOt, LSE, delta, grad_scale, dK, dV,
-                                 dkey_a, dkey_b, st BEVR_DROP_ARGS);
+                                 dkey_a, dkey_b, slow_list, max_wg, st BEVR_DROP_ARGS);
   if (d->precision == BEVR_PREC_BF16X3)
     return launch<BEVR_PREC_BF16X3>(*d, Q, Qt, K, V, key_a, key_b, table_pair, dO, dOt, LSE, delta, grad_scale, dK, dV,
-                               dkey_a, dkey_b, st BEVR_DROP_ARGS);
+                                    dkey_a, dkey_b, slow_list, max_wg, st BEVR_DROP_ARGS);
   return launch<BEVR_PREC_F32>(*d, Q, Qt, K, V, key_a, key_b, table_pair, dO, dOt, LSE, delta, grad_scale, dK, dV,
-                               dkey_a, dkey_b, st BEVR_DROP_ARGS);
-}
+                               dkey_a, dkey_b, slow_list, max_wg, st BEVR_DROP_ARGS);
+}
+
+}
+
+#if BEVR_DROP
+extern "C" int bevr_attn_bwd_k_dropout(const bevr_attn_desc* d, const void* Q, const void* Qt, const void* K, const void* V,
+                                       const float* key_a, const float* key_b, const float* table_pair, const void* dO,
+                                       const void* dOt, const float* LSE, const float* delta, const float* grad_scale,
+                                       float* dK, float* dV, float* dkey_a, float* dkey_b, unsigned drop_thr,
+                                       unsigned drop_seed, void* stream) {
+  if (drop_thr >= 65536u) return BEVR_E_SHAPE;
+  return run(d, Q, Qt, K, V, key_a, key_b, table_pair, dO, dOt, LSE, delta, grad_scale, dK, dV, dkey_a, dkey_b, nullptr, 0,
+             stream, drop_thr, drop_seed);
+}
+#else
+extern "C" int bevr_attn_bwd_k(const bevr_attn_desc* d, const void* Q, const void* Qt, const void* K, const void* V,
+                               const float* key_a, const float* key_b, const float* table_pair, const void* dO,
+                               const void* dOt, const float* LSE, const float* delta, const float* grad_scale,
+                               float* dK, float* dV, float* dkey_a, float* dkey_b, void* stream) {
+  return run(d, Q, Qt, K, V, key_a, key_b, table_pair, dO, dOt, LSE, delta, grad_scale, dK, dV, dkey_a, dkey_b, nullptr, 0,
+             stream);
+}
+
+extern "C" size_t bevr_attn_bwd_k_ws_bytes(const bevr_attn_desc* d) {
+  if (bevr_check_desc(d)) return 0;
+  const size_t n_kb = ((size_t)d->Np + KEYS_WG - 1) / KEYS_WG;
+  return (LIST_HEAD + (size_t)d->n_prob * d->heads * n_kb) * sizeof(int);
+}
+
+extern "C" int bevr_attn_bwd_k_ws(const bevr_attn_desc* d, const void* Q, const void* Qt, const void* K, const void* V,
+                                  const float* key_a, const float* key_b, const float* table_pair, const void* dO,
+                                  const void* dOt, const float* LSE, const float* delta, const float* grad_scale,
+                                  float* dK, float* dV, float* dkey_a, float* dkey_b, void* ws, int max_workgroups,
+                                  void* stream) {
+  if (!ws) return BEVR_E_NULL;
+  if (!bevr_aligned16(ws)) return BEVR_E_ALIGN;
+  if (max_workgroups < 0) return BEVR_E_SHAPE;
+  return run(d, Q, Qt, K, V, key_a, key_b, table_pair, dO, dOt, LSE, delta, grad_scale, dK, dV, dkey_a, dkey_b, (int*)ws,
+             max_workgroups, stream);
+}
+#endif
diff --git a/bevrender_amd/csrc/attn_tap_bwd_k.hip b/bevrender_amd/csrc/attn_tap_bwd_k.hip
--- a/bevrender_amd/csrc/attn_tap_bwd_k.hip
+++ b/bevrender_amd/csrc/attn_tap_bwd_k.hip
@@ -25,21 +25,24 @@
   return sb.amax >= sb.amin && da >= 0 && da <= NRX && box_fits(sb, jrx) && dx >= 0 && dx <= NCW - CELL_C;
 }
 
-template <int PREC, bool SLOW>
-__global__ __launch_bounds__(64 * (NKW + 1), tap_bwd_k_waves(PREC)) void attn_tap_bwd_k_kernel(
-    bevr_attn_desc d, const char* __restrict__ G, const char* __restrict__ H, const char* __restrict__ tap_ws,
+constexpr int MODE_FIT = 0, MODE_SLOW = 1, MODE_LIST = 2;
+constexpr int LIST_HEAD = 4;
+constexpr int LIST_WAVES = 4;
+constexpr int LIST_MIN_COLS = 8;
+constexpr int LIST_ITEMS_PER_WAVE = 4;
+
+template <int PREC, int MODE>
+__device__ __forceinline__ void tap_bwd_k_body(
+    const bevr_attn_desc& d, const char* __restrict__ G, const char* __restrict__ H, const char* __restrict__ tap_ws,
     const float* __restrict__ table_t, float* __restrict__ dkey_a, float* __restrict__ dkey_b,
-    float* __restrict__ dkey_y, float* __restrict__ dkey_x, int n_wg_ph TAP_DROP_PARAMS) {
+    float* __restrict__ dkey_y, float* __restrict__ dkey_x, char* smem, int ph, int wg, int tslot, int j_first, int j_end,
+    int* __restrict__ slow_list TAP_DROP_PARAMS) {
   typedef LdsKp<PREC> L;
+  constexpr bool SLOW = MODE != MODE_FIT;
   constexpr bool X3 = tap_split(PREC);
   constexpr int NP = tap_np<PREC>;
-  extern __shared__ __attribute__((aligned(16))) char smem[];
 
   const int n_ph = d.n_prob * d.heads;
-  const int xcd = blockIdx.x & 7, slot = blockIdx.x >> 3;
-  const int ph = (slot / n_wg_ph) * 8 + xcd;
-  if (ph >= n_ph) return;
-  const int wg = slot % n_wg_ph;
   const int prob = ph / d.heads, hd = ph % d.heads;
   const int tid = threadIdx.x;
   const int wave = __builtin_amdgcn_readfirstlane(tid >> 6), lane = tid & 63;
@@ -54,7 +57,7 @@
   const int NRWD = win_dwords(d.Sp);
   const int win_bytes = 4 * NCW * NRWD * 4;
   char* win_base = smem + 2 * L::BUF;
-  TapRec* stash = reinterpret_cast<TapRec*>(win_base + 3 * win_bytes) + wave * 32;
+  TapRec* stash = reinterpret_cast<TapRec*>(MODE == MODE_LIST ? smem + LIST_WAVES * 2 * L::SLAB : win_base + 3 * win_bytes) + wave * 32;
 
   int a0w = 0x7fffffff;
   float bminw = 3.0e38f;
@@ -69,7 +72,7 @@
     }
   }
   if (a0w == 0x7fffffff) { a0w = 0; bminw = 0.f; }
-  if constexpr (SLOW) {
+  if constexpr (MODE == MODE_SLOW) {
     bool unfit = false;
     for (int t = 0; t < NKW; ++t) {
       const int tile = wg * NKW + t;
@@ -81,7 +84,7 @@
     if (!__any(unfit)) return;
   }
 
-  if (wave == NKW) {
+  if (MODE != MODE_LIST && wave == NKW) {
     __builtin_amdgcn_s_setprio(3);
     const int n_quad = (NRWD + 1) / 2, n_item = NCW * n_quad;
     auto item_load = [&](int jn, int it, float (&t)[5]) {
@@ -180,7 +183,7 @@
     return;
   }
 
-  const int tile = wg * NKW + wave;
+  const int tile = wg * NKW + tslot;
   const bool have_tile = tile < n_tiles;
   const TapRec* recs = reinterpret_cast<const TapRec*>(tap_ws) + (size_t)prob * d.Np;
   const int tl = have_tile ? tile : 0;
@@ -330,7 +333,8 @@
     }
   };
 
-  for (int j = 0; j < d.S; ++j) {
+  bool any_unfit = false;
+  for (int j = j_first; j < j_end; ++j) {
     jrx = (float)j * rx;
 #if BEVR_DROP
     hcol = (uint32_t)(j * d.Sp + 4 * g) * 0x85EBCA77u;
@@ -339,6 +343,31 @@
     const int dx = x0 - (int)floorf(jrx + bminw);
     const bool fit = tile_fits(sb, jrx, a0w, bminw);
     const bool mine = have_tile && sb.amax >= sb.amin && fit != SLOW;
+    if constexpr (MODE == MODE_FIT) any_unfit = any_unfit || (have_tile && sb.amax >= sb.amin && !fit);
+    if constexpr (MODE == MODE_LIST) {
+      if (!mine) continue;
+      any_unfit = true;
+#pragma unroll
+      for (int kb = 0; kb < 2; ++kb)
+        if (g >= 2) bk[kb] = TapOp<NP>{};
+      char* wbuf = smem + wave * 2 * L::SLAB;
+      const char* Gs = G + ((size_t)ph * Mp + (size_t)j * d.Sp) * 32 + lane * 16;
+      const char* Hs = H + ((size_t)ph * Mp + (size_t)j * d.Sp) * 32 + lane * 16;
+      u32x4 gv = gload16(Gs), hv = gload16(Hs);
+      for (int s = 0; s < nslab; ++s) {
+        char* bb = wbuf + (s & 1) * L::SLAB;
+        __builtin_amdgcn_fence(__ATOMIC_ACQ_REL, "wavefront");
+        *reinterpret_cast<u32x4*>(bb + L::OFF_G + lane * 16) = gv;
+        *reinterpret_cast<u32x4*>(bb + L::OFF_H + lane * 16) = hv;
+        __builtin_amdgcn_fence(__ATOMIC_ACQ_REL, "wavefront");
+        if (s + 1 < nslab) {
+          gv = gload16(Gs + (size_t)(s + 1) * 1024);
+          hv = gload16(Hs + (size_t)(s + 1) * 1024);
+        }
+        slab(std::false_type{}, bb, 32 * s);
+      }
+      continue;
+    }
     auto chunk_coords = [&](int kb, float& tcol, float& trow) {
       const TapRec rk = stash[16 * kb + li];
       const float tx = jrx + rk.b;
@@ -391,9 +420,13 @@
       }
     }
   }
-  __syncthreads();
+  if constexpr (MODE != MODE_LIST) __syncthreads();
 
   if (!have_tile) return;
+  if (MODE == MODE_LIST && !any_unfit) return;
+  if constexpr (MODE == MODE_FIT) {
+    if (slow_list && any_unfit && lane == 0) slow_list[LIST_HEAD + atomicAdd(slow_list, 1)] = ph * n_tiles + tile;
+  }
 #pragma unroll
   for (int kb = 0; kb < 2; ++kb) {
     const TapRec rk = stash[16 * kb + li];
@@ -424,9 +457,62 @@
   }
 }
 
+template <int PREC, bool SLOW>
+__global__ __launch_bounds__(64 * (NKW + 1), tap_bwd_k_waves(PREC)) void attn_tap_bwd_k_kernel(
+    bevr_attn_desc d, const char* __restrict__ G, const char* __restrict__ H, const char* __restrict__ tap_ws,
+    const float* __restrict__ table_t, float* __restrict__ dkey_a, float* __restrict__ dkey_b,
+    float* __restrict__ dkey_y, float* __restrict__ dkey_x, int n_wg_ph, int* __restrict__ slow_list TAP_DROP_PARAMS) {
+  extern __shared__ __attribute__((aligned(16))) char smem[];
+  const int xcd = blockIdx.x & 7, slot = blockIdx.x >> 3;
+  const int ph = (slot / n_wg_ph) * 8 + xcd;
+  if (ph >= d.n_prob * d.heads) return;
+  tap_bwd_k_body<PREC, SLOW ? MODE_SLOW : MODE_FIT>(d, G, H, tap_ws, table_t, dkey_a, dkey_b, dkey_y, dkey_x, smem, ph,
+                                                    slot % n_wg_ph, __builtin_amdgcn_readfirstlane(threadIdx.x >> 6), 0,
+                                                    d.S, slow_list TAP_DROP_ARGS);
+}
+
+#if !BEVR_DROP && !BEVR_TAP_X3
+template <int PREC>
+__global__ __launch_bounds__(64 * LIST_WAVES, 3) void attn_tap_bwd_k_list_kernel(
+    bevr_attn_desc d, const char* __restrict__ G, const char* __restrict__ H, const char* __restrict__ tap_ws,
+    const float* __restrict__ table_t, float* __restrict__ dkey_a, float* __restrict__ dkey_b,
+    float* __restrict__ dkey_y, float* __restrict__ dkey_x, int* __restrict__ list) {
+  static_assert(tap_np<PREC> == 1, "the waves stage one image per operand");
+  extern __shared__ __attribute__((aligned(16))) char smem[];
+  const int n_list = __builtin_amdgcn_readfirstlane(list[0]);
+  if (n_list <= 0) return;
+  const int n_tiles = d.Np / 32;
+  const int want = (LIST_ITEMS_PER_WAVE * LIST_WAVES * (int)gridDim.x + n_list - 1) / n_list;
+  const int n_rng0 = max(1, min(want, d.S / LIST_MIN_COLS));
+  const int cols = (d.S + n_rng0 - 1) / n_rng0;
+  const int n_rng = (d.S + cols - 1) / cols;
+  const int n_item = n_list * n_rng;
+  for (;;) {
+    int item = 0;
+    if ((threadIdx.x & 63) == 0) item = atomicAdd(list + 1, 1);
+    item = __builtin_amdgcn_readfirstlane(item);
+    if (item >= n_item) return;
+    const int unit = list[LIST_HEAD + item % n_list], rng = item / n_list;
+    const int tile = unit % n_tiles;
+    tap_bwd_k_body<PREC, MODE_LIST>(d, G, H, tap_ws, table_t, dkey_a, dkey_b, dkey_y, dkey_x, smem, unit / n_tiles,
+                                    tile / NKW, tile % NKW, rng * cols, min(d.S, (rng + 1) * cols), nullptr);
+  }
+}
+
+template <typename Kern>
+int resident_workgroups(Kern kern, int threads, size_t lds) {
+  int dev = 0, cus = 0, per_cu = 0;
+  if (hipGetDevice(&dev) != hipSuccess ||
+      hipDeviceGetAttribute(&cus, hipDeviceAttributeMultiprocessorCount, dev) != hipSuccess ||
+      hipOccupancyMaxActiveBlocksPerMultiprocessor(&per_cu, kern, threads, lds) != hipSuccess)
+    return 0;
+  return cus * per_cu;
+}
+#endif
+
 template <int PREC>
 int launch(const bevr_attn_desc& d, const void* G, const void* H, const void* tap_ws, const float* table_t, float* dkey_a,
-           float* dkey_b, float* dkey_y, float* dkey_x, hipStream_t st TAP_DROP_PARAMS) {
+           float* dkey_b, float* dkey_y, float* dkey_x, int* slow_list, int max_wg, hipStream_t st TAP_DROP_PARAMS) {
   typedef LdsKp<PREC> L;
   const int n_ph = d.n_prob * d.heads;
   const int n_tiles = d.Np / 32;
@@ -435,12 +521,29 @@
   if (lds > 160 * 1024) return BEVR_E_SHAPE;
   const long long grid = (long long)((n_ph + 7) / 8) * 8 * n_wg_ph;
   if (grid > 0x7fffffffLL) return BEVR_E_SHAPE;
+  int rc;
+  if (slow_list) {
+    if ((long long)n_ph * n_tiles * (d.S / LIST_MIN_COLS + 1) > 0x7fffffffLL) return BEVR_E_SHAPE;
+    rc = (int)hipMemsetAsync(slow_list, 0, LIST_HEAD * sizeof(int), st);
+    if (rc) return rc;
+  }
   hipLaunchKernelGGL((attn_tap_bwd_k_kernel<PREC, false>), dim3((unsigned)grid), dim3(64 * (NKW + 1)), lds, st, d, (const char*)G,
-                     (const char*)H, (const char*)tap_ws, table_t, dkey_a, dkey_b, dkey_y, dkey_x, n_wg_ph TAP_DROP_ARGS);
-  const int rc = (int)hipGetLastError();
+                     (const char*)H, (const char*)tap_ws, table_t, dkey_a, dkey_b, dkey_y, dkey_x, n_wg_ph, slow_list TAP_DROP_ARGS);
+  rc = (int)hipGetLastError();
   if (rc) return rc;
+#if !BEVR_DROP && !BEVR_TAP_X3
+  if (slow_list) {
+    const size_t lds_list = LIST_WAVES * (2 * L::SLAB + 32 * sizeof(TapRec));
+    static const int resident = resident_workgroups(attn_tap_bwd_k_list_kernel<PREC>, 64 * LIST_WAVES, lds_list);
+    if (resident <= 0) return (int)hipErrorInvalidDevice;
+    const int n_wg = max_wg > 0 && max_wg < resident ? max_wg : resident;
+    hipLaunchKernelGGL((attn_tap_bwd_k_list_kernel<PREC>), dim3(n_wg), dim3(64 * LIST_WAVES), lds_list, st, d, (const char*)G,
+                       (const char*)H, (const char*)tap_ws, table_t, dkey_a, dkey_b, dkey_y, dkey_x, slow_list);
+    return (int)hipGetLastError();
+  }
+#endif
   hipLaunchKernelGGL((attn_tap_bwd_k_kernel<PREC, true>), dim3((unsigned)grid), dim3(64 * (NKW + 1)), lds, st, d, (const char*)G,
-                     (const char*)H, (const char*)tap_ws, table_t, dkey_a, dkey_b, dkey_y, dkey_x, n_wg_ph TAP_DROP_ARGS);
+                     (const char*)H, (const char*)tap_ws, table_t, dkey_a, dkey_b, dkey_y, dkey_x, n_wg_ph, (int*)nullptr TAP_DROP_ARGS);
   return (int)hipGetLastError();
 }
 
@@ -449,31 +552,57 @@
 #if BEVR_TAP_X3
 int bevr_tap_bwd_k_x3(const bevr_attn_desc& d, const void* G, const void* H, const void* tap_ws, const float* table_t,
                       float* dkey_a, float* dkey_b, float* dkey_y, float* dkey_x, hipStream_t st) {
-  return launch<BEVR_PREC_BF16X3>(d, G, H, tap_ws, table_t, dkey_a, dkey_b, dkey_y, dkey_x, st);
+  return launch<BEVR_PREC_BF16X3>(d, G, H, tap_ws, table_t, dkey_a, dkey_b, dkey_y, dkey_x, nullptr, 0, st);
 }
 #else
+namespace {
+int run(const bevr_attn_desc* d, const void* G, const void* H, const void* tap_ws, const float* table_t, float* dkey_a,
+        float* dkey_b, float* dkey_y, float* dkey_x, int* slow_list, int max_wg, void* stream TAP_DROP_PARAMS) {
+  int rc = bevr_check_desc(d);
+  if (rc) return rc;
+  if (!G || !H || !tap_ws || !table_t || !dkey_a || !dkey_b || !dkey_y || !dkey_x) return BEVR_E_NULL;
+  if (d->groups != 1) return BEVR_E_SHAPE;
+  if (!bevr_aligned16(G) || !bevr_aligned16(H) || !bevr_aligned16(tap_ws)) return BEVR_E_ALIGN;
+  hipStream_t st = (hipStream_t)stream;
+  if (d->precision == BEVR_PREC_BF16)
+    return launch<BEVR_PREC_BF16>(*d, G, H, tap_ws, table_t, dkey_a, dkey_b, dkey_y, dkey_x, slow_list, max_wg, st TAP_DROP_ARGS);
+  if (d->precision == BEVR_PREC_F16)
+    return launch<BEVR_PREC_F16>(*d, G, H, tap_ws, table_t, dkey_a, dkey_b, dkey_y, dkey_x, slow_list, max_wg, st TAP_DROP_ARGS);
+#if !BEVR_DROP
+  if (d->precision == BEVR_PREC_BF16X3 && !slow_list)
+    return bevr_tap_bwd_k_x3(*d, G, H, tap_ws, table_t, dkey_a, dkey_b, dkey_y, dkey_x, st);
+#endif
+  return BEVR_E_PRECISION;
+}
+}
+
 #if BEVR_DROP
 extern "C" int bevr_attn_tap_bwd_k_dropout(const bevr_attn_desc* d, const void* G, const void* H, const void* tap_ws,
                                            const float* table_t, float* dkey_a, float* dkey_b, float* dkey_y,
                                            float* dkey_x, unsigned key0, unsigned drop_thr, unsigned drop_seed,
                                            void* stream) {
   if (drop_thr >= 65536u) return BEVR_E_SHAPE;
+  return run(d, G, H, tap_ws, table_t, dkey_a, dkey_b, dkey_y, dkey_x, nullptr, 0, stream, key0, drop_thr, drop_seed);
+}
 #else
 extern "C" int bevr_attn_tap_bwd_k(const bevr_attn_desc* d, const void* G, const void* H, const void* tap_ws,
                                    const float* table_t, float* dkey_a, float* dkey_b, float* dkey_y, float* dkey_x,
                                    void* stream) {
-#endif
-  int rc = bevr_check_desc(d);
-  if (rc) return rc;
-  if (!G || !H || !tap_ws || !table_t || !dkey_a || !dkey_b || !dkey_y || !dkey_x) return BEVR_E_NULL;
-  if (d->groups != 1) return BEVR_E_SHAPE;
-  if (!bevr_aligned16(G) || !bevr_aligned16(H) || !bevr_aligned16(tap_ws)) return BEVR_E_ALIGN;
-  hipStream_t st = (hipStream_t)stream;
-  if (d->precision == BEVR_PREC_BF16) return launch<BEVR_PREC_BF16>(*d, G, H, tap_ws, table_t, dkey_a, dkey_b, dkey_y, dkey_x, st TAP_DROP_ARGS);
-  if (d->precision == BEVR_PREC_F16) return launch<BEVR_PREC_F16>(*d, G, H, tap_ws, table_t, dkey_a, dkey_b, dkey_y, dkey_x, st TAP_DROP_ARGS);
-#if !BEVR_DROP
-  if (d->precision == BEVR_PREC_BF16X3) return bevr_tap_bwd_k_x3(*d, G, H, tap_ws, table_t, dkey_a, dkey_b, dkey_y, dkey_x, st);
-#endif
-  return BEVR_E_PRECISION;
-}
-#endif
+  return run(d, G, H, tap_ws, table_t, dkey_a, dkey_b, dkey_y, dkey_x, nullptr, 0, stream);
+}
+
+extern "C" size_t bevr_attn_tap_bwd_k_ws_bytes(const bevr_attn_desc* d) {
+  if (bevr_check_desc(d)) return 0;
+  return (LIST_HEAD + (size_t)d->n_prob * d->heads * (d->Np / 32)) * sizeof(int);
+}
+
+extern "C" int bevr_attn_tap_bwd_k_ws(const bevr_attn_desc* d, const void* G, const void* H, const void* tap_ws,
+                                      const float* table_t, float* dkey_a, float* dkey_b, float* dkey_y, float* dkey_x,
+                                      void* ws, int max_workgroups, void* stream) {
+  if (!ws) return BEVR_E_NULL;
+  if (!bevr_aligned16(ws)) return BEVR_E_ALIGN;
+  if (max_workgroups < 0) return BEVR_E_SHAPE;
+  return run(d, G, H, tap_ws, table_t, dkey_a, dkey_b, dkey_y, dkey_x, (int*)ws, max_workgroups, stream);
+}
+#endif
+#endif
diff --git a/bevrender_amd/ops.py b/bevrender_amd/ops.py
--- a/bevrender_amd/ops.py
+++ b/bevrender_amd/ops.py
@@ -423,8 +423,8 @@
     return (x >> 16) >= thr16
 
 
-def _launch(entry, *args, flops=None, nbytes=0.0, tag="", timer=None, label=None):
-    fn = getattr(_lib.lib(), entry)
+def _launch(entry, *args, flops=None, nbytes=0.0, tag="", timer=None, label=None, symbol=None):
+    fn = getattr(_lib.lib(), symbol or entry)
     rc = fn(*args) if flops is None else KERNEL_TIMER.run(timer or entry, flops, fn, *args, nbytes=nbytes, tag=tag)
     _lib.check(rc, label or entry)
 
@@ -662,7 +662,22 @@
             _stream(), flops=_attn_flops(o.g, 4), tag=_call_tag(o.g))
 
 
+def bwd_k_list() -> bool:
+    return os.environ.get("BEVR_BWDK_LIST", "1") != "0"
+
+
+def _list_ws(ws_bytes, o, like):
+    return torch.empty(getattr(_lib.lib(), ws_bytes)(C.byref(o.desc)), device=like.device, dtype=torch.uint8)
+
+
 def _bwd_k_tile(name, o):
+    if name == K.BWD_K and bwd_k_list():
+        ws = _list_ws("bevr_attn_bwd_k_ws_bytes", o, o.dK)
+        _launch(name, C.byref(o.desc), _ptr(o.Qe), _ptr(o.Qt), _ptr(o.Ke), _ptr(o.Ve), _ptr(o.ka), _ptr(o.kb),
+                _ptr(o.pair), _ptr(o.dOe), _ptr(o.dOt), _ptr(o.LSE), _ptr(o.delta), _ptr(o.gscale), _ptr(o.dK), _ptr(o.dV),
+                _ptr(o.da), _ptr(o.db), _ptr(ws), 0, _stream(), flops=_attn_flops(o.g, 4), tag=_call_tag(o.g),
+                symbol="bevr_attn_bwd_k_ws")
+        return
     _bwd_k(name, o, _ptr(o.ka), _ptr(o.kb))
 
 
@@ -681,6 +696,11 @@
 
 
 def _tap_bwd_k(name, o):
+    if name == K.TAP_BWD_K and o.desc.precision in (_lib.PREC_BF16, _lib.PREC_F16) and bwd_k_list():
+        ws = _list_ws("bevr_attn_tap_bwd_k_ws_bytes", o, o.dk[0])
+        _launch(name, C.byref(o.desc), _ptr(o.Gq), _ptr(o.H16), _ptr(o.ws), _ptr(o.Ttc), *[_ptr(t) for t in o.dk], _ptr(ws),
+                0, _stream(), flops=_attn_flops(o.g, 4), tag=_call_tag(o.g), symbol="bevr_attn_tap_bwd_k_ws")
+        return
     _launch(name, C.byref(o.desc), _ptr(o.Gq), _ptr(o.H16), _ptr(o.ws), _ptr(o.Ttc), *[_ptr(t) for t in o.dk], *o.drop,
             _stream(), flops=_attn_flops(o.g, 4), tag=_call_tag(o.g))
 
diff --git a/include/bevrender_hip.h b/include/bevrender_hip.h
--- a/include/bevrender_hip.h
+++ b/include/bevrender_hip.h
@@ -58,6 +58,12 @@
                     const void* dO, const void* dOt, const float* LSE, const float* delta, const float* grad_scale,
                     float* dK, float* dV, float* dkey_a, float* dkey_b, void* stream);
 
+size_t bevr_attn_bwd_k_ws_bytes(const bevr_attn_desc* d);
+int bevr_attn_bwd_k_ws(const bevr_attn_desc* d, const void* Q, const void* Qt, const void* K, const void* V,
+                       const float* key_a, const float* key_b, const float* table_pair,
+                       const void* dO, const void* dOt, const float* LSE, const float* delta, const float* grad_scale,
+                       float* dK, float* dV, float* dkey_a, float* dkey_b, void* ws, int max_workgroups, void* stream);
+
 int bevr_attn_fwd_dropout(const bevr_attn_desc* d, const void* Q, const void* K, const void* Vt,
                           const void* key_ws, const float* table_pair, float* O, float* LSE,
                           unsigned drop_thr, unsigned drop_seed, void* stream);
@@ -92,6 +98,11 @@
 int bevr_attn_tap_bwd_k(const bevr_attn_desc* d, const void* G, const void* H, const void* tap_ws,
                         const float* table, float* dkey_a, float* dkey_b, float* dkey_y, float* dkey_x, void* stream);
 
+size_t bevr_attn_tap_bwd_k_ws_bytes(const bevr_attn_desc* d);
+int bevr_attn_tap_bwd_k_ws(const bevr_attn_desc* d, const void* G, const void* H, const void* tap_ws,
+                           const float* table, float* dkey_a, float* dkey_b, float* dkey_y, float* dkey_x,
+                           void* ws, int max_workgroups, void* stream);
+
 int bevr_attn_tap_fwd_dropout(const bevr_attn_desc* d, const void* G, const void* tap_ws, const float* table_pair,
                               float* mref, float* R, float* lsum, int32_t* flags, unsigned key0, unsigned drop_thr,
                               unsigned drop_seed, void* stream);
```

After: 5.861 samples/s, median of 6. 1.01x the previous value.
